# GoekeLab/m6anet

Measured on AMD Instinct MI355X. Metric: DRACH sites/sec at num_iterations=1000, higher is better.
Workload: dtype f32

## Files before the change

include/m6a.h:

```cpp
#ifndef M6A_H
#define M6A_H
#include <stddef.h>
#include <stdint.h>
#ifdef __cplusplus
extern "C" {
#endif

typedef struct m6a_ctx m6a_ctx;

enum {
    M6A_OK = 0,
    M6A_EINVAL = -1,
    M6A_ENOMEM = -2,
    M6A_EHIP = -3,
    M6A_ESTREAM = -4,
    M6A_ENODEV = -5,
    M6A_EUNSUPPORTED = -6,
    M6A_EFORMAT = -7,
    M6A_EIO = -8,
    M6A_EDECLINED = -9
};

enum { M6A_RNG_NUMPY = 0 };

#define M6A_N_WEIGHTS 7997
#define M6A_N_FEATURES 9
#define M6A_MAX_SAMPLES 64
#define M6A_N_REPR 32
#define M6A_N_KMERS 66

int m6a_create(m6a_ctx **out, const float *weights, size_t n_floats, int device_id);
void m6a_destroy(m6a_ctx *ctx);
const char *m6a_last_error(const m6a_ctx *ctx);

int m6a_set_stream(m6a_ctx *ctx, void *hip_stream);
int m6a_set_job_offset(m6a_ctx *ctx, int64_t first_site);
int m6a_sync(m6a_ctx *ctx);
int m6a_set_host_offsets(m6a_ctx *ctx, const int64_t *off_host);
int m6a_prepare_host_io(m6a_ctx *ctx);
int m6a_host_alloc(size_t bytes, void **out);
int m6a_host_free(void *p);
int m6a_host_is_pinned(const void *p, size_t bytes);

int m6a_encode_reads(m6a_ctx *ctx, const float *X, const uint8_t *site_kmers, const int64_t *off,
                     int64_t n_sites, float *read_prob);

int m6a_read_representation(m6a_ctx *ctx, const float *X, const uint8_t *site_kmers, const int64_t *off,
                            int64_t n_sites, float *repr, float *read_prob);

#define M6A_REPR_F32 0
#define M6A_REPR_F16 1
int m6a_read_representation_dtype(m6a_ctx *ctx, const float *X, const uint8_t *site_kmers, const int64_t *off,
                                  int64_t n_sites, void *repr, int dtype, float *read_prob);

int m6a_site_pool(m6a_ctx *ctx, const float *read_prob, const int64_t *off, int64_t n_sites,
                  int n_iters, int n_samples, float read_proba_threshold, uint32_t seed,
                  int rng_mode, int64_t batch_size, int64_t save_per_batch,
                  float *site_prob, double *mod_ratio);

int m6a_infer(m6a_ctx *ctx, const float *X, const uint8_t *site_kmers, const int64_t *off,
              int64_t n_sites, int n_iters, int n_samples, float read_proba_threshold,
              uint32_t seed, int rng_mode, int64_t batch_size, int64_t save_per_batch,
              float *read_prob, float *site_prob, double *mod_ratio);

int m6a_site_expectation(m6a_ctx *ctx, const float *read_prob, const int64_t *off, int64_t n_sites, int n_samples,
                         float read_proba_threshold, float *site_prob, double *mod_ratio, double *mc_sigma);
enum { M6A_SITE_SAMPLED = 0, M6A_SITE_EXPECTED = 1 };
int m6a_set_site_mode(m6a_ctx *ctx, int mode);

int m6a_job_begin(m6a_ctx *ctx, int n_iters, int n_samples, float read_proba_threshold, uint32_t seed, int rng_mode,
                  int64_t batch_size, int64_t save_per_batch, int64_t expect_sites, int64_t expect_reads);
int m6a_job_feed(m6a_ctx *ctx, const float *X, const uint8_t *site_kmers, const int64_t *off, int64_t n_sites);
int m6a_job_feed_collated(m6a_ctx *ctx, const float *features, const int64_t *kmers, const int64_t *n_reads, int64_t n_sites);
int m6a_job_size(const m6a_ctx *ctx, int64_t *n_sites, int64_t *n_reads);
int m6a_job_end(m6a_ctx *ctx, float *read_prob, float *site_prob, double *mod_ratio);
int m6a_job_abort(m6a_ctx *ctx);

int m6a_bag_forward(m6a_ctx *ctx, const float *X, const uint8_t *site_kmers, int64_t n_bags,
                    int bag, float *site_prob);

int m6a_validate_pool(m6a_ctx *ctx, const float *read_prob, const int64_t *off, int64_t n_sites,
                      int n_iters, int n_samples, uint32_t seed, float *y_pred, float *y_pred_avg);
int m6a_validate(m6a_ctx *ctx, const float *X, const uint8_t *site_kmers, const int64_t *off,
                 int64_t n_sites, int n_iters, int n_samples, uint32_t seed, float *read_prob,
                 float *y_pred, float *y_pred_avg);


int64_t m6a_flush_groups(int64_t n_sites, int64_t batch_size, int64_t save_per_batch,
                         int64_t *group_off, int64_t cap);

int64_t m6a_reference_written_sites(int64_t n_sites, int64_t batch_size, int64_t save_per_batch);

int m6a_shard_plan(const int64_t *off, int64_t n_sites, int64_t batch_size, int64_t save_per_batch,
                   int n_shards, int64_t *shard_site_off);

#define M6A_COMM_ID_BYTES 128
int m6a_comm_unique_id(void *id_out);
int m6a_comm_init(m6a_ctx *ctx, const void *unique_id, int rank, int world_size);
int m6a_gather(m6a_ctx *ctx, const float *site_prob, const double *mod_ratio, const int64_t *shard_site_off,
               int dst, float *site_all, double *mod_all);
int m6a_gather_reads(m6a_ctx *ctx, const float *read_prob, const int64_t *shard_read_off, int dst, float *read_all);
int m6a_comm_destroy(m6a_ctx *ctx);
int m6a_comm_count(m6a_ctx *ctx, int *ranks_seen);
int m6a_comm_info(m6a_ctx *ctx, int *rank, int *device, int *rccl_version);
int m6a_device_link(int dev_a, int dev_b, int *link_type, int *hops, int *peer_access);
int m6a_device_count(void);

int m6a_random_stream(m6a_ctx *ctx, uint32_t seed, int64_t n_words, uint32_t *words);

int m6a_profile_enable(m6a_ctx *ctx, int on);
int m6a_profile_read(m6a_ctx *ctx, int kind, double *total_ms, int64_t *n_launches);
int m6a_profile_clock(m6a_ctx *ctx, int kind, double *ghz_median, double *ghz_min, double *ghz_max, double *span_ms, int *n_waves);
int m6a_set_encoder_variant(m6a_ctx *ctx, int mode);
const char *m6a_last_encoder_variant(const m6a_ctx *ctx);
const char *m6a_last_encoder_kernel(const m6a_ctx *ctx);
int m6a_set_scan_driver(m6a_ctx *ctx, int mode);
int m6a_set_table_variant(m6a_ctx *ctx, int mode);
const char *m6a_last_pool_variant(const m6a_ctx *ctx);

const char *m6a_version(void);

typedef struct m6a_prep m6a_prep;
struct m6a_io_prep_table;
int m6a_prep_eventalign(int device_id, const char *path, int n_neighbors, const char *index_path, m6a_prep **out);
const struct m6a_io_prep_table *m6a_prep_table(const m6a_prep *p);
int m6a_prep_times(const m6a_prep *p, double *ms6);
void m6a_prep_free(m6a_prep *p);
const char *m6a_prep_last_error(void);

typedef struct m6a_prep_sites m6a_prep_sites;
struct m6a_io_rows;
typedef struct m6a_prep_host_half {
    int (*rows)(const char *eventalign_path, int64_t n_runs, const int64_t *start, const int64_t *end, const int64_t *read,
                int n_neighbors, int n_threads, struct m6a_io_rows **out);
    const struct m6a_io_prep_table *(*table)(const struct m6a_io_rows *r);
    void (*free)(struct m6a_io_rows *r);
    const char *(*error)(void);
} m6a_prep_host_half;
typedef struct m6a_prep_sites_info {
    int64_t n_sites, n_reads, n_tx;
    const float *X;
    const uint8_t *site_kmers;
    const int64_t *off;
    float *read_prob, *site_prob;
    double *mod_ratio;
    const int64_t *off_host;
    const uint32_t *site_tx;
    const int64_t *site_pos;
    const char *site_kmer7;
    const char *tx_blob;
    const int64_t *tx_off;
    const double *read_ids;
    double ms[8];
    int64_t d2h_bytes;
    int n_rep;
    const int32_t *read_rep;
    int64_t peak_bytes;
    int64_t n_windows, window_bytes;
    int64_t n_bgzf_blocks, compressed_bytes;
    double ms_inflate;
    int64_t n_declined_sites;
} m6a_prep_sites_info;
int m6a_prep_sites_build(int device_id, const char *path, int readcount_min, int readcount_max, int min_segment_count,
                         const char *norm_kmers, const double *norm_mean, const double *norm_std, int n_norm,
                         const m6a_prep_host_half *host, int n_threads, m6a_prep_sites **out);
int m6a_prep_sites_build_multi(int device_id, const char *const *paths, int n_paths, int readcount_min, int readcount_max,
                               int min_segment_count, const char *norm_kmers, const double *norm_mean, const double *norm_std, int n_norm,
                               const m6a_prep_host_half *host, int n_threads, m6a_prep_sites **out);
int m6a_prep_sites_build_windows(int device_id, const char *const *paths, int n_paths, int readcount_min, int readcount_max,
                                 int min_segment_count, const char *norm_kmers, const double *norm_mean, const double *norm_std, int n_norm,
                                 const m6a_prep_host_half *host, int n_threads, int64_t window_bytes, m6a_prep_sites **out);
int m6a_prep_sites_build_names(int device_id, const char *const *paths, int n_paths, int readcount_min, int readcount_max,
                               int min_segment_count, const char *norm_kmers, const double *norm_mean, const double *norm_std, int n_norm,
                               const m6a_prep_host_half *host, int n_threads, int64_t window_bytes, int read_names, m6a_prep_sites **out);
int m6a_prep_sites_read_names(const m6a_prep_sites *p, const uint8_t **names16, const int64_t **name_off, int *n_rep);
double m6a_prep_sites_intern_ms(const m6a_prep_sites *p);
#define M6A_PREP_STREAM_WINDOW_BYTES ((int64_t)256 << 20)
int64_t m6a_prep_sites_stream_bytes(const m6a_prep_sites *p);
int64_t m6a_prep_sites_n_streams(const m6a_prep_sites *p);
const m6a_prep_sites_info *m6a_prep_sites_get(const m6a_prep_sites *p);
int m6a_prep_sites_fetch(m6a_prep_sites *p, float *read_prob, float *site_prob, double *mod_ratio);
int m6a_prep_sites_inputs(m6a_prep_sites *p, float *X, uint8_t *site_kmers, int64_t *off);
void m6a_prep_sites_free(m6a_prep_sites *p);

struct m6a_io_info;
struct m6a_io_info_table;
typedef struct m6a_json_host_half {
    int (*open)(const char *dir, int min_reads, struct m6a_io_info **out);
    const struct m6a_io_info_table *(*table)(const struct m6a_io_info *info);
    int (*rows)(struct m6a_io_info *info, const int64_t *sites, int64_t n, const char *norm_kmers, const double *norm_mean,
                const double *norm_std, int n_norm, int n_threads, float *X, double *read_ids, uint8_t *site_kmers, char *kmer7);
    void (*free)(struct m6a_io_info *info);
    const char *(*error)(void);
} m6a_json_host_half;
int m6a_json_sites_build(int device_id, const char *const *dirs, int n_dirs, int min_reads, const char *norm_kmers,
                         const double *norm_mean, const double *norm_std, int n_norm, const m6a_json_host_half *host, int n_threads,
                         m6a_prep_sites **out);

typedef struct m6a_norm_host_half {
    int (*partials)(const char *json_path, int64_t n_sites, const char *tx_blob, const int64_t *tx_off, const int64_t *pos,
                    const int64_t *start, const int64_t *end, const int64_t *n_reads, const int64_t *sites, int64_t n, int n_threads,
                    double *s, double *s2, char *kmer7);
    const char *(*error)(void);
} m6a_norm_host_half;
typedef struct m6a_norm_stats {
    double ms_upload, ms_kernels, ms_host, ms_fold, ms_total;
    int64_t n_sites, n_reads, n_kmers, n_declined, d2h_bytes, peak_bytes;
} m6a_norm_stats;
int m6a_norm_factors_build(int device_id, const char *json_path, int64_t n_sites, const char *tx_blob, const int64_t *tx_off,
                           const int64_t *pos, const int64_t *start, const int64_t *end, const int64_t *n_reads,
                           const m6a_norm_host_half *host, int n_threads, char *kmers, int64_t *N, double *S, double *S2, double *mean,
                           double *std, int64_t *n_kmers, uint8_t *status, char *kmer7, m6a_norm_stats *stats);

typedef struct m6a_csv_arrays {
    int64_t n_sites, n_tx;
    const int64_t *off;
    const uint32_t *site_tx;
    const int64_t *site_pos;
    const char *kmer5;
    const char *tx_blob;
    const int64_t *tx_off;
    const double *read_ids;
    const int32_t *read_rep;
    int n_rep;
    const float *read_prob, *site_prob;
    const double *mod_ratio;
} m6a_csv_arrays;
typedef struct m6a_csv_stats {
    double ms_format, ms_copy, ms_write;
    int64_t site_bytes, indiv_bytes;
    int64_t n_declined, d2h_bytes, n_rounds;
} m6a_csv_stats;
int m6a_csv_format(int device_id, const m6a_csv_arrays *a, int64_t site_begin, int64_t site_end, char *site_text, int64_t site_cap,
                   char *indiv_text, int64_t indiv_cap, int64_t *site_bytes, int64_t *indiv_bytes, int64_t *n_declined);
int m6a_prep_sites_write_csv(m6a_prep_sites *p, const char *out_dir, int write_header, int64_t n_sites_limit, int n_threads,
                             m6a_csv_stats *stats);

typedef struct m6a_dataprep_stats {
    double ms_front, ms_back, ms_format, ms_copy, ms_write;
    int64_t json_bytes, index_bytes;
    int64_t n_sites, n_runs, n_declined, n_rounds;
    int64_t d2h_bytes, peak_bytes;
} m6a_dataprep_stats;
int m6a_repr_format(int device_id, const double *v, int64_t n, int round3, char *text, int64_t cap, int64_t *off ,
                    int64_t *n_declined);
int m6a_prep_dataprep_write(int device_id, const char *path, const char *out_dir, int readcount_min, int readcount_max,
                            int min_segment_count, int compress, const m6a_prep_host_half *host, int n_threads,
                            m6a_dataprep_stats *stats);

typedef struct m6a_bgzf_stats {
    int64_t n_blocks, compressed_bytes;
    double ms_upload, ms_inflate, ms_crc, ms_copy;
    int64_t d2h_bytes;
} m6a_bgzf_stats;
int m6a_bgzf_inflate(int device_id, const char *path, char *text, int64_t cap, int64_t *n_bytes, m6a_bgzf_stats *stats);

typedef struct m6a_deflate_stats {
    int64_t n_blocks, n_stored;
    double ms_deflate, ms_copy;
    int64_t d2h_bytes;
} m6a_deflate_stats;
int m6a_bgzf_deflate(int device_id, const char *text, int64_t n, char *out, int64_t cap, int64_t *n_bytes, m6a_deflate_stats *stats);
int m6a_bgzf_deflate_level(int device_id, const char *text, int64_t n, int level, char *out, int64_t cap, int64_t *n_bytes,
                           m6a_deflate_stats *stats, int64_t n_by_type[3]);
typedef struct m6a_csv_bgzf_stats {
    double ms_format, ms_deflate, ms_copy, ms_write;
    int64_t site_bytes, indiv_bytes;
    int64_t site_compressed, indiv_compressed;
    int64_t n_blocks, n_stored;
    int64_t n_declined, d2h_bytes, n_rounds;
} m6a_csv_bgzf_stats;
int m6a_prep_sites_write_csv_bgzf(m6a_prep_sites *p, const char *out_dir, int write_header, int64_t n_sites_limit, int n_threads,
                                  m6a_csv_bgzf_stats *stats);
int m6a_prep_sites_write_csv_bgzf_level(m6a_prep_sites *p, const char *out_dir, int write_header, int64_t n_sites_limit, int n_threads,
                                        int level, m6a_csv_bgzf_stats *stats, int64_t n_by_type[3]);

typedef struct m6a_repr_write_stats {
    double ms_kernel, ms_copy, ms_write;
    int64_t n_rounds, n_rows;
    int64_t bytes;
    int64_t round_bytes;
    int64_t d2h_bytes;
} m6a_repr_write_stats;
int m6a_prep_sites_write_read_representation(m6a_prep_sites *p, m6a_ctx *ctx, const char *path, int dtype, int64_t n_sites_limit,
                                             m6a_repr_write_stats *stats);

typedef struct m6a_trainer m6a_trainer;
typedef struct { float lr, beta1, beta2, eps, weight_decay; } m6a_train_config;
int m6a_train_create(m6a_ctx *ctx, const float *weights, size_t n_floats, const m6a_train_config *cfg, m6a_trainer **out);
void m6a_train_destroy(m6a_trainer *t);
int m6a_train_step(m6a_trainer *t, const float *X, const uint8_t *site_kmers, const float *y, int64_t n_bags, int bag,
                   float *loss, float *y_pred);
int m6a_train_epoch(m6a_trainer *t, const float *X, const uint8_t *site_kmers, const int64_t *off, const float *y, int64_t n_sites,
                    const int64_t *order, int64_t n_order, int64_t batch_size, int bag, uint64_t seed,
                    float *loss, float *y_pred);
int m6a_train_sample(const int64_t *off, const int64_t *order, int64_t n_order, int bag, uint64_t seed, int64_t *read_idx);
int m6a_train_grads(m6a_trainer *t, float *grads);
int m6a_train_weights(m6a_trainer *t, float *weights, int64_t *n_steps);
int m6a_train_stats(const m6a_trainer *t, int64_t *n_steps, int64_t *n_launches, int64_t *n_syncs);
int m6a_train_set_clip(m6a_trainer *t, float max_norm);
int m6a_train_last_norm(m6a_trainer *t, float *total_norm);
int m6a_train_state_get(m6a_trainer *t, float *m, float *v, int64_t *n_steps);
int m6a_train_state_set(m6a_trainer *t, const float *m, const float *v, int64_t n_steps);
int m6a_train_set_weights(m6a_trainer *t, const float *blob);
int m6a_train_forward(m6a_trainer *t, const float *X, const uint8_t *site_kmers, int64_t n_bags, int bag, int training,
                      float *s, int64_t *ticket);
int m6a_train_running_stats(m6a_trainer *t, float *stats);
int m6a_train_backward(m6a_trainer *t, int64_t ticket, const float *grad_s, float *grads);

#ifdef __cplusplus
}
#endif
#endif
```

m6anet_amd/_lib.py:

```python
import ctypes as C
import os

_PKG = os.path.dirname(os.path.abspath(__file__))
LIB_PATH = os.environ.get("M6A_HIP_LIB") or os.path.join(_PKG, "libm6a_hip.so")

M6A_OK = 0
ERRORS = {-1: "M6A_EINVAL", -2: "M6A_ENOMEM", -3: "M6A_EHIP", -4: "M6A_ESTREAM", -5: "M6A_ENODEV",
          -6: "M6A_EUNSUPPORTED", -7: "M6A_EFORMAT", -8: "M6A_EIO", -9: "M6A_EDECLINED"}
M6A_EDECLINED = -9
RNG_NUMPY = 0
REPR_DTYPES = {"float32": 0, "float16": 1}

SYMBOLS = ["m6a_create", "m6a_destroy", "m6a_last_error", "m6a_set_stream", "m6a_set_job_offset", "m6a_set_scan_driver", "m6a_set_table_variant", "m6a_set_encoder_variant", "m6a_last_encoder_variant", "m6a_last_encoder_kernel", "m6a_sync", "m6a_set_host_offsets", "m6a_prepare_host_io", "m6a_host_alloc", "m6a_host_free", "m6a_host_is_pinned",
           "m6a_encode_reads", "m6a_read_representation", "m6a_read_representation_dtype", "m6a_site_pool", "m6a_site_expectation", "m6a_set_site_mode", "m6a_infer", "m6a_job_begin", "m6a_job_feed", "m6a_job_feed_collated", "m6a_job_size", "m6a_job_end", "m6a_job_abort", "m6a_bag_forward", "m6a_validate_pool", "m6a_validate", "m6a_flush_groups",
           "m6a_reference_written_sites",
           "m6a_shard_plan", "m6a_comm_unique_id", "m6a_comm_init", "m6a_gather", "m6a_gather_reads", "m6a_device_count", "m6a_random_stream", "m6a_comm_destroy", "m6a_comm_count", "m6a_comm_info", "m6a_device_link", "m6a_profile_enable", "m6a_profile_read", "m6a_profile_clock", "m6a_last_pool_variant",
           "m6a_version", "m6a_prep_eventalign", "m6a_prep_table", "m6a_prep_times", "m6a_prep_free", "m6a_prep_last_error",
           "m6a_prep_sites_build", "m6a_prep_sites_build_multi", "m6a_prep_sites_build_windows", "m6a_prep_sites_build_names", "m6a_prep_sites_read_names", "m6a_prep_sites_intern_ms", "m6a_prep_sites_stream_bytes", "m6a_prep_sites_n_streams", "m6a_prep_sites_get", "m6a_prep_sites_fetch", "m6a_prep_sites_inputs", "m6a_prep_sites_free",
           "m6a_csv_format", "m6a_prep_sites_write_csv", "m6a_bgzf_inflate", "m6a_bgzf_deflate", "m6a_prep_sites_write_csv_bgzf",
           "m6a_bgzf_deflate_level", "m6a_prep_sites_write_csv_bgzf_level", "m6a_prep_sites_write_read_representation", "m6a_json_sites_build", "m6a_norm_factors_build", "m6a_repr_format", "m6a_prep_dataprep_write",
           "m6a_train_create", "m6a_train_destroy", "m6a_train_step", "m6a_train_epoch", "m6a_train_sample", "m6a_train_grads", "m6a_train_weights", "m6a_train_stats",
           "m6a_train_set_clip", "m6a_train_last_norm", "m6a_train_state_get", "m6a_train_state_set",
           "m6a_train_set_weights", "m6a_train_forward", "m6a_train_running_stats", "m6a_train_backward"]

_lib = None


class HostHalf(C.Structure):
    _fields_ = [("rows", C.c_void_p), ("table", C.c_void_p), ("free", C.c_void_p), ("error", C.c_void_p)]


class JsonHostHalf(C.Structure):
    _fields_ = [("open", C.c_void_p), ("table", C.c_void_p), ("rows", C.c_void_p), ("free", C.c_void_p), ("error", C.c_void_p)]


class NormHostHalf(C.Structure):
    _fields_ = [("partials", C.c_void_p), ("error", C.c_void_p)]


class NormStats(C.Structure):
    _fields_ = [("ms_upload", C.c_double), ("ms_kernels", C.c_double), ("ms_host", C.c_double), ("ms_fold", C.c_double),
                ("ms_total", C.c_double), ("n_sites", C.c_int64), ("n_reads", C.c_int64), ("n_kmers", C.c_int64),
                ("n_declined", C.c_int64), ("d2h_bytes", C.c_int64), ("peak_bytes", C.c_int64)]


class PrepSitesInfo(C.Structure):
    _fields_ = [("n_sites", C.c_int64), ("n_reads", C.c_int64), ("n_tx", C.c_int64), ("X", C.c_void_p), ("site_kmers", C.c_void_p),
                ("off", C.c_void_p), ("read_prob", C.c_void_p), ("site_prob", C.c_void_p), ("mod_ratio", C.c_void_p),
                ("off_host", C.c_void_p), ("site_tx", C.c_void_p), ("site_pos", C.c_void_p), ("site_kmer7", C.c_void_p),
                ("tx_blob", C.c_void_p), ("tx_off", C.c_void_p), ("read_ids", C.c_void_p), ("ms", C.c_double * 8),
                ("d2h_bytes", C.c_int64), ("n_rep", C.c_int), ("read_rep", C.c_void_p), ("peak_bytes", C.c_int64),
                ("n_windows", C.c_int64), ("window_bytes", C.c_int64),
                ("n_bgzf_blocks", C.c_int64), ("compressed_bytes", C.c_int64), ("ms_inflate", C.c_double),
                ("n_declined_sites", C.c_int64)]


class BgzfStats(C.Structure):
    _fields_ = [("n_blocks", C.c_int64), ("compressed_bytes", C.c_int64), ("ms_upload", C.c_double), ("ms_inflate", C.c_double),
                ("ms_crc", C.c_double), ("ms_copy", C.c_double), ("d2h_bytes", C.c_int64)]


class DeflateStats(C.Structure):
    _fields_ = [("n_blocks", C.c_int64), ("n_stored", C.c_int64), ("ms_deflate", C.c_double), ("ms_copy", C.c_double), ("d2h_bytes", C.c_int64)]


class CsvBgzfStats(C.Structure):
    _fields_ = [("ms_format", C.c_double), ("ms_deflate", C.c_double), ("ms_copy", C.c_double), ("ms_write", C.c_double),
                ("site_bytes", C.c_int64), ("indiv_bytes", C.c_int64), ("site_compressed", C.c_int64), ("indiv_compressed", C.c_int64),
                ("n_blocks", C.c_int64), ("n_stored", C.c_int64), ("n_declined", C.c_int64), ("d2h_bytes", C.c_int64), ("n_rounds", C.c_int64)]


class CsvArrays(C.Structure):
    _fields_ = [("n_sites", C.c_int64), ("n_tx", C.c_int64), ("off", C.c_void_p), ("site_tx", C.c_void_p), ("site_pos", C.c_void_p),
                ("kmer5", C.c_void_p), ("tx_blob", C.c_char_p), ("tx_off", C.c_void_p), ("read_ids", C.c_void_p), ("read_rep", C.c_void_p),
                ("n_rep", C.c_int), ("read_prob", C.c_void_p), ("site_prob", C.c_void_p), ("mod_ratio", C.c_void_p)]


class CsvStats(C.Structure):
    _fields_ = [("ms_format", C.c_double), ("ms_copy", C.c_double), ("ms_write", C.c_double), ("site_bytes", C.c_int64),
                ("indiv_bytes", C.c_int64), ("n_declined", C.c_int64), ("d2h_bytes", C.c_int64), ("n_rounds", C.c_int64)]


class ReprWriteStats(C.Structure):
    _fields_ = [("ms_kernel", C.c_double), ("ms_copy", C.c_double), ("ms_write", C.c_double), ("n_rounds", C.c_int64), ("n_rows", C.c_int64),
                ("bytes", C.c_int64), ("round_bytes", C.c_int64), ("d2h_bytes", C.c_int64)]


class DataprepStats(C.Structure):
    _fields_ = [("ms_front", C.c_double), ("ms_back", C.c_double), ("ms_format", C.c_double), ("ms_copy", C.c_double), ("ms_write", C.c_double),
                ("json_bytes", C.c_int64), ("index_bytes", C.c_int64), ("n_sites", C.c_int64), ("n_runs", C.c_int64), ("n_declined", C.c_int64),
                ("n_rounds", C.c_int64), ("d2h_bytes", C.c_int64), ("peak_bytes", C.c_int64)]


class TrainConfig(C.Structure):
    _fields_ = [("lr", C.c_float), ("beta1", C.c_float), ("beta2", C.c_float), ("eps", C.c_float), ("weight_decay", C.c_float)]


class M6AError(RuntimeError):
    def __init__(self, code, msg):
        super().__init__("%s (%d): %s" % (ERRORS.get(code, "M6A_E?"), code, msg))
        self.code = code


def _preload_hip_runtime():
    import importlib.util
    try:
        spec = importlib.util.find_spec("torch")
    except (ImportError, ValueError):
        spec = None
    if spec and spec.submodule_search_locations:
        libdir = os.path.join(list(spec.submodule_search_locations)[0], "lib")
        rt = os.path.join(libdir, "libamdhip64.so")
        if os.path.exists(rt):
            C.CDLL(rt, mode=C.RTLD_GLOBAL)
        rccl = os.path.join(libdir, "librccl.so")
        if os.path.exists(rccl):
            os.environ.setdefault("M6A_RCCL_LIB", rccl)


def load():
    global _lib
    if _lib is not None:
        return _lib
    if not os.path.exists(LIB_PATH):
        raise ImportError("libm6a_hip.so is not built: run `python -m m6anet_amd.build` "
                          "(or __graft_entry__.build()); there is no CPU fallback")
    _preload_hip_runtime()
    L = C.CDLL(LIB_PATH)
    vp, i64, i32, u32, f32, sz = C.c_void_p, C.c_int64, C.c_int, C.c_uint32, C.c_float, C.c_size_t
    L.m6a_create.argtypes = [C.POINTER(vp), vp, sz, i32]
    L.m6a_destroy.argtypes = [vp]
    L.m6a_destroy.restype = None
    L.m6a_last_error.argtypes = [vp]
    L.m6a_last_error.restype = C.c_char_p
    L.m6a_set_stream.argtypes = [vp, vp]
    L.m6a_sync.argtypes = [vp]
    L.m6a_set_host_offsets.argtypes = [vp, vp]
    L.m6a_prepare_host_io.argtypes = [vp]
    L.m6a_set_job_offset.argtypes = [vp, i64]
    L.m6a_set_scan_driver.argtypes = [vp, i32]
    L.m6a_set_table_variant.argtypes = [vp, i32]
    L.m6a_set_encoder_variant.argtypes = [vp, i32]
    L.m6a_last_encoder_variant.argtypes = [vp]
    L.m6a_last_encoder_variant.restype = C.c_char_p
    L.m6a_host_alloc.argtypes = [C.c_size_t, C.POINTER(vp)]
    L.m6a_host_free.argtypes = [vp]
    L.m6a_host_is_pinned.argtypes = [vp, C.c_size_t]
    L.m6a_last_encoder_kernel.argtypes = [vp]
    L.m6a_last_encoder_kernel.restype = C.c_char_p
    L.m6a_encode_reads.argtypes = [vp, vp, vp, vp, i64, vp]
    L.m6a_read_representation.argtypes = [vp, vp, vp, vp, i64, vp, vp]
    L.m6a_read_representation_dtype.argtypes = [vp, vp, vp, vp, i64, vp, i32, vp]
    L.m6a_site_pool.argtypes = [vp, vp, vp, i64, i32, i32, f32, u32, i32, i64, i64, vp, vp]
    L.m6a_site_expectation.argtypes = [vp, vp, vp, i64, i32, f32, vp, vp, vp]
    L.m6a_set_site_mode.argtypes = [vp, i32]
    L.m6a_infer.argtypes = [vp, vp, vp, vp, i64, i32, i32, f32, u32, i32, i64, i64, vp, vp, vp]
    L.m6a_job_begin.argtypes = [vp, i32, i32, f32, u32, i32, i64, i64, i64, i64]
    L.m6a_job_feed.argtypes = [vp, vp, vp, vp, i64]
    L.m6a_job_feed_collated.argtypes = [vp, vp, vp, vp, i64]
    L.m6a_job_size.argtypes = [vp, C.POINTER(i64), C.POINTER(i64)]
    L.m6a_job_end.argtypes = [vp, vp, vp, vp]
    L.m6a_job_abort.argtypes = [vp]
    L.m6a_bag_forward.argtypes = [vp, vp, vp, i64, i32, vp]
    L.m6a_validate_pool.argtypes = [vp, vp, vp, i64, i32, i32, C.c_uint32, vp, vp]
    L.m6a_validate.argtypes = [vp, vp, vp, vp, i64, i32, i32, C.c_uint32, vp, vp, vp]
    L.m6a_flush_groups.argtypes = [i64, i64, i64, vp, i64]
    L.m6a_flush_groups.restype = i64
    L.m6a_reference_written_sites.argtypes = [i64, i64, i64]
    L.m6a_reference_written_sites.restype = i64
    L.m6a_shard_plan.argtypes = [vp, i64, i64, i64, i32, vp]
    L.m6a_comm_unique_id.argtypes = [vp]
    L.m6a_comm_init.argtypes = [vp, vp, i32, i32]
    L.m6a_gather.argtypes = [vp, vp, vp, vp, i32, vp, vp]
    L.m6a_gather_reads.argtypes = [vp, vp, vp, i32, vp]
    L.m6a_device_count.argtypes = []
    L.m6a_random_stream.argtypes = [vp, u32, i64, vp]
    L.m6a_comm_destroy.argtypes = [vp]
    pi = C.POINTER(i32)
    L.m6a_comm_count.argtypes = [vp, pi]
    L.m6a_comm_info.argtypes = [vp, pi, pi, pi]
    L.m6a_device_link.argtypes = [i32, i32, pi, pi, pi]
    L.m6a_profile_enable.argtypes = [vp, i32]
    L.m6a_profile_read.argtypes = [vp, i32, C.POINTER(C.c_double), C.POINTER(i64)]
    L.m6a_profile_clock.argtypes = [vp, i32] + [C.POINTER(C.c_double)] * 4 + [C.POINTER(i32)]
    L.m6a_last_pool_variant.argtypes = [vp]
    L.m6a_last_pool_variant.restype = C.c_char_p
    L.m6a_version.restype = C.c_char_p
    L.m6a_prep_eventalign.argtypes = [i32, C.c_char_p, i32, C.c_char_p, C.POINTER(vp)]
    L.m6a_prep_table.argtypes = [vp]
    L.m6a_prep_table.restype = vp
    L.m6a_prep_times.argtypes = [vp, C.POINTER(C.c_double)]
    L.m6a_prep_free.argtypes = [vp]
    L.m6a_prep_free.restype = None
    L.m6a_prep_sites_build.argtypes = [i32, C.c_char_p, i32, i32, i32, C.c_char_p, vp, vp, i32, C.POINTER(HostHalf), i32, C.POINTER(vp)]
    L.m6a_prep_sites_build_multi.argtypes = [i32, C.POINTER(C.c_char_p), i32, i32, i32, i32, C.c_char_p, vp, vp, i32, C.POINTER(HostHalf), i32,
                                             C.POINTER(vp)]
    L.m6a_prep_sites_build_windows.argtypes = [i32, C.POINTER(C.c_char_p), i32, i32, i32, i32, C.c_char_p, vp, vp, i32, C.POINTER(HostHalf), i32,
                                               i64, C.POINTER(vp)]
    L.m6a_prep_sites_build_names.argtypes = [i32, C.POINTER(C.c_char_p), i32, i32, i32, i32, C.c_char_p, vp, vp, i32, C.POINTER(HostHalf), i32,
                                             i64, i32, C.POINTER(vp)]
    L.m6a_prep_sites_read_names.argtypes = [vp, C.POINTER(vp), C.POINTER(vp), C.POINTER(i32)]
    L.m6a_prep_sites_intern_ms.argtypes = [vp]
    L.m6a_prep_sites_intern_ms.restype = C.c_double
    for f in (L.m6a_prep_sites_stream_bytes, L.m6a_prep_sites_n_streams):
        f.argtypes = [vp]
        f.restype = C.c_int64
    L.m6a_json_sites_build.argtypes = [i32, C.POINTER(C.c_char_p), i32, i32, C.c_char_p, vp, vp, i32, C.POINTER(JsonHostHalf), i32, C.POINTER(vp)]
    L.m6a_norm_factors_build.argtypes = [i32, C.c_char_p, i64, vp, vp, vp, vp, vp, vp, C.POINTER(NormHostHalf), i32, vp, vp, vp, vp, vp, vp,
                                         C.POINTER(i64), vp, vp, C.POINTER(NormStats)]
    L.m6a_prep_sites_get.argtypes = [vp]
    L.m6a_prep_sites_get.restype = C.POINTER(PrepSitesInfo)
    L.m6a_prep_sites_fetch.argtypes = [vp, vp, vp, vp]
    L.m6a_prep_sites_inputs.argtypes = [vp, vp, vp, vp]
    L.m6a_prep_sites_free.argtypes = [vp]
    L.m6a_prep_sites_free.restype = None
    pl = C.POINTER(i64)
    L.m6a_csv_format.argtypes = [i32, C.POINTER(CsvArrays), i64, i64, vp, i64, vp, i64, pl, pl, pl]
    L.m6a_prep_sites_write_csv.argtypes = [vp, C.c_char_p, i32, i64, i32, C.POINTER(CsvStats)]
    L.m6a_bgzf_inflate.argtypes = [i32, C.c_char_p, vp, i64, pl, C.POINTER(BgzfStats)]
    L.m6a_bgzf_deflate.argtypes = [i32, C.c_char_p, i64, vp, i64, pl, C.POINTER(DeflateStats)]
    L.m6a_prep_sites_write_csv_bgzf.argtypes = [vp, C.c_char_p, i32, i64, i32, C.POINTER(CsvBgzfStats)]
    L.m6a_bgzf_deflate_level.argtypes = [i32, C.c_char_p, i64, i32, vp, i64, pl, C.POINTER(DeflateStats), pl]
    L.m6a_prep_sites_write_csv_bgzf_level.argtypes = [vp, C.c_char_p, i32, i64, i32, i32, C.POINTER(CsvBgzfStats), pl]
    L.m6a_prep_sites_write_read_representation.argtypes = [vp, vp, C.c_char_p, i32, i64, C.POINTER(ReprWriteStats)]
    L.m6a_repr_format.argtypes = [i32, vp, i64, i32, vp, i64, vp, pl]
    L.m6a_prep_dataprep_write.argtypes = [i32, C.c_char_p, C.c_char_p, i32, i32, i32, i32, C.POINTER(HostHalf), i32, C.POINTER(DataprepStats)]
    L.m6a_train_create.argtypes = [vp, vp, sz, C.POINTER(TrainConfig), C.POINTER(vp)]
    L.m6a_train_destroy.argtypes = [vp]
    L.m6a_train_destroy.restype = None
    L.m6a_train_step.argtypes = [vp, vp, vp, vp, i64, i32, vp, vp]
    L.m6a_train_epoch.argtypes = [vp, vp, vp, vp, vp, i64, vp, i64, i64, i32, C.c_uint64, vp, vp]
    L.m6a_train_sample.argtypes = [vp, vp, i64, i32, C.c_uint64, vp]
    L.m6a_train_grads.argtypes = [vp, vp]
    L.m6a_train_weights.argtypes = [vp, vp, pl]
    L.m6a_train_stats.argtypes = [vp, pl, pl, pl]
    L.m6a_train_set_clip.argtypes = [vp, C.c_float]
    L.m6a_train_last_norm.argtypes = [vp, vp]
    L.m6a_train_state_get.argtypes = [vp, vp, vp, pl]
    L.m6a_train_state_set.argtypes = [vp, vp, vp, i64]
    L.m6a_train_set_weights.argtypes = [vp, vp]
    L.m6a_train_forward.argtypes = [vp, vp, vp, i64, i32, i32, vp, pl]
    L.m6a_train_running_stats.argtypes = [vp, vp]
    L.m6a_train_backward.argtypes = [vp, i64, vp, vp]
    L.m6a_prep_last_error.argtypes = []
    L.m6a_prep_last_error.restype = C.c_char_p
    for name in SYMBOLS:
        fn = getattr(L, name)
        if fn.restype is C.c_int and name not in ("m6a_flush_groups", "m6a_reference_written_sites"):
            fn.restype = C.c_int
    _lib = L
    return L
```

m6anet_amd/csrc/m6a_api.hip:

```cpp
#include "m6a_ctx.h"

#if !defined(__HIP_DEVICE_COMPILE__)
#ifndef M6A_MT_JUMP_PATH
#error "build with -DM6A_MT_JUMP_PATH=\"<repo>/m6anet_amd/assets/mt19937_jump.bin\" (m6anet_amd/build.py does)"
#endif
asm(".section .rodata\n"
    ".global m6a_mt_jump_blob\n.global m6a_mt_jump_blob_end\n.hidden m6a_mt_jump_blob\n.hidden m6a_mt_jump_blob_end\n.balign 64\n"
    "m6a_mt_jump_blob:\n.incbin \"" M6A_MT_JUMP_PATH "\"\n"
    "m6a_mt_jump_blob_end:\n.byte 0\n.previous\n");
#endif

namespace {

thread_local std::string g_create_error;

std::mutex g_live_mu;
std::vector<m6a_ctx *> g_live;
void join_background_setups()
{
    std::lock_guard<std::mutex> g(g_live_mu);
    for (m6a_ctx *c : g_live)
        if (c->warm.joinable()) c->warm.join();
    g_live.clear();
}

}

using namespace m6a_detail;

namespace m6a_detail {


int fail(m6a_ctx *c, int code, const char *fmt, ...)
{
    char buf[512];
    va_list ap;
    va_start(ap, fmt);
    vsnprintf(buf, sizeof buf, fmt, ap);
    va_end(ap);
    if (c && c->warm.joinable() && std::this_thread::get_id() != c->warm.get_id()) c->warm.join();
    if (c) c->err = buf; else g_create_error = buf;
    return code;
}


bool is_device_ptr(const void *p)
{
    if (!p) return false;
    hipPointerAttribute_t at;
    hipError_t e = hipPointerGetAttributes(&at, p);
    if (e != hipSuccess) { (void)hipGetLastError(); return false; }
    return at.type == hipMemoryTypeDevice || at.type == hipMemoryTypeManaged;
}

enum { O_E = 0, O_W1 = 132, O_B1 = 2382, O_G = 2532, O_BE = 2682, O_MU = 2832, O_VAR = 2982,
       O_W2 = 3132, O_B2 = 7932, O_W3 = 7964, O_B3 = 7996 };

void build_fragments(const float *w, std::vector<float> &frag, std::vector<float> &frag2, std::vector<float> &w1e)
{
    std::vector<float> w1(160 * 16, 0.f), w2(32 * 160, 0.f), alpha(160, 0.f), beta(160, 0.f);
    for (int j = 0; j < 150; j++) {
        for (int k = 0; k < 15; k++) w1[j * 16 + k] = w[O_W1 + 15 * j + k];
        w1[j * 16 + 15] = w[O_B1 + j];
        const float invstd = 1.0f / std::sqrt(w[O_VAR + j] + 1e-5f);
        alpha[j] = w[O_G + j] * invstd;
        beta[j] = std::fmaf(-w[O_MU + j], alpha[j], w[O_BE + j]);
    }
    w1[150 * 16 + 15] = 1.0f;
    alpha[150] = 1.0f;
    for (int o = 0; o < 32; o++) {
        for (int k = 0; k < 150; k++) w2[o * 160 + k] = w[O_W2 + 150 * o + k];
        w2[o * 160 + 150] = w[O_B2 + o];
    }
    const float bn_scale = 0x1p-64f;
    for (float &v : alpha) v *= bn_scale;
    for (float &v : beta) v *= bn_scale;
    for (float &v : w2) v *= 0x1p+64f;
    const float w3_scale = 0.5f;
    auto unit_of_row = [](int m, int i) { return 32 * m + 2 * ((i & 3) + 4 * (i >> 3)) + ((i >> 2) & 1); };
    auto out_unit = [](int q, int half) {
        if (half == 0) return q < 8 ? 2 * q + 1 : 2 * (q - 8) + 17;
        return q < 8 ? 2 * q + 2 : (q < 15 ? 2 * (q - 8) + 18 : 0);
    };
    auto out_unit_of_row = [&](int i) { return out_unit((i & 3) + 4 * (i >> 3), (i >> 2) & 1); };
    frag.assign(M6A_WFRAG_FLOATS, 0.f);
    for (int lane = 0; lane < 64; lane++) {
        const int col = lane & 31, half = lane >> 5;
        for (int m = 0; m < 5; m++) {
            for (int st = 0; st < 8; st++)
                frag[(m * 8 + st) * 64 + lane] = w1[unit_of_row(m, col) * 16 + 2 * st + half];
            for (int q = 0; q < 16; q++)
                frag[(40 + m * 16 + q) * 64 + lane] = w2[out_unit_of_row(col) * 160 + 32 * m + 2 * q + half];
        }
        for (int q = 0; q < 16; q++)
            frag[(120 + q) * 64 + lane] = w3_scale * w[O_W3 + out_unit(q, half)];
    }
    frag2.assign(M6A_WFRAG2_FLOATS, 0.f);
    w1e.assign(M6A_W1E_FLOATS + M6A_BN_FLOATS, 0.f);
    for (int lane = 0; lane < 64; lane++) {
        const int col = lane & 31, half = lane >> 5;
        for (int m = 0; m < 5; m++) {
            for (int st = 0; st < 4; st++) frag2[(m * 4 + st) * 64 + lane] = w1[unit_of_row(m, col) * 16 + 2 * st + half];
            frag2[(20 + m) * 64 + lane] = w1[unit_of_row(m, col) * 16 + 8];
        }
    }
    for (int m = 0; m < 5; m++)
        for (int col = 0; col < 32; col++) {
            for (int e = 0; e < 6; e++) w1e[(m * 7 + e) * 32 + col] = w1[unit_of_row(m, col) * 16 + 9 + e];
            w1e[(m * 7 + 6) * 32 + col] = w1[unit_of_row(m, col) * 16 + 15];
        }
    for (int m = 0; m < 5; m++)
        for (int half = 0; half < 2; half++)
            for (int q = 0; q < 16; q++) {
                const int u = 32 * m + 2 * q + half;
                w1e[M6A_W1E_FLOATS + ((m * 2 + half) * 16 + q) * 2] = alpha[u];
                w1e[M6A_W1E_FLOATS + ((m * 2 + half) * 16 + q) * 2 + 1] = beta[u];
            }
}

int64_t flush_groups(int64_t S, int64_t bs, int64_t spb, int64_t base, std::vector<int64_t> &goff)
{
    goff.clear();
    goff.push_back(0);
    if (S <= 0) return 0;
    const int64_t it0 = base / bs;
    const int64_t nb = (S + bs - 1) / bs;
    int64_t start_b = 0;
    for (int64_t b = 0; b < nb; b++) {
        if ((it0 + b + 1) % spb) {
            goff.push_back(std::min((b + 1) * bs, S));
            start_b = b + 1;
        }
    }
    if (start_b < nb) goff.push_back(S);
    return (int64_t)goff.size() - 1;
}

bool base_is_group_start(int64_t base, int64_t bs, int64_t spb)
{
    if (base < 0 || base % bs) return false;
    const int64_t it0 = base / bs;
    return it0 == 0 || (it0 % spb) != 0;
}

int ensure_groups(m6a_ctx *c, hipStream_t st, int64_t S, int64_t bs, int64_t spb)
{
    const int64_t base = c->job_offset;
    if (c->goff_key.valid && c->goff_key.S == S && c->goff_key.bs == bs && c->goff_key.spb == spb &&
        c->goff_key.base == base) return M6A_OK;
    if (!base_is_group_start(base, bs, spb))
        return fail(c, M6A_EINVAL, "job offset %lld does not start a flush group for batch_size=%lld save_per_batch=%lld",
                    (long long)base, (long long)bs, (long long)spb);
    std::vector<int64_t> g;
    const int64_t G = flush_groups(S, bs, spb, base, g);
    int64_t gmax = 0;
    for (int64_t i = 0; i < G; i++) gmax = std::max(gmax, g[i + 1] - g[i]);
    HIPCHK(c, c->goff.ensure(g.size() * sizeof(int64_t)));
    HIPCHK(c, hipMemcpyAsync(c->goff.p, g.data(), g.size() * sizeof(int64_t), hipMemcpyHostToDevice, st));
    HIPCHK(c, hipStreamSynchronize(st));
    c->goff_key = {S, bs, spb, base, G, gmax, true};
    return M6A_OK;
}

constexpr int kJumpPerRegime = 31, kJumpPolyWords = 312;
constexpr int64_t kXheadWords = 22016;

extern "C" const unsigned char m6a_mt_jump_blob[];
extern "C" const unsigned char m6a_mt_jump_blob_end[];

struct JumpRegime { int64_t G; const uint64_t *polys; };

const JumpRegime *jump_regimes(int *n_out)
{
    static JumpRegime reg[8];
    static int n = 0;
    static std::once_flag once;
    std::call_once(once, [] {
        const unsigned char *b = m6a_mt_jump_blob;
        const size_t len = (size_t)(m6a_mt_jump_blob_end - m6a_mt_jump_blob);
        uint32_t hdr[4];
        if (len >= 24 && std::memcmp(b, "M6AMTJP1", 8) == 0) {
            std::memcpy(hdr, b + 8, 16);
            const size_t per = 8 + (size_t)hdr[1] * hdr[2] * 8;
            if (hdr[0] <= 8 && hdr[1] == (uint32_t)kJumpPerRegime && hdr[2] == (uint32_t)kJumpPolyWords && hdr[3] == 512 &&
                len == 24 + hdr[0] * per)
                for (uint32_t r = 0; r < hdr[0]; r++) {
                    const unsigned char *q = b + 24 + r * per;
                    int64_t G;
                    std::memcpy(&G, q, 8);
                    reg[n++] = {G, (const uint64_t *)(q + 8)};
                }
        }
    });
    *n_out = n;
    return reg;
}

int launch_stream(m6a_ctx *c, hipStream_t st, uint32_t seed, int64_t len, uint32_t *raw)
{
    int n_reg = 0;
    const JumpRegime *reg = jump_regimes(&n_reg);
    const JumpRegime *use = nullptr;
    static const bool allowed = !(getenv("M6A_MT_SEGMENTS") && getenv("M6A_MT_SEGMENTS")[0] == '0');
    if (allowed && n_reg > 0 && len > reg[0].G + kXheadWords) {
        use = &reg[n_reg - 1];
        for (int r = 0; r < n_reg; r++) if (len <= (int64_t)(kJumpPerRegime + 1) * reg[r].G) { use = &reg[r]; break; }
    }
    if (!use) {
        hipLaunchKernelGGL(mt19937_kernel, dim3(1), dim3(640), 0, st, seed, len, raw, (const uint32_t *)nullptr, len,
                           (uint32_t *)nullptr, (int64_t)0);
        HIPCHK(c, hipGetLastError());
        return M6A_OK;
    }
    const int n_seg = (int)std::min<int64_t>((len + use->G - 1) / use->G, kJumpPerRegime + 1);
    const size_t poly_bytes = (size_t)kJumpPerRegime * kJumpPolyWords * 8;
    HIPCHK(c, c->mt_scratch.ensure((size_t)kXheadWords * 4 + (size_t)kJumpPerRegime * 1078 * 4 + poly_bytes));
    uint32_t *xhead = (uint32_t *)c->mt_scratch.p, *hist = xhead + kXheadWords;
    uint64_t *d_polys = (uint64_t *)(hist + (size_t)kJumpPerRegime * 1078);
    if (c->mt_polys_G != use->G) {
        HIPCHK(c, hipMemcpyAsync(d_polys, use->polys, poly_bytes, hipMemcpyHostToDevice, st));
        c->mt_polys_G = use->G;
    }
    hipLaunchKernelGGL(mt19937_kernel, dim3(1), dim3(640), 0, st, seed, kXheadWords - 624, raw, (const uint32_t *)nullptr,
                       kXheadWords, xhead, kXheadWords);
    hipLaunchKernelGGL(mt_jump_kernel, dim3(17, (unsigned)(n_seg - 1)), dim3(256), 0, st, (const uint32_t *)xhead,
                       (const uint64_t *)d_polys, hist);
    hipLaunchKernelGGL(mt19937_kernel, dim3((unsigned)n_seg), dim3(640), 0, st, seed, len, raw, (const uint32_t *)hist, use->G,
                       (uint32_t *)nullptr, (int64_t)0);
    HIPCHK(c, hipGetLastError());
    return M6A_OK;
}

int ensure_raw(m6a_ctx *c, hipStream_t st, uint32_t seed, int64_t len)
{
    if (c->raw_len >= len && c->raw_seed == seed) return M6A_OK;
    if (len > ((int64_t)1 << 31) - 512)
        return fail(c, M6A_ESTREAM, "a flush group would need %lld MT19937 words (cap 2^31); "
                    "reduce batch_size*save_per_batch or num_iterations", (long long)len);
    len = (len + 1023) / 1024 * 1024;
    c->raw_len = 0;
    c->rt.valid = false;
    HIPCHK(c, c->raw.ensure((size_t)len * 4));
    int rc = launch_stream(c, st, seed, len, (uint32_t *)c->raw.p);
    if (rc) return rc;
    c->raw_seed = seed; c->raw_len = len;
    return M6A_OK;
}

void pairwise_rec(int lo, int n, MeanPlan &p)
{
    if (n <= 128) {
        p.leaf_start.push_back(lo);
        p.merge_after.push_back(0);
        return;
    }
    int n2 = n / 2;
    n2 -= n2 % 8;
    pairwise_rec(lo, n2, p);
    pairwise_rec(lo + n2, n - n2, p);
    p.merge_after.back()++;
}

int plan_iteration(const MeanPlan &p, int row, int lane)
{
    const int L = (int)p.merge_after.size();
    const int ps = p.row_pass[row], i = p.row_round[row];
    if (ps < 0) return lane < p.n_rem ? p.T - p.n_rem + lane : -1;
    const int b = 8 * ps + (lane >> 3);
    if (b >= L) return -1;
    const int len = p.leaf_start[b + 1] - p.leaf_start[b];
    return i < len / 8 ? p.leaf_start[b] + 8 * i + (lane & 7) : -1;
}

void build_mean_plan(int T, MeanPlan &p)
{
    p = MeanPlan();
    p.T = T;
    pairwise_rec(0, T, p);
    p.leaf_start.push_back(T);
    const int L = (int)p.merge_after.size();
    const int last_len = p.leaf_start[L] - p.leaf_start[L - 1];
    p.n_rem = last_len % 8;
    if (p.n_rem) { p.row_pass.push_back(-1); p.row_round.push_back(0); }
    const int P = (L + 7) / 8;
    for (int ps = 0; ps < P; ps++) {
        int rounds = 0;
        for (int b = 8 * ps; b < std::min(L, 8 * ps + 8); b++)
            rounds = std::max(rounds, (p.leaf_start[b + 1] - p.leaf_start[b]) / 8);
        rounds = std::max(rounds, 1);
        for (int i = 0; i < rounds; i++) { p.row_pass.push_back(ps); p.row_round.push_back(i); }
    }
    int d = 0;
    for (int b = 0; b < L; b++) {
        d++; p.depth = std::max(p.depth, d); d -= p.merge_after[b];
        p.max_merge = std::max<int>(p.max_merge, p.merge_after[b]);
    }
    p.reg_ctl.assign((size_t)std::max(1, (T - p.n_rem) / 8), 0u);
    for (int b = 0; b + 1 < L; b++) p.reg_ctl[(size_t)p.leaf_start[b + 1] / 8 - 1] = 1u | ((uint32_t)p.merge_after[b] << 8);
    const int rows = (int)p.row_pass.size();
    p.row_meta.assign((size_t)rows * 4, 0u);
    for (int r = 0; r < rows; r++) {
        uint32_t *m = &p.row_meta[(size_t)r * 4];
        uint64_t live = 0;
        for (int l = 0; l < 64; l++) live |= (uint64_t)(plan_iteration(p, r, l) >= 0) << l;
        m[1] = (uint32_t)live; m[2] = (uint32_t)(live >> 32);
        const int ps = p.row_pass[r];
        if (ps < 0) { m[0] = 1u << 25; continue; }
        if (r + 1 == rows || p.row_pass[r + 1] != ps) {
            const int nl = std::min(8, L - 8 * ps);
            m[0] = (1u << 24) | ((uint32_t)nl << 26) | (ps == P - 1 ? 1u << 30 : 0u);
            for (int bl = 0; bl < nl; bl++) m[3] |= (uint32_t)(p.merge_after[8 * ps + bl] & 15) << (4 * bl);
        }
    }
}

int ensure_mean_plan(m6a_ctx *c, hipStream_t st, int T)
{
    if (c->plan.T == T && c->plan_dev.p) return M6A_OK;
    build_mean_plan(T, c->plan);
    const MeanPlan &p = c->plan;
    if (p.depth > M6A_MEAN_STACK) return fail(c, M6A_EUNSUPPORTED, "n_iters %d: pairwise-sum tree deeper than %d", T, M6A_MEAN_STACK);
    const size_t b0 = p.leaf_start.size() * 4, b1 = (p.merge_after.size() + 3) / 4 * 4, b2 = std::max<size_t>(p.row_meta.size(), 1) * 4;
    const size_t b3 = p.reg_ctl.size() * 4;
    HIPCHK(c, c->plan_dev.ensure(b0 + b1 + b2 + b3));
    char *d = (char *)c->plan_dev.p;
    HIPCHK(c, hipMemcpyAsync(d, p.leaf_start.data(), b0, hipMemcpyHostToDevice, st));
    HIPCHK(c, hipMemcpyAsync(d + b0, p.merge_after.data(), p.merge_after.size(), hipMemcpyHostToDevice, st));
    if (!p.row_meta.empty())
        HIPCHK(c, hipMemcpyAsync(d + b0 + b1, p.row_meta.data(), p.row_meta.size() * 4, hipMemcpyHostToDevice, st));
    HIPCHK(c, hipMemcpyAsync(d + b0 + b1 + b2, p.reg_ctl.data(), b3, hipMemcpyHostToDevice, st));
    HIPCHK(c, hipStreamSynchronize(st));
    c->plan_off[0] = 0; c->plan_off[1] = b0; c->plan_off[2] = b0 + b1; c->plan_off[3] = b0 + b1 + b2;
    c->tab_key.valid = false;
    return M6A_OK;
}

void plan_args(m6a_ctx *c, PoolArgs &a)
{
    const char *d = (const char *)c->plan_dev.p;
    a.leaf_start = (const int *)(d + c->plan_off[0]);
    a.merge_after = (const uint8_t *)(d + c->plan_off[1]);
    a.row_meta = (const uint32_t *)(d + c->plan_off[2]);
    a.n_leaves = (int)c->plan.merge_after.size();
    a.n_rows = (int)c->plan.row_pass.size();
    a.n_rem = c->plan.n_rem;
    a.stack_depth = c->plan.depth;
    a.reg_ctl = (const uint32_t *)(d + c->plan_off[3]);
    a.reg_rounds = (a.T - c->plan.n_rem) / 8;
    a.reg_final_merges = c->plan.merge_after.back();
}

int64_t stream_need(int64_t gmax, int T, int K)
{
    const int64_t A = (int64_t)T * K;
    return gmax * (2 * A + A / 16) + 8192;
}

uint32_t *ctl_cursor(m6a_ctx *c) { return c->h_ctl; }
int32_t *ctl_slot(m6a_ctx *c) { return (int32_t *)(c->h_ctl + M6A_HIST_BINS); }
int32_t *ctl_build_n(m6a_ctx *c) { return ctl_slot(c) + M6A_RTAB_MAX_N + 1; }
int32_t *ctl_build_slot(m6a_ctx *c) { return ctl_build_n(c) + M6A_RTAB_MAX_N; }
constexpr size_t kCtlWords = M6A_HIST_BINS + (M6A_RTAB_MAX_N + 1) + 2 * M6A_RTAB_MAX_N;

int rtab_missing(const m6a_ctx *c, uint32_t seed, int T, int K, int64_t need, const uint32_t *hist, int *n_distinct)
{
    const bool valid = c->rt.valid && c->rt.seed == seed && c->rt.A == (int64_t)T * K && c->raw_seed == seed &&
                       c->rt.n_blk * 64 >= need && c->rt.n_blk == c->raw_len / 64;
    int missing = 0, distinct = 0;
    for (int n = 2; n <= M6A_RTAB_MAX_N; n++)
        if (hist[n]) { distinct++; if (!valid || c->rt.slot_of_n[n] < 0) missing++; }
    if (n_distinct) *n_distinct = distinct;
    return missing;
}

int ensure_rtab(m6a_ctx *c, hipStream_t st, uint32_t seed, int T, int K, int64_t gmax, const uint32_t *hist, bool *usable)
{
    *usable = false;
    const int64_t need = stream_need(gmax, T, K);
    int rc = ensure_raw(c, st, seed, need);
    if (rc) return rc;
    auto &rt = c->rt;
    const int64_t n_blk = c->raw_len / 64;
    if (!(rt.valid && rt.seed == seed && rt.A == (int64_t)T * K && rt.n_blk == n_blk)) {
        rt.valid = false; rt.used = 0;
        for (int n = 0; n <= M6A_RTAB_MAX_N; n++) rt.slot_of_n[n] = -1;
    }
    std::vector<int> todo;
    for (int n = 2; n <= M6A_RTAB_MAX_N; n++)
        if (hist[n] && rt.slot_of_n[n] < 0) todo.push_back(n);
    const int64_t c_stride = n_blk * 64;
    const size_t slot_bytes = (size_t)c_stride * 2 + (size_t)(n_blk + 1) * 4;
    const bool fresh = !rt.valid || rt.n_blk != n_blk;
    const int want = (fresh ? 1 : rt.used) + (int)todo.size();
    if (fresh || want > rt.cap) {
        int new_cap = std::max(want, fresh ? 0 : rt.cap * 2);
        new_cap = std::min(std::max(new_cap, std::max(32, c->rt_presize)), M6A_RTAB_MAX_N + 1);
        size_t free_b = 0, total_b = 0;
        HIPCHK(c, hipMemGetInfo(&free_b, &total_b));
        const size_t held = fresh ? 0 : (size_t)rt.cap * slot_bytes;
        const size_t budget = std::min<size_t>((size_t)16 << 30, (free_b + held) / 2);
        if ((size_t)new_cap * slot_bytes > budget) new_cap = want;
        if ((size_t)new_cap * slot_bytes > budget) return M6A_OK;
        uint16_t *nC = nullptr; uint32_t *nRS = nullptr;
        if (fresh) {
            if (rt.C) (void)hipFree(rt.C);
            if (rt.RS) (void)hipFree(rt.RS);
            rt.C = nullptr; rt.RS = nullptr; rt.cap = 0;
        }
        if (hipMalloc((void **)&nC, (size_t)new_cap * c_stride * 2 + 64) != hipSuccess) { (void)hipGetLastError(); return M6A_OK; }
        if (hipMalloc((void **)&nRS, (size_t)new_cap * (n_blk + 1) * 4) != hipSuccess) { (void)hipGetLastError(); (void)hipFree(nC); return M6A_OK; }
        if (!fresh && rt.used) {
            HIPCHK(c, hipMemcpyAsync(nC, rt.C, (size_t)rt.used * c_stride * 2, hipMemcpyDeviceToDevice, st));
            HIPCHK(c, hipMemcpyAsync(nRS, rt.RS, (size_t)rt.used * (n_blk + 1) * 4, hipMemcpyDeviceToDevice, st));
            HIPCHK(c, hipStreamSynchronize(st));
            c->graveyard.push_back(rt.C); c->graveyard.push_back(rt.RS);
        }
        rt.C = nC; rt.RS = nRS; rt.cap = new_cap;
        if (fresh) {
            HIPCHK(c, hipMemsetAsync(rt.C, 0, (size_t)c_stride * 2, st));
            HIPCHK(c, hipMemsetAsync(rt.RS, 0, (size_t)(n_blk + 1) * 4, st));
            rt.used = 1;
        }
        rt.valid = true; rt.seed = seed; rt.A = (int64_t)T * K; rt.n_blk = n_blk;
    }
    if (!todo.empty()) {
        int32_t *bn = ctl_build_n(c), *bs = ctl_build_slot(c);
        for (size_t i = 0; i < todo.size(); i++) { bn[i] = todo[i]; bs[i] = rt.used; rt.slot_of_n[todo[i]] = rt.used++; }
        HIPCHK(c, c->ctl_dev.ensure(kCtlWords * 4));
        int32_t *d_bn = (int32_t *)c->ctl_dev.p + (ctl_build_n(c) - (int32_t *)c->h_ctl);
        HIPCHK(c, hipMemcpyAsync(d_bn, bn, (size_t)2 * M6A_RTAB_MAX_N * 4, hipMemcpyHostToDevice, st));
        RtabBuild b;
        b.raw = (const uint32_t *)c->raw.p; b.n_blk = (uint32_t)n_blk; b.build_n = d_bn; b.build_slot = d_bn + M6A_RTAB_MAX_N;
        b.C = rt.C; b.RS = rt.RS; b.c_stride = c_stride; b.n_build = (int)todo.size();
        const unsigned gx = (unsigned)std::min<int64_t>((n_blk + 63) / 64, 65535);
        const unsigned gn = (unsigned)((todo.size() + 7) / 8);
        hipLaunchKernelGGL(rtab_count_kernel, dim3(gn, gx), dim3(256), 0, st, b);
        hipLaunchKernelGGL(rtab_scan_kernel, dim3((unsigned)todo.size()), dim3(256), 0, st, b);
        hipLaunchKernelGGL(rtab_fill_kernel, dim3(gn, gx), dim3(256), 0, st, b);
        HIPCHK(c, hipGetLastError());
        HIPCHK(c, hipStreamSynchronize(st));
    }
    *usable = true;
    return M6A_OK;
}

int uniform_slice(m6a_ctx *c, hipStream_t st, uint32_t seed, int n, int T, int K, int jmax, const uint16_t **C)
{
    *C = nullptr;
    if (n < 2) return M6A_OK;
    std::vector<uint32_t> hist(M6A_HIST_BINS, 0u);
    hist[n] = 1;
    bool usable = false;
    int rc = ensure_rtab(c, st, seed, T, K, jmax, hist.data(), &usable);
    if (rc) return rc;
    if (!usable) return fail(c, M6A_ENOMEM, "no device memory for the index table of bag size %d", n);
    const int64_t slot = c->rt.slot_of_n[n], A = (int64_t)T * K;
    uint32_t total = 0;
    HIPCHK(c, hipMemcpyAsync(&total, c->rt.RS + slot * (c->rt.n_blk + 1) + c->rt.n_blk, 4, hipMemcpyDeviceToHost, st));
    HIPCHK(c, hipStreamSynchronize(st));
    if ((int64_t)total < A * jmax) return fail(c, M6A_ESTREAM, "MT19937 stream too short for a flush group");
    *C = c->rt.C + slot * c->rt.n_blk * 64;
    return M6A_OK;
}

int ensure_table_reg(m6a_ctx *c, hipStream_t st, uint32_t seed, int n, int T, int K, int jmax)
{
    auto &k = c->tab_reg_key;
    if (k.valid && k.seed == seed && k.n == n && k.T == T && k.K == K && k.jmax >= jmax) return M6A_OK;
    k.valid = false;
    const size_t per_j = (size_t)(T + 8) * K;
    const size_t bytes = (size_t)jmax * per_j * 2 + 4096;
    HIPCHK(c, c->tab_reg.ensure(bytes));
    HIPCHK(c, hipMemsetAsync(c->tab_reg.p, 0, bytes, st));
    const uint16_t *C = nullptr;
    int rc = uniform_slice(c, st, seed, n, T, K, jmax, &C);
    if (rc) return rc;
    if (C) {
        const int64_t A = (int64_t)T * K;
        hipLaunchKernelGGL(rtab_to_reg_table_kernel, dim3((unsigned)((A * jmax + 255) / 256)), dim3(256), 0, st,
                           C, A, (int64_t)per_j, jmax, (uint16_t *)c->tab_reg.p);
        HIPCHK(c, hipGetLastError());
    }
    k = {seed, n, T, K, jmax, true};
    return M6A_OK;
}

int ensure_table(m6a_ctx *c, hipStream_t st, uint32_t seed, int n, int T, int K, int jmax)
{
    int rc = ensure_mean_plan(c, st, T);
    if (rc) return rc;
    auto &k = c->tab_key;
    if (k.valid && k.seed == seed && k.n == n && k.T == T && k.K == K && k.jmax >= jmax) return M6A_OK;
    k.valid = false;
    const MeanPlan &p = c->plan;
    const int rows = (int)p.row_pass.size();
    c->iter_of.resize((size_t)rows * 64);
    for (int r = 0; r < rows; r++)
        for (int l = 0; l < 64; l++) c->iter_of[(size_t)r * 64 + l] = plan_iteration(p, r, l);
    const size_t words = (size_t)jmax * rows * 5 * 64;
    HIPCHK(c, c->tab.ensure(words * 4 + c->iter_of.size() * 4));
    int *d_iter = (int *)((uint32_t *)c->tab.p + words);
    HIPCHK(c, hipMemcpyAsync(d_iter, c->iter_of.data(), c->iter_of.size() * 4, hipMemcpyHostToDevice, st));
    const uint16_t *C = nullptr;
    rc = uniform_slice(c, st, seed, n, T, K, jmax, &C);
    if (rc) return rc;
    if (C) {
        hipLaunchKernelGGL(rtab_to_lds_table_kernel, dim3((unsigned)((words + 255) / 256)), dim3(256), 0, st,
                           C, (int64_t)T * K, K, rows, jmax, (const int *)d_iter, (uint32_t *)c->tab.p);
        HIPCHK(c, hipGetLastError());
    } else {
        HIPCHK(c, hipMemsetAsync(c->tab.p, 0, words * 4, st));
    }
    k = {seed, n, T, K, jmax, true};
    return M6A_OK;
}

void prof_begin(m6a_ctx *c, int kind)
{
    Profiler &p = c->prof;
    if (!p.on || !(p.mask >> kind & 1)) return;
    if (p.used[kind] >= kMaxProfiled) { p.dropped[kind]++; return; }
    if ((int)p.start[kind].size() <= p.used[kind]) {
        hipEvent_t a, b;
        (void)hipEventCreate(&a); (void)hipEventCreate(&b);
        p.start[kind].push_back(a); p.stop[kind].push_back(b);
    }
    (void)hipEventRecord(p.start[kind][p.used[kind]], c->stream);
}
void prof_end(m6a_ctx *c, int kind)
{
    Profiler &p = c->prof;
    if (!p.on || !(p.mask >> kind & 1) || p.used[kind] >= kMaxProfiled) return;
    (void)hipEventRecord(p.stop[kind][p.used[kind]], c->stream);
    p.used[kind]++;
}

void host_bag_range(m6a_ctx *c, const int64_t *off, int64_t S);
int sync_and_check(m6a_ctx *c);

int query_bags(m6a_ctx *c, const int64_t *d_off, int64_t S)
{
    if (c->side_work) { HIPCHK(c, hipStreamSynchronize(c->s_prep)); c->side_work = false; }
    c->h_minmax[0] = ~0ull; c->h_minmax[1] = 0ull; c->h_minmax[2] = 0ull;
    HIPCHK(c, hipMemcpyAsync(c->d_minmax, c->h_minmax, 24, hipMemcpyHostToDevice, c->stream));
    HIPCHK(c, hipMemsetAsync(c->d_hist, 0, M6A_HIST_BINS * 4, c->stream));
    hipLaunchKernelGGL(bag_minmax_kernel, dim3((unsigned)std::min<int64_t>((S + 255) / 256, 512)), dim3(256), 0,
                       c->stream, d_off, S, c->d_minmax, c->d_hist);
    HIPCHK(c, hipGetLastError());
    HIPCHK(c, hipMemcpyAsync(c->h_minmax, c->d_minmax, 24, hipMemcpyDeviceToHost, c->stream));
    HIPCHK(c, hipMemcpyAsync(c->h_hist, c->d_hist, M6A_HIST_BINS * 4, hipMemcpyDeviceToHost, c->stream));
    HIPCHK(c, hipStreamSynchronize(c->stream));
    c->bag_min = (int64_t)c->h_minmax[0];
    c->bag_max = (int64_t)c->h_minmax[1];
    c->n_reads = (int64_t)c->h_minmax[2];
    return M6A_OK;
}

int bag_stats(m6a_ctx *c, const int64_t *d_off, int64_t S)
{
    const int64_t *h = c->hint_off;
    c->hint_off = nullptr;
    if (!h) return query_bags(c, d_off, S);
    if (h[0] != 0) return fail(c, M6A_EINVAL, "off[0] must be 0");
    host_bag_range(c, h, S);
    if (c->bag_min < 0) return fail(c, M6A_EINVAL, "off[] must be non-decreasing");
    unsigned long long hash = 0;
    for (int i = 0; i < M6A_HIST_BINS; i++) hash += (unsigned long long)c->h_hist[i] * m6a_bin_weight(i);
    hipStream_t st = c->s_prep ? c->s_prep : c->stream;
    if (st != c->stream) {
        HIPCHK(c, hipEventRecord(c->ev_main, c->stream));
        HIPCHK(c, hipStreamWaitEvent(st, c->ev_main, 0));
    }
    HIPCHK(c, hipMemsetAsync(c->d_minmax, 0xff, 8, st));
    HIPCHK(c, hipMemsetAsync(c->d_minmax + 1, 0, 16, st));
    HIPCHK(c, hipMemsetAsync(c->d_hist, 0, M6A_HIST_BINS * 4, st));
    hipLaunchKernelGGL(bag_minmax_kernel, dim3((unsigned)std::min<int64_t>((S + 255) / 256, 512)), dim3(256), 0,
                       st, d_off, S, c->d_minmax, c->d_hist);
    hipLaunchKernelGGL(bag_verify_kernel, dim3(1), dim3(256), 0, st, c->d_minmax, c->d_hist, (unsigned long long)c->bag_min,
                       (unsigned long long)c->bag_max, (unsigned long long)c->n_reads, hash, c->d_err);
    HIPCHK(c, hipGetLastError());
    c->side_work = true;
    return M6A_OK;
}

static unsigned enc_args(m6a_ctx *c, EncArgs &a, const float *X, const uint8_t *km, const int64_t *off, int64_t S, int64_t R, float *rp)
{
    a.X = X; a.site_kmers = km; a.off = off; a.wfrag = c->d_wfrag; a.emb = c->d_emb; a.read_prob = rp;
    a.wfrag2 = c->d_wfrag2; a.w1e_tab = c->d_w1e; a.bn = c->d_w1e + M6A_W1E_FLOATS; a.err = c->d_err;
    a.n_sites = S; a.n_reads = R; a.n_tiles = (R + 31) / 32; a.b3 = c->b3;
    a.clk = nullptr;
    const int64_t max_waves = (int64_t)c->n_cu * 8;
    a.tiles_per_wave = (a.n_tiles + max_waves - 1) / max_waves;
    const int64_t waves = (a.n_tiles + a.tiles_per_wave - 1) / a.tiles_per_wave;
    return (unsigned)((waves + 3) / 4);
}

int launch_encode(m6a_ctx *c, const float *X, const uint8_t *km, const int64_t *off, int64_t S,
                  int64_t R, float *rp)
{
    if (R <= 0 || S <= 0) return M6A_OK;
    EncArgs a;
    const unsigned blocks = enc_args(c, a, X, km, off, S, R, rp);
    a.clk = c->prof.clk_for(0);
    const bool fits32 = S < 0x7ffffff0LL && a.n_tiles < 0x7ffffff0LL;
    if (c->enc_variant == 2 && !fits32) return fail(c, M6A_EUNSUPPORTED, "12-slot encoder: more than 2^31 sites or tiles");
    const bool scalar_chain = c->bag_min >= M6A_CSITE_MIN_BAG && fits32;
    const bool csite = c->enc_variant == 2 || (c->enc_variant == 4 && scalar_chain);
    const bool site16 = !csite && c->enc_variant != 3 && scalar_chain;
    c->enc_variant_used = csite ? "csite12" : "general16";
    c->enc_kernel_used = csite ? "enc_csite_kernel" : site16 ? "enc_site16_kernel" : "enc_kernel";
    prof_begin(c, 0);
    if (csite) hipLaunchKernelGGL(enc_csite_kernel, dim3(blocks), dim3(256), 0, c->stream, a);
    else if (site16) hipLaunchKernelGGL(enc_site16_kernel, dim3(blocks), dim3(256), 0, c->stream, a);
    else hipLaunchKernelGGL(enc_kernel, dim3(blocks), dim3(256), 0, c->stream, a);
    prof_end(c, 0);
    HIPCHK(c, hipGetLastError());
    return M6A_OK;
}

int launch_repr(m6a_ctx *c, const float *X, const uint8_t *km, const int64_t *off, int64_t S, int64_t R, void *repr, int dtype, float *rp)
{
    if (R <= 0 || S <= 0) return M6A_OK;
    EncReprArgs ra;
    const unsigned blocks = enc_args(c, ra.enc, X, km, off, S, R, rp);
    ra.repr = repr;
    c->enc_variant_used = "general16";
    c->enc_kernel_used = dtype == M6A_REPR_F16 ? "enc_repr_kernel<true>" : "enc_repr_kernel";
    prof_begin(c, 0);
    if (dtype == M6A_REPR_F16)
        hipLaunchKernelGGL(enc_repr_kernel<true>, dim3(blocks), dim3(256), 0, c->stream, ra);
    else
        hipLaunchKernelGGL(enc_repr_kernel<false>, dim3(blocks), dim3(256), 0, c->stream, ra);
    prof_end(c, 0);
    HIPCHK(c, hipGetLastError());
    return M6A_OK;
}

int repr_writer_begin(m6a_ctx *c, int device, hipStream_t *stream)
{
    settle(c);
    HintScope hint_scope(c);
    if (c->job.open) return job_busy(c);
    if (c->device != device) return fail(c, M6A_EINVAL, "the context is on device %d, the sites are on device %d", c->device, device);
    HIPCHK(c, hipSetDevice(c->device));
    *stream = c->stream;
    return M6A_OK;
}

int repr_writer_round(m6a_ctx *c, const float *X, const uint8_t *km, const int64_t *off, int64_t *off_round, int64_t s0, int64_t s1,
                      int64_t r0, int64_t nr, void *repr, int dtype)
{
    if (nr <= 0 || s1 <= s0) return M6A_OK;
    hipLaunchKernelGGL(rebase_off_kernel, dim3((unsigned)((s1 - s0 + 1 + 255) / 256)), dim3(256), 0, c->stream, off + s0, s1 - s0 + 1, off_round);
    HIPCHK(c, hipGetLastError());
    return launch_repr(c, X + r0 * 9, km + s0 * 3, off_round, s1 - s0, nr, repr, dtype, nullptr);
}

RtabUse rtab_use(m6a_ctx *c, int64_t nmax, uint32_t si_base = 0, uint32_t si_count = 0)
{
    RtabUse u;
    u.C = c->rt.C; u.RS = c->rt.RS; u.slot_of_n = (const int32_t *)c->ctl_dev.p + M6A_HIST_BINS;
    u.rank = (uint32_t *)c->rt_rank.p; u.order = (const uint32_t *)c->rt_order.p;
    u.c_stride = c->rt.n_blk * 64; u.n_blk = (uint32_t)c->rt.n_blk;
    u.bag_cap = (int)std::max<int64_t>(64, (nmax + 63) / 64 * 64);
    u.si_base = si_base; u.si_count = si_count;
    return u;
}

int rtab_prepare(m6a_ctx *c, hipStream_t st, PoolArgs a, int64_t nmax, int64_t gmax, uint32_t seed, bool *use)
{
    *use = false;
    const int T = a.T, K = a.K;
    const int64_t S = a.n_sites;
    const int64_t need = stream_need(gmax, T, K);
    if (nmax > M6A_RTAB_MAX_N || c->scan_driver == 1 || c->scan_driver == 2) {
        if (c->scan_driver == 3)
            return fail(c, M6A_EUNSUPPORTED, "index-table pooling needs every bag <= %d reads (largest: %lld)", M6A_RTAB_MAX_N, (long long)nmax);
        return M6A_OK;
    }
    int distinct = 0;
    const int missing = rtab_missing(c, seed, T, K, need, c->h_hist, &distinct);
    if (c->rt_credit_seed != seed || c->rt_credit_A != (int64_t)T * K) { c->rt_credit_seed = seed; c->rt_credit_A = (int64_t)T * K; c->rt_credit = 0; }
    bool use_rtab = c->scan_driver == 3 || missing == 0 || c->rt_credit + S >= (int64_t)16 * missing;
    if (use_rtab) c->rt_credit = 0; else c->rt_credit += S;
    if (!use_rtab) return M6A_OK;
    int rc = ensure_rtab(c, st, seed, T, K, gmax, c->h_hist, &use_rtab);
    if (rc) return rc;
    if (!use_rtab) return M6A_OK;
    a.raw = (const uint32_t *)c->raw.p; a.raw_len = c->raw_len;
    HIPCHK(c, c->rt_rank.ensure((size_t)S * 4));
    HIPCHK(c, c->rt_order.ensure((size_t)S * 4));
    HIPCHK(c, c->ctl_dev.ensure(kCtlWords * 4));
    HIPCHK(c, hipEventSynchronize(c->ev_ctl));
    uint32_t *cur = ctl_cursor(c);
    uint32_t run = 0;
    for (int n = M6A_HIST_BINS - 1; n > M6A_RTAB_SMALL_N; n--) { cur[n] = run; run += c->h_hist[n]; }
    for (int x = 0; x < 8; x++)
        for (int n = M6A_RTAB_SMALL_N - ((M6A_RTAB_SMALL_N - x) & 7); n >= 0; n -= 8) { cur[n] = run; run += c->h_hist[n]; }
    std::memcpy(ctl_slot(c), c->rt.slot_of_n, sizeof c->rt.slot_of_n);
    HIPCHK(c, hipMemcpyAsync(c->ctl_dev.p, c->h_ctl, (size_t)(M6A_HIST_BINS + M6A_RTAB_MAX_N + 1) * 4, hipMemcpyHostToDevice, st));
    HIPCHK(c, hipEventRecord(c->ev_ctl, st));
    const RtabUse u = rtab_use(c, nmax);
    const unsigned n_order_blocks = (unsigned)((S + 255) / 256);
    const unsigned n_chain_blocks = (unsigned)std::min<int64_t>((a.n_groups + 3) / 4, (int64_t)c->n_cu * 16);
    hipLaunchKernelGGL(rtab_prep_kernel, dim3(n_order_blocks + n_chain_blocks), dim3(256), 0, st, a, u,
                       (uint32_t *)c->ctl_dev.p, (uint32_t *)c->rt_order.p, n_order_blocks);
    HIPCHK(c, hipGetLastError());
    *use = true;
    return M6A_OK;
}

struct PoolPlan {
    enum Kind { none, table_reg, table, ragged_table, scan_group, scan_site, expected } kind = none;
    PoolArgs a = {};
    int64_t bag_min = 0, bag_max = 0;
    unsigned blocks = 0, start_blocks = 0;
    size_t lds = 0;
    int64_t n_big = 0, cap_big = 0, cap_small = 0;
};

int pool_plan(m6a_ctx *c, hipStream_t st, const int64_t *off, int64_t S, int T, int K, uint32_t seed, int64_t bs, int64_t spb,
              PoolPlan *p)
{
    *p = PoolPlan();
    PoolArgs &a = p->a;
    if (S <= 0) return M6A_OK;
    if (c->site_mode == M6A_SITE_EXPECTED) {
        if (!base_is_group_start(c->job_offset, bs, spb))
            return fail(c, M6A_EINVAL, "job offset %lld does not start a flush group for batch_size=%lld save_per_batch=%lld",
                        (long long)c->job_offset, (long long)bs, (long long)spb);
        if (c->bag_min < 0 || c->bag_max > 0x7fffffff) return fail(c, M6A_EINVAL, "off[] is not a non-decreasing CSR array");
        a.off = off; a.n_sites = S; a.K = K;
        p->bag_min = c->bag_min; p->bag_max = c->bag_max;
        p->kind = PoolPlan::expected;
        return M6A_OK;
    }
    int rc = ensure_groups(c, st, S, bs, spb);
    if (rc) return rc;
    const int64_t nmin = c->bag_min, nmax = c->bag_max;
    if (nmin < 0 || nmax > 0x7fffffff) return fail(c, M6A_EINVAL, "off[] is not a non-decreasing CSR array");
    a.off = off; a.goff = (const int64_t *)c->goff.p; a.err = c->d_err;
    a.n_groups = c->goff_key.G; a.n_sites = S; a.T = T; a.K = K;
    const int64_t gmax = c->goff_key.gmax;

    rc = ensure_mean_plan(c, st, T);
    if (rc) return rc;
    plan_args(c, a);
    const bool uniform = nmin == nmax && nmin >= 1 && nmin <= M6A_TABLE_MAX_N && K == 20 && gmax <= 4096;
    const bool reg_ok = uniform && c->plan.depth <= M6A_REG_STACK && c->n_reads < (int64_t)1 << 30 &&
                        (int64_t)gmax * (T + 8) * K * 2 <= (int64_t)256 << 20;
    if (uniform && reg_ok && c->table_variant != 1) {
        rc = ensure_table_reg(c, st, seed, (int)nmin, T, K, (int)gmax);
        if (rc) return rc;
        a.tab = (const uint32_t *)c->tab_reg.p; a.uniform_n = (int)nmin; a.jmax = (int)gmax;
        const int64_t wpj = (a.n_groups + 255) / 256;
        a.reg_items = wpj * a.jmax;
        p->blocks = (unsigned)((a.reg_items + 7) / 8 * 8);
        p->kind = PoolPlan::table_reg;
        return M6A_OK;
    }
    if (uniform && c->plan.max_merge <= 15) {
        rc = ensure_table(c, st, seed, (int)nmin, T, K, (int)gmax);
        if (rc) return rc;
        a.tab = (const uint32_t *)c->tab.p; a.uniform_n = (int)nmin; a.jmax = (int)gmax;
        const int64_t gblocks = (a.n_groups + 7) / 8;
        int64_t nbj = std::max<int64_t>(1, ((int64_t)c->n_cu * 5 + a.jmax - 1) / a.jmax);
        nbj = std::min<int64_t>(nbj, (gblocks + 3) / 4);
        p->blocks = (unsigned)(nbj * a.jmax);
        p->lds = (size_t)4 * (128 + 8 * a.stack_depth) * sizeof(float);
        p->kind = PoolPlan::table;
        return M6A_OK;
    }
    bool use_rtab = false;
    rc = rtab_prepare(c, st, a, nmax, gmax, seed, &use_rtab);
    if (rc) return rc;
    if (use_rtab) {
        a.raw = (const uint32_t *)c->raw.p; a.raw_len = c->raw_len;
        for (int n = M6A_RTAB_SMALL_N + 1; n < M6A_HIST_BINS; n++) p->n_big += c->h_hist[n];
        p->cap_big = nmax; p->cap_small = std::min<int64_t>(nmax, M6A_RTAB_SMALL_N);
        p->kind = PoolPlan::ragged_table;
        return M6A_OK;
    }
    rc = ensure_raw(c, st, seed, stream_need(gmax, T, K));
    if (rc) return rc;
    a.raw = (const uint32_t *)c->raw.p; a.raw_len = c->raw_len;
    HIPCHK(c, c->start_pos.ensure((size_t)S * sizeof(uint32_t)));
    a.start_pos = (uint32_t *)c->start_pos.p;
    int64_t cap = 64;
    while (cap < nmax && cap < M6A_BAG_LDS) cap *= 2;
    a.bag_cap = (int)cap;
    p->lds = (size_t)4 * (a.bag_cap + (32 * K + 256) * 5 / 4 + 32 + M6A_MEAN_STACK) * sizeof(float);
    const int64_t wg_per_cu = std::max<int64_t>(1, std::min<int64_t>(a.bag_cap >= 256 ? 5 : 8, (160 * 1024) / (int64_t)p->lds));
    const int64_t wave_slots = (int64_t)c->n_cu * wg_per_cu * 4;
    const bool by_group = c->scan_driver ? c->scan_driver == 1 : a.n_groups * 5 >= wave_slots * 3;
    p->kind = by_group ? PoolPlan::scan_group : PoolPlan::scan_site;
    p->blocks = (unsigned)std::min<int64_t>(((by_group ? a.n_groups : S) + 3) / 4, wave_slots / 4);
    p->start_blocks = (unsigned)std::min<int64_t>((a.n_groups + 3) / 4, (int64_t)c->n_cu * 8);
    return M6A_OK;
}

int launch_expect(m6a_ctx *c, const float *rp, const int64_t *off, int64_t S, int K, float thr, int64_t nmin, int64_t nmax,
                  float *site, double *mod, double *sigma)
{
    if (S <= 0) return M6A_OK;
    ExpectArgs a;
    a.read_prob = rp; a.off = off; a.site_prob = site; a.mod_ratio = mod; a.mc_sigma = sigma;
    a.n_sites = S; a.K = K; a.thr = thr;
    const bool lane = nmin == nmax && nmin >= 1 && nmin <= 32;
    a.uniform_n = lane ? (int)nmin : 0;
    c->pool_variant = lane ? "expected-lane" : "expected-wave";
    prof_begin(c, 1);
    if (lane) {
        const unsigned blocks = (unsigned)std::min<int64_t>((S + 255) / 256, (int64_t)c->n_cu * 8);
        if (nmin % 4 == 0 && (uintptr_t)rp % 16 == 0) hipLaunchKernelGGL(site_expect_lane_kernel<true>, dim3(blocks), dim3(256), 0, c->stream, a);
        else hipLaunchKernelGGL(site_expect_lane_kernel<false>, dim3(blocks), dim3(256), 0, c->stream, a);
    } else {
        const unsigned blocks = (unsigned)std::min<int64_t>((S + 15) / 16, (int64_t)c->n_cu * 4);
        hipLaunchKernelGGL(site_expect_wave_kernel, dim3(blocks), dim3(256), 0, c->stream, a);
    }
    prof_end(c, 1);
    HIPCHK(c, hipGetLastError());
    return M6A_OK;
}

int pool_run(m6a_ctx *c, const PoolPlan &p, const float *rp, float thr, float *site, double *mod)
{
    if (p.kind == PoolPlan::none) return M6A_OK;
    if (p.kind == PoolPlan::expected)
        return launch_expect(c, rp, p.a.off, p.a.n_sites, p.a.K, thr, p.bag_min, p.bag_max, site, mod, nullptr);
    static const char *const names[] = {"none", "table-reg", "table", "ragged-table", "scan-group", "scan-site"};
    PoolArgs a = p.a;
    a.read_prob = rp; a.site_prob = site; a.mod_ratio = mod; a.thr = thr;
    a.clk = c->prof.clk_for(1);
    c->pool_variant = names[p.kind];
    const bool k20 = a.K == 20;
    prof_begin(c, 1);
    switch (p.kind) {
    case PoolPlan::none: case PoolPlan::expected: break;
    case PoolPlan::table_reg:
        hipLaunchKernelGGL(pool_reg_kernel, dim3(p.blocks), dim3(64), 0, c->stream, a);
        break;
    case PoolPlan::table:
        hipLaunchKernelGGL(pool_table_kernel, dim3(p.blocks), dim3(256), p.lds, c->stream, a);
        break;
    case PoolPlan::ragged_table: {
        auto launch = [&](int64_t base, int64_t count, int64_t cap_n) {
            if (count <= 0) return;
            const RtabUse u = rtab_use(c, cap_n, (uint32_t)base, (uint32_t)count);
            const size_t lds = (size_t)(u.bag_cap + 16 + M6A_MEAN_STACK) * sizeof(float);
            const unsigned blocks = (unsigned)((count + 7) / 8 * 8);
            if (k20) hipLaunchKernelGGL(pool_rtab_kernel<20>, dim3(blocks), dim3(64), lds, c->stream, a, u);
            else hipLaunchKernelGGL(pool_rtab_kernel<0>, dim3(blocks), dim3(64), lds, c->stream, a, u);
        };
        launch(0, p.n_big, p.cap_big);
        launch(p.n_big, a.n_sites - p.n_big, p.cap_small);
        break;
    }
    case PoolPlan::scan_group:
        if (k20) hipLaunchKernelGGL(pool_scan_group_kernel<20>, dim3(p.blocks), dim3(256), p.lds, c->stream, a);
        else hipLaunchKernelGGL(pool_scan_group_kernel<0>, dim3(p.blocks), dim3(256), p.lds, c->stream, a);
        break;
    case PoolPlan::scan_site:
        hipLaunchKernelGGL(pool_scan_start_kernel, dim3(p.start_blocks), dim3(256), 0, c->stream, a);
        if (k20) hipLaunchKernelGGL(pool_scan_site_kernel<20>, dim3(p.blocks), dim3(256), p.lds, c->stream, a);
        else hipLaunchKernelGGL(pool_scan_site_kernel<0>, dim3(p.blocks), dim3(256), p.lds, c->stream, a);
        break;
    }
    prof_end(c, 1);
    HIPCHK(c, hipGetLastError());
    return M6A_OK;
}

int launch_pool(m6a_ctx *c, const float *rp, const int64_t *off, int64_t S, int T, int K, float thr,
                uint32_t seed, int64_t bs, int64_t spb, float *site, double *mod)
{
    PoolPlan p;
    const int rc = pool_plan(c, c->stream, off, S, T, K, seed, bs, spb, &p);
    return rc ? rc : pool_run(c, p, rp, thr, site, mod);
}

template <int>
static inline void bag_range_loop(const int64_t *off, int64_t S, int64_t *mn_out, int64_t *mx_out)
{
    int64_t mn = INT64_MAX, mx = 0;
    for (int64_t s = 0; s < S; s++) {
        const int64_t n = off[s + 1] - off[s];
        mn = n < mn ? n : mn;
        mx = n > mx ? n : mx;
    }
    *mn_out = mn; *mx_out = mx;
}
__attribute__((target("avx2"))) static void bag_range_avx2(const int64_t *off, int64_t S, int64_t *mn, int64_t *mx) { bag_range_loop<1>(off, S, mn, mx); }
static void bag_range_base(const int64_t *off, int64_t S, int64_t *mn, int64_t *mx) { bag_range_loop<0>(off, S, mn, mx); }

void host_bag_range(m6a_ctx *c, const int64_t *off, int64_t S)
{
    int64_t mn = INT64_MAX, mx = 0;
    static const bool avx2 = __builtin_cpu_supports("avx2");
    (avx2 ? bag_range_avx2 : bag_range_base)(off, S, &mn, &mx);
    auto bin = [](int64_t n) { return n < 0 ? 0 : n > M6A_RTAB_MAX_N ? M6A_RTAB_MAX_N + 1 : n; };
    std::memset(c->h_hist, 0, M6A_HIST_BINS * 4);
    if (mn == mx || S == 0) {
        if (S > 0) c->h_hist[bin(mn)] = (uint32_t)S;
    } else {
        c->hist_part.assign((size_t)8 * M6A_HIST_BINS, 0u);
        uint32_t (*part)[M6A_HIST_BINS] = (uint32_t (*)[M6A_HIST_BINS])c->hist_part.data();
        int64_t s = 0;
        for (; s + 8 <= S; s += 8)
            for (int k = 0; k < 8; k++) part[k][bin(off[s + k + 1] - off[s + k])]++;
        for (; s < S; s++) part[0][bin(off[s + 1] - off[s])]++;
        for (int i = 0; i < M6A_HIST_BINS; i++) {
            uint32_t t = 0;
            for (int k = 0; k < 8; k++) t += part[k][i];
            c->h_hist[i] = t;
        }
    }
    c->bag_min = S > 0 ? mn : 0; c->bag_max = mx; c->n_reads = off[S];
}

int job_busy(m6a_ctx *c)
{
    if (c->job.open) return fail(c, M6A_EINVAL, "a streaming job is open on this context (m6a_job_end or m6a_job_abort first)");
    return M6A_OK;
}

int check_pool_args(m6a_ctx *c, int64_t S, int T, int K, int rng_mode, int64_t bs, int64_t spb)
{
    if (!c) return M6A_EINVAL;
    if (S < 0) return fail(c, M6A_EINVAL, "n_sites < 0");
    if (T < 1) return fail(c, M6A_EINVAL, "n_iters must be >= 1");
    if (K < 1 || K > M6A_MAX_SAMPLES) return fail(c, M6A_EINVAL, "n_samples must be in 1..%d", M6A_MAX_SAMPLES);
    if ((int64_t)T * K > 0x3fffffff) return fail(c, M6A_EINVAL, "n_iters*n_samples too large");
    if (rng_mode != M6A_RNG_NUMPY) return fail(c, M6A_EINVAL, "rng_mode %d: M6A_RNG_NUMPY (0) is the only value (include/m6a.h)", rng_mode);
    if (bs < 1 || spb < 1) return fail(c, M6A_EINVAL, "batch_size and save_per_batch must be >= 1");
    return M6A_OK;
}

int deferred_error(m6a_ctx *c)
{
    if (*c->h_err) {
        const int e = *c->h_err;
        *c->h_err = 0;
        if (e == 2) return fail(c, M6A_EINVAL, "encoder: a 32-read tile spans more than 3 sites (bag < 16 reads) in the 12-slot kernel");
        if (e == 4) return fail(c, M6A_EHIP, "pool_rtab_kernel: the dynamic LDS block does not start at offset 0");
        if (e == 3) return fail(c, M6A_EINVAL, "the host offsets given to m6a_set_host_offsets differ from the device off[] of the call");
        return fail(c, M6A_ESTREAM, "MT19937 stream too short for a flush group");
    }
    return M6A_OK;
}

int sync_and_check(m6a_ctx *c)
{
    if (c->side_work) { HIPCHK(c, hipStreamSynchronize(c->s_prep)); c->side_work = false; }
    HIPCHK(c, hipMemcpyAsync(c->h_err, c->d_err, sizeof(int), hipMemcpyDeviceToHost, c->stream));
    HIPCHK(c, hipStreamSynchronize(c->stream));
    for (void *p : c->graveyard) (void)hipFree(p);
    c->graveyard.clear();
    if (*c->h_err) {
        HIPCHK(c, hipMemsetAsync(c->d_err, 0, sizeof(int), c->stream));
        return deferred_error(c);
    }
    return M6A_OK;
}

void warm_default(m6a_ctx *c)
{
    if (hipSetDevice(c->device) != hipSuccess) { (void)hipGetLastError(); return; }
    const uint32_t seed = 0;
    const int T = 1000, K = 20, n = 20;
    const int64_t gmax = 32;
    hipStream_t st = c->s_prep;
    hipLaunchKernelGGL(m6a_touch_kernels, dim3(1), dim3(1), 0, st);
    hipLaunchKernelGGL(m6a_touch_pool_reg, dim3(1), dim3(1), 0, st);
    hipLaunchKernelGGL(m6a_touch_pool_rtab, dim3(1), dim3(1), 0, st);
    hipLaunchKernelGGL(m6a_touch_expect, dim3(1), dim3(1), 0, st);
    (void)hipGetLastError();
    auto cancelled = [c] { return c->warm_cancel.load(std::memory_order_relaxed); };
    int rc = cancelled() ? 0 : ensure_mean_plan(c, st, T);
    if (!rc && !cancelled()) rc = ensure_raw(c, st, seed, stream_need(gmax, T, K));
    if (!rc && !cancelled()) {
        const char *e = getenv("M6A_WARM_SLOTS");
        c->rt_presize = e && atoi(e) > 0 ? std::min(atoi(e), M6A_RTAB_MAX_N + 1) : 0;
        rc = ensure_table_reg(c, st, seed, n, T, K, (int)gmax);
        if (!rc && c->rt_presize > 2) {
            std::vector<uint32_t> hist(M6A_HIST_BINS, 0u);
            for (int m = 2; m < c->rt_presize && m <= M6A_RTAB_MAX_N; m++) hist[m] = 1;
            bool usable = false;
            rc = ensure_rtab(c, st, seed, T, K, gmax, hist.data(), &usable);
        }
        c->rt_presize = 0;
    }
    (void)hipStreamSynchronize(st);
    if (rc) { c->tab_reg_key.valid = false; c->err.clear(); }
}

}


extern "C" {

const char *m6a_version(void) { return "m6a_hip 0.1 (gfx950)"; }

const char *m6a_last_error(const m6a_ctx *ctx)
{
    settle(const_cast<m6a_ctx *>(ctx));
    return ctx ? ctx->err.c_str() : g_create_error.c_str();
}

int m6a_create(m6a_ctx **out, const float *weights, size_t n_floats, int device_id)
{
    if (!out) return M6A_EINVAL;
    *out = nullptr;
    if (!weights || n_floats != M6A_N_WEIGHTS)
        return fail(nullptr, M6A_EINVAL, "weights must be %d floats (got %zu)", M6A_N_WEIGHTS, n_floats);
    for (int i = O_W2; i < O_W3; i++)
        if (std::isfinite(weights[i]) && std::fabs(weights[i]) >= 0x1p+63f)
            return fail(nullptr, M6A_EUNSUPPORTED, "layer-2 weight %d is %g: beyond 2^63 in magnitude", i - O_W2, (double)weights[i]);
    int env_enc = 0;
    if (const char *ev = getenv("M6A_ENCODER")) {
        if (!*ev || !strcmp(ev, "auto") || !strcmp(ev, "reference")) env_enc = 0;
        else if (!strcmp(ev, "general16")) env_enc = 1;
        else if (!strcmp(ev, "csite12")) env_enc = 2;
        else if (!strcmp(ev, "walk16")) env_enc = 3;
        else if (!strcmp(ev, "fast")) env_enc = 4;
        else return fail(nullptr, M6A_EINVAL, "M6A_ENCODER=%s: must be auto, reference, general16, csite12, walk16 or fast", ev);
    }
    int ndev = 0;
    if (hipGetDeviceCount(&ndev) != hipSuccess || ndev <= 0) {
        (void)hipGetLastError();
        return fail(nullptr, M6A_ENODEV, "no HIP device visible");
    }
    if (device_id < 0 || device_id >= ndev) return fail(nullptr, M6A_EINVAL, "device_id %d out of range (%d devices)", device_id, ndev);
    m6a_ctx *c = new (std::nothrow) m6a_ctx;
    if (!c) return fail(nullptr, M6A_ENOMEM, "out of host memory");
    c->device = device_id;
#define CRCHK(expr)                                                                                  \
    do {                                                                                             \
        hipError_t e_ = (expr);                                                                      \
        if (e_ != hipSuccess) {                                                                      \
            (void)hipGetLastError();                                                                 \
            fail(nullptr, M6A_EHIP, "%s: %s", #expr, hipGetErrorString(e_));                         \
            m6a_destroy(c);                                                                          \
            return M6A_EHIP;                                                                         \
        }                                                                                            \
    } while (0)
    CRCHK(hipSetDevice(device_id));
    hipDeviceProp_t prop;
    CRCHK(hipGetDeviceProperties(&prop, device_id));
    if (std::strncmp(prop.gcnArchName, "gfx950", 6) != 0) {
        fail(nullptr, M6A_ENODEV, "device %d is %s; this library is built for gfx950 only", device_id, prop.gcnArchName);
        m6a_destroy(c);
        return M6A_ENODEV;
    }
    c->n_cu = prop.multiProcessorCount > 0 ? prop.multiProcessorCount : 256;
    CRCHK(hipStreamCreate(&c->own_stream));
    CRCHK(hipStreamCreateWithFlags(&c->s_prep, hipStreamNonBlocking));
    CRCHK(hipEventCreateWithFlags(&c->ev_main, hipEventDisableTiming));
    CRCHK(hipEventCreateWithFlags(&c->ev_prep, hipEventDisableTiming));
    CRCHK(hipEventCreateWithFlags(&c->ev_ctl, hipEventDisableTiming));
    c->stream = c->own_stream;
    std::vector<float> frag, frag2, w1e;
    build_fragments(weights, frag, frag2, w1e);
    CRCHK(hipMalloc((void **)&c->d_wfrag, frag.size() * sizeof(float)));
    CRCHK(hipMalloc((void **)&c->d_wfrag2, frag2.size() * sizeof(float)));
    CRCHK(hipMalloc((void **)&c->d_w1e, w1e.size() * sizeof(float)));
    CRCHK(hipMemcpy(c->d_wfrag2, frag2.data(), frag2.size() * sizeof(float), hipMemcpyHostToDevice));
    CRCHK(hipMemcpy(c->d_w1e, w1e.data(), w1e.size() * sizeof(float), hipMemcpyHostToDevice));
    CRCHK(hipMalloc((void **)&c->d_emb, 132 * sizeof(float)));
    CRCHK(hipMemcpy(c->d_wfrag, frag.data(), frag.size() * sizeof(float), hipMemcpyHostToDevice));
    CRCHK(hipMemcpy(c->d_emb, weights + O_E, 132 * sizeof(float), hipMemcpyHostToDevice));
    c->b3 = weights[O_B3];
    CRCHK(hipMalloc((void **)&c->d_err, sizeof(int)));
    CRCHK(hipMemset(c->d_err, 0, sizeof(int)));
    CRCHK(hipMalloc((void **)&c->d_minmax, 24));
    CRCHK(hipHostMalloc((void **)&c->h_minmax, 24, hipHostMallocDefault));
    CRCHK(hipHostMalloc((void **)&c->h_err, sizeof(int), hipHostMallocDefault));
    *c->h_err = 0;
    CRCHK(hipMalloc((void **)&c->d_hist, M6A_HIST_BINS * 4));
    CRCHK(hipHostMalloc((void **)&c->h_hist, M6A_HIST_BINS * 4, hipHostMallocDefault));
    CRCHK(hipHostMalloc((void **)&c->h_ctl, kCtlWords * 4, hipHostMallocDefault));
    for (int n = 0; n <= M6A_RTAB_MAX_N; n++) c->rt.slot_of_n[n] = -1;
#undef CRCHK
    c->enc_variant = env_enc;
    const char *w = getenv("M6A_WARMUP");
    if (!(w && w[0] == '0')) {
        try { c->warm = std::thread(warm_default, c); } catch (...) {  }
        if (c->warm.joinable()) {
            static std::once_flag once;
            std::call_once(once, [] { atexit(join_background_setups); });
            std::lock_guard<std::mutex> g(g_live_mu);
            g_live.push_back(c);
        }
    }
    *out = c;
    return M6A_OK;
}

void m6a_destroy(m6a_ctx *c)
{
    if (!c) return;
    settle(c);
    {
        std::lock_guard<std::mutex> g(g_live_mu);
        g_live.erase(std::remove(g_live.begin(), g_live.end(), c), g_live.end());
    }
    (void)hipSetDevice(c->device);
    if (c->stream) (void)hipStreamSynchronize(c->stream);
    for (int k = 0; k < 2; k++) {
        for (auto e : c->prof.start[k]) (void)hipEventDestroy(e);
        for (auto e : c->prof.stop[k]) (void)hipEventDestroy(e);
    }
    for (DevBuf *b : {&c->raw, &c->tab, &c->goff, &c->rp_scratch, &c->off_scratch, &c->start_pos, &c->plan_dev, &c->tab_reg, &c->val_idx, &c->val_y, &c->val_avg, &c->sX, &c->sK, &c->sOff,
                      &c->sP, &c->sSite, &c->sMod}) b->release();
    if (c->prof.d_clk) (void)hipFree(c->prof.d_clk);
    if (c->d_wfrag) (void)hipFree(c->d_wfrag);
    if (c->d_wfrag2) (void)hipFree(c->d_wfrag2);
    if (c->d_w1e) (void)hipFree(c->d_w1e);
    if (c->d_emb) (void)hipFree(c->d_emb);
    if (c->d_err) (void)hipFree(c->d_err);
    if (c->d_minmax) (void)hipFree(c->d_minmax);
    if (c->h_minmax) (void)hipHostFree(c->h_minmax);
    if (c->h_err) (void)hipHostFree(c->h_err);
    if (c->d_hist) (void)hipFree(c->d_hist);
    if (c->h_hist) (void)hipHostFree(c->h_hist);
    if (c->h_ctl) (void)hipHostFree(c->h_ctl);
    for (void *p : c->graveyard) (void)hipFree(p);
    if (c->rt.C) (void)hipFree(c->rt.C);
    if (c->rt.RS) (void)hipFree(c->rt.RS);
    for (DevBuf *b : {&c->ctl_dev, &c->rt_rank, &c->rt_order, &c->sOffChunk, &c->jX, &c->jP, &c->jOff, &c->gSite, &c->gMod, &c->gP, &c->mt_scratch, &c->sSigma, &c->sRepr}) b->release();
    for (auto e : c->job.ev_h2d) (void)hipEventDestroy(e);
    for (auto e : c->job.ev_enc) (void)hipEventDestroy(e);
    release_staging(c);
    comm_release(c);
    if (c->s_prep) (void)hipStreamDestroy(c->s_prep);
    if (c->ev_main) (void)hipEventDestroy(c->ev_main);
    if (c->ev_prep) (void)hipEventDestroy(c->ev_prep);
    if (c->ev_ctl) (void)hipEventDestroy(c->ev_ctl);
    if (c->own_stream) (void)hipStreamDestroy(c->own_stream);
    delete c;
}

int m6a_set_stream(m6a_ctx *c, void *hip_stream)
{
    settle(c);
    if (!c) return M6A_EINVAL;
    if (c->job.open) return job_busy(c);
    c->stream = hip_stream ? (hipStream_t)hip_stream : c->own_stream;
    return M6A_OK;
}

int m6a_set_host_offsets(m6a_ctx *c, const int64_t *off_host)
{
    if (!c) return M6A_EINVAL;
    if (off_host && is_device_ptr(off_host)) return fail(c, M6A_EINVAL, "m6a_set_host_offsets takes a host pointer");
    c->hint_off = off_host;
    return M6A_OK;
}

int m6a_set_job_offset(m6a_ctx *c, int64_t first_site)
{
    if (!c) return M6A_EINVAL;
    if (c->job.open) return job_busy(c);
    if (first_site < 0) return fail(c, M6A_EINVAL, "job offset must be >= 0");
    c->job_offset = first_site;
    return M6A_OK;
}

int m6a_set_encoder_variant(m6a_ctx *c, int mode)
{
    if (!c) return M6A_EINVAL;
    if (mode < 0 || mode > 4)
        return fail(c, M6A_EINVAL, "encoder variant must be 0 (auto: 16-slot), 1 (16-slot), 2 (12-slot), 3 (16-slot, per-lane walk) or 4 (fast: 12-slot where every bag has >= 16 reads)");
    c->enc_variant = mode;
    return M6A_OK;
}

const char *m6a_last_encoder_variant(const m6a_ctx *c) { return c ? c->enc_variant_used : "none"; }
const char *m6a_last_encoder_kernel(const m6a_ctx *c) { return c ? c->enc_kernel_used : "none"; }

int m6a_set_scan_driver(m6a_ctx *c, int mode)
{
    if (!c) return M6A_EINVAL;
    if (mode < 0 || mode > 3) return fail(c, M6A_EINVAL, "scan driver must be 0 (auto), 1 (group), 2 (site) or 3 (index tables)");
    c->scan_driver = mode;
    return M6A_OK;
}

int m6a_set_table_variant(m6a_ctx *c, int mode)
{
    if (!c) return M6A_EINVAL;
    if (mode < 0 || mode > 2) return fail(c, M6A_EINVAL, "table variant must be 0 (auto), 1 (LDS) or 2 (registers)");
    c->table_variant = mode;
    return M6A_OK;
}

int m6a_sync(m6a_ctx *c)
{
    settle(c);
    if (!c) return M6A_EINVAL;
    HIPCHK(c, hipSetDevice(c->device));
    return sync_and_check(c);
}

int m6a_prepare_host_io(m6a_ctx *c)
{
    settle(c);
    if (!c) return M6A_EINVAL;
    HIPCHK(c, hipSetDevice(c->device));
    return ensure_staging(c);
}

int m6a_host_alloc(size_t bytes, void **out)
{
    if (!out) return M6A_EINVAL;
    *out = nullptr;
    if (bytes == 0) return M6A_OK;
    const hipError_t e = hipHostMalloc(out, bytes, hipHostMallocDefault);
    if (e != hipSuccess) { (void)hipGetLastError(); *out = nullptr; return e == hipErrorOutOfMemory ? M6A_ENOMEM : M6A_EHIP; }
    return M6A_OK;
}

int m6a_host_free(void *p)
{
    if (!p) return M6A_OK;
    if (hipHostFree(p) != hipSuccess) { (void)hipGetLastError(); return M6A_EHIP; }
    return M6A_OK;
}

int m6a_encode_reads(m6a_ctx *c, const float *X, const uint8_t *km, const int64_t *off, int64_t S, float *rp)
{
    settle(c);
    HintScope hint_scope(c);
    if (c && c->job.open) return job_busy(c);
    if (!c) return M6A_EINVAL;
    if (S < 0) return fail(c, M6A_EINVAL, "n_sites < 0");
    if (S == 0) return M6A_OK;
    if (!X || !km || !off || !rp) return fail(c, M6A_EINVAL, "null pointer argument");
    HIPCHK(c, hipSetDevice(c->device));
    const bool dev = is_device_ptr(X);
    if (dev != is_device_ptr(km) || dev != is_device_ptr(off) || dev != is_device_ptr(rp))
        return fail(c, M6A_EINVAL, "X, site_kmers, off, read_prob must be all host or all device pointers");
    if (!dev) {
        if (off[0] != 0) return fail(c, M6A_EINVAL, "off[0] must be 0");
        for (int64_t s = 0; s < S; s++) if (off[s + 1] < off[s]) return fail(c, M6A_EINVAL, "off[] must be non-decreasing");
        const int64_t R = off[S];
        if (R == 0) return M6A_OK;
        host_bag_range(c, off, S);
        Prefault pf_rp;
        pf_rp.start(rp, (size_t)R * 4, 2);
        int rc = staged_encode(c, X, km, off, S, R, rp);
        if (rc) return rc;
        return sync_and_check(c);
    }
    int rc = bag_stats(c, off, S);
    if (rc) return rc;
    return launch_encode(c, X, km, off, S, c->n_reads, rp);
}

int m6a_read_representation(m6a_ctx *c, const float *X, const uint8_t *km, const int64_t *off, int64_t S, float *repr, float *rp)
{
    return m6a_read_representation_dtype(c, X, km, off, S, repr, M6A_REPR_F32, rp);
}

int m6a_read_representation_dtype(m6a_ctx *c, const float *X, const uint8_t *km, const int64_t *off, int64_t S, void *repr, int dtype, float *rp)
{
    settle(c);
    HintScope hint_scope(c);
    if (c && c->job.open) return job_busy(c);
    if (!c) return M6A_EINVAL;
    if (dtype != M6A_REPR_F32 && dtype != M6A_REPR_F16) return fail(c, M6A_EINVAL, "dtype %d is neither M6A_REPR_F32 nor M6A_REPR_F16", dtype);
    const size_t row_bytes = dtype == M6A_REPR_F16 ? M6A_N_REPR * 2 : M6A_N_REPR * 4;
    if (S < 0) return fail(c, M6A_EINVAL, "n_sites < 0");
    if (!repr) return fail(c, M6A_EINVAL, "repr is NULL: m6a_encode_reads is the call without the representation");
    if (S == 0) return M6A_OK;
    if (!X || !km || !off) return fail(c, M6A_EINVAL, "null pointer argument");
    HIPCHK(c, hipSetDevice(c->device));
    const bool dev = is_device_ptr(X);
    if (dev != is_device_ptr(km) || dev != is_device_ptr(off) || dev != is_device_ptr(repr) || (rp && dev != is_device_ptr(rp)))
        return fail(c, M6A_EINVAL, "X, site_kmers, off, repr, read_prob must be all host or all device pointers");
    if (dev) {
        if ((uintptr_t)repr & 15) return fail(c, M6A_EINVAL, "repr must be 16-byte aligned in device memory");
        int rc = bag_stats(c, off, S);
        if (rc) return rc;
        return launch_repr(c, X, km, off, S, c->n_reads, repr, dtype, rp);
    }
    if (off[0] != 0) return fail(c, M6A_EINVAL, "off[0] must be 0");
    for (int64_t s = 0; s < S; s++) if (off[s + 1] < off[s]) return fail(c, M6A_EINVAL, "off[] must be non-decreasing");
    const int64_t R = off[S];
    if (R == 0) return M6A_OK;
    const int64_t chunk_reads = (int64_t)1 << 20;
    std::vector<int64_t> cs{0};
    int64_t widest = 0;
    while (cs.back() < S) {
        const int64_t s0 = cs.back();
        int64_t s1 = std::upper_bound(off + s0, off + S + 1, off[s0] + chunk_reads) - off - 1;
        s1 = std::min<int64_t>(S, std::max<int64_t>(s1, s0 + 1));
        widest = std::max(widest, off[s1] - off[s0]);
        cs.push_back(s1);
    }
    const int64_t nchunk = (int64_t)cs.size() - 1;
    HIPCHK(c, c->sX.ensure((size_t)widest * 9 * 4));
    HIPCHK(c, c->sK.ensure((size_t)S * 3));
    HIPCHK(c, c->sOff.ensure((size_t)(S + 1) * 8));
    HIPCHK(c, c->sOffChunk.ensure((size_t)(S + nchunk) * 8));
    HIPCHK(c, c->sRepr.ensure((size_t)widest * row_bytes));
    if (rp) HIPCHK(c, c->sP.ensure((size_t)widest * 4));
    HIPCHK(c, hipMemcpyAsync(c->sK.p, km, (size_t)S * 3, hipMemcpyHostToDevice, c->stream));
    HIPCHK(c, hipMemcpyAsync(c->sOff.p, off, (size_t)(S + 1) * 8, hipMemcpyHostToDevice, c->stream));
    for (int64_t k = 0; k < nchunk; k++) {
        const int64_t s0 = cs[k], s1 = cs[k + 1], r0 = off[s0], nr = off[s1] - r0;
        if (nr == 0) continue;
        HIPCHK(c, hipMemcpyAsync(c->sX.p, X + r0 * 9, (size_t)nr * 9 * 4, hipMemcpyHostToDevice, c->stream));
        int64_t *d_off = (int64_t *)c->sOffChunk.p + s0 + k;
        hipLaunchKernelGGL(rebase_off_kernel, dim3((unsigned)((s1 - s0 + 1 + 255) / 256)), dim3(256), 0, c->stream,
                           (const int64_t *)c->sOff.p + s0, s1 - s0 + 1, d_off);
        int rc = launch_repr(c, (const float *)c->sX.p, (const uint8_t *)c->sK.p + s0 * 3, d_off, s1 - s0, nr, c->sRepr.p, dtype,
                             rp ? (float *)c->sP.p : nullptr);
        if (rc) return rc;
        HIPCHK(c, hipMemcpyAsync((char *)repr + (size_t)r0 * row_bytes, c->sRepr.p, (size_t)nr * row_bytes, hipMemcpyDeviceToHost, c->stream));
        if (rp) HIPCHK(c, hipMemcpyAsync(rp + r0, c->sP.p, (size_t)nr * 4, hipMemcpyDeviceToHost, c->stream));
        HIPCHK(c, hipStreamSynchronize(c->stream));
    }
    return sync_and_check(c);
}

int m6a_site_pool(m6a_ctx *c, const float *rp, const int64_t *off, int64_t S, int T, int K, float thr,
                  uint32_t seed, int rng_mode, int64_t bs, int64_t spb, float *site, double *mod)
{
    settle(c);
    HintScope hint_scope(c);
    if (c && c->job.open) return job_busy(c);
    int rc = check_pool_args(c, S, T, K, rng_mode, bs, spb);
    if (rc) return rc;
    if (S == 0) return M6A_OK;
    if (!rp || !off || !site || !mod) return fail(c, M6A_EINVAL, "null pointer argument");
    HIPCHK(c, hipSetDevice(c->device));
    const bool dev = is_device_ptr(rp);
    if (dev != is_device_ptr(off) || dev != is_device_ptr(site) || dev != is_device_ptr(mod))
        return fail(c, M6A_EINVAL, "read_prob, off, site_prob, mod_ratio must be all host or all device pointers");
    if (dev) {
        rc = bag_stats(c, off, S);
        if (rc) return rc;
        return launch_pool(c, rp, off, S, T, K, thr, seed, bs, spb, site, mod);
    }
    if (off[0] != 0) return fail(c, M6A_EINVAL, "off[0] must be 0");
    for (int64_t s = 0; s < S; s++) if (off[s + 1] < off[s]) return fail(c, M6A_EINVAL, "off[] must be non-decreasing");
    const int64_t R = off[S];
    HIPCHK(c, c->sP.ensure((size_t)std::max<int64_t>(R, 1) * 4));
    HIPCHK(c, c->sOff.ensure((size_t)(S + 1) * 8));
    HIPCHK(c, c->sSite.ensure((size_t)S * 4));
    HIPCHK(c, c->sMod.ensure((size_t)S * 8));
    HIPCHK(c, hipMemcpyAsync(c->sP.p, rp, (size_t)R * 4, hipMemcpyHostToDevice, c->stream));
    HIPCHK(c, hipMemcpyAsync(c->sOff.p, off, (size_t)(S + 1) * 8, hipMemcpyHostToDevice, c->stream));
    host_bag_range(c, off, S);
    rc = launch_pool(c, (const float *)c->sP.p, (const int64_t *)c->sOff.p, S, T, K, thr, seed, bs, spb,
                     (float *)c->sSite.p, (double *)c->sMod.p);
    if (rc) return rc;
    HIPCHK(c, hipMemcpyAsync(site, c->sSite.p, (size_t)S * 4, hipMemcpyDeviceToHost, c->stream));
    HIPCHK(c, hipMemcpyAsync(mod, c->sMod.p, (size_t)S * 8, hipMemcpyDeviceToHost, c->stream));
    return sync_and_check(c);
}

int m6a_set_site_mode(m6a_ctx *c, int mode)
{
    if (!c) return M6A_EINVAL;
    if (mode != M6A_SITE_SAMPLED && mode != M6A_SITE_EXPECTED) {
        settle(c);
        return fail(c, M6A_EINVAL, "site mode must be M6A_SITE_SAMPLED (0) or M6A_SITE_EXPECTED (1), not %d", mode);
    }
    if (mode == M6A_SITE_EXPECTED) c->warm_cancel.store(true, std::memory_order_relaxed);
    settle(c);
    if (c->job.open) return job_busy(c);
    c->site_mode = mode;
    return M6A_OK;
}

int m6a_site_expectation(m6a_ctx *c, const float *rp, const int64_t *off, int64_t S, int K, float thr,
                         float *site, double *mod, double *sigma)
{
    settle(c);
    HintScope hint_scope(c);
    if (c && c->job.open) return job_busy(c);
    int rc = check_pool_args(c, S, 1, K, M6A_RNG_NUMPY, 1, 1);
    if (rc) return rc;
    if (S == 0) return M6A_OK;
    if (!rp || !off || !site || !mod) return fail(c, M6A_EINVAL, "null pointer argument");
    HIPCHK(c, hipSetDevice(c->device));
    const bool dev = is_device_ptr(rp);
    if (dev != is_device_ptr(off) || dev != is_device_ptr(site) || dev != is_device_ptr(mod) || (sigma && dev != is_device_ptr(sigma)))
        return fail(c, M6A_EINVAL, "read_prob, off, site_prob, mod_ratio, mc_sigma must be all host or all device pointers");
    if (dev) {
        rc = bag_stats(c, off, S);
        if (rc) return rc;
        if (c->bag_min < 0 || c->bag_max > 0x7fffffff) return fail(c, M6A_EINVAL, "off[] is not a non-decreasing CSR array");
        return launch_expect(c, rp, off, S, K, thr, c->bag_min, c->bag_max, site, mod, sigma);
    }
    if (off[0] != 0) return fail(c, M6A_EINVAL, "off[0] must be 0");
    for (int64_t s = 0; s < S; s++) if (off[s + 1] < off[s]) return fail(c, M6A_EINVAL, "off[] must be non-decreasing");
    const int64_t R = off[S];
    HIPCHK(c, c->sP.ensure((size_t)std::max<int64_t>(R, 1) * 4));
    HIPCHK(c, c->sOff.ensure((size_t)(S + 1) * 8));
    HIPCHK(c, c->sSite.ensure((size_t)S * 4));
    HIPCHK(c, c->sMod.ensure((size_t)S * 8));
    if (sigma) HIPCHK(c, c->sSigma.ensure((size_t)S * 8));
    HIPCHK(c, hipMemcpyAsync(c->sP.p, rp, (size_t)R * 4, hipMemcpyHostToDevice, c->stream));
    HIPCHK(c, hipMemcpyAsync(c->sOff.p, off, (size_t)(S + 1) * 8, hipMemcpyHostToDevice, c->stream));
    host_bag_range(c, off, S);
    if (c->bag_max > 0x7fffffff) return fail(c, M6A_EINVAL, "a bag of more than 2^31 reads");
    rc = launch_expect(c, (const float *)c->sP.p, (const int64_t *)c->sOff.p, S, K, thr, c->bag_min, c->bag_max,
                       (float *)c->sSite.p, (double *)c->sMod.p, sigma ? (double *)c->sSigma.p : nullptr);
    if (rc) return rc;
    HIPCHK(c, hipMemcpyAsync(site, c->sSite.p, (size_t)S * 4, hipMemcpyDeviceToHost, c->stream));
    HIPCHK(c, hipMemcpyAsync(mod, c->sMod.p, (size_t)S * 8, hipMemcpyDeviceToHost, c->stream));
    if (sigma) HIPCHK(c, hipMemcpyAsync(sigma, c->sSigma.p, (size_t)S * 8, hipMemcpyDeviceToHost, c->stream));
    return sync_and_check(c);
}

int m6a_infer(m6a_ctx *c, const float *X, const uint8_t *km, const int64_t *off, int64_t S, int T, int K,
              float thr, uint32_t seed, int rng_mode, int64_t bs, int64_t spb, float *rp, float *site, double *mod)
{
    settle(c);
    HintScope hint_scope(c);
    if (c && c->job.open) return job_busy(c);
    int rc = check_pool_args(c, S, T, K, rng_mode, bs, spb);
    if (rc) return rc;
    if (S == 0) return M6A_OK;
    if (!X || !km || !off || !site || !mod) return fail(c, M6A_EINVAL, "null pointer argument");
    HIPCHK(c, hipSetDevice(c->device));
    const bool dev = is_device_ptr(X);
    if (dev != is_device_ptr(km) || dev != is_device_ptr(off) || dev != is_device_ptr(site) ||
        dev != is_device_ptr(mod) || (rp && dev != is_device_ptr(rp)))
        return fail(c, M6A_EINVAL, "all data pointers must be host pointers or all device pointers");
    if (dev) {
        rc = bag_stats(c, off, S);
        if (rc) return rc;
        const int64_t R = c->n_reads;
        float *p = rp;
        if (!p) { HIPCHK(c, c->rp_scratch.ensure((size_t)std::max<int64_t>(R, 1) * 4)); p = (float *)c->rp_scratch.p; }
        HIPCHK(c, hipEventRecord(c->ev_main, c->stream));
        rc = launch_encode(c, X, km, off, S, R, p);
        if (rc) return rc;
        hipStream_t st = c->s_prep ? c->s_prep : c->stream;
        if (st != c->stream) HIPCHK(c, hipStreamWaitEvent(st, c->ev_main, 0));
        PoolPlan plan;
        rc = pool_plan(c, st, off, S, T, K, seed, bs, spb, &plan);
        if (rc) return rc;
        if (st != c->stream) {
            HIPCHK(c, hipEventRecord(c->ev_prep, st));
            HIPCHK(c, hipStreamWaitEvent(c->stream, c->ev_prep, 0));
        }
        return pool_run(c, plan, p, thr, site, mod);
    }
    if (off[0] != 0) return fail(c, M6A_EINVAL, "off[0] must be 0");
    for (int64_t s = 0; s < S; s++) if (off[s + 1] < off[s]) return fail(c, M6A_EINVAL, "off[] must be non-decreasing");
    const int64_t R = off[S];
    HIPCHK(c, c->sSite.ensure((size_t)S * 4));
    HIPCHK(c, c->sMod.ensure((size_t)S * 8));
    host_bag_range(c, off, S);
    Prefault pf_rp, pf_out;
    if (rp) pf_rp.start(rp, (size_t)R * 4, 2);
    pf_out.start(mod, (size_t)S * 8, 1);
    rc = staged_encode(c, X, km, off, S, R, rp);
    if (rc) return rc;
    rc = launch_pool(c, (const float *)c->sP.p, (const int64_t *)c->sOff.p, S, T, K, thr, seed, bs, spb,
                     (float *)c->sSite.p, (double *)c->sMod.p);
    if (rc) return rc;
    return staged_outputs(c, S, site, mod);
}

int m6a_bag_forward(m6a_ctx *c, const float *X, const uint8_t *km, int64_t B, int bag, float *site)
{
    settle(c);
    HintScope hint_scope(c);
    if (c && c->job.open) return job_busy(c);
    if (!c) return M6A_EINVAL;
    if (B < 0 || bag < 1) return fail(c, M6A_EINVAL, "n_bags must be >= 0 and bag >= 1");
    if (B == 0) return M6A_OK;
    if (!X || !km || !site) return fail(c, M6A_EINVAL, "null pointer argument");
    HIPCHK(c, hipSetDevice(c->device));
    const bool dev = is_device_ptr(X);
    if (dev != is_device_ptr(km) || dev != is_device_ptr(site))
        return fail(c, M6A_EINVAL, "X, site_kmers, site_prob must be all host or all device pointers");
    const int64_t R = B * bag;
    HIPCHK(c, c->off_scratch.ensure((size_t)(B + 1) * 8));
    HIPCHK(c, c->rp_scratch.ensure((size_t)R * 4));
    int64_t *d_off = (int64_t *)c->off_scratch.p;
    float *d_p = (float *)c->rp_scratch.p;
    hipLaunchKernelGGL(iota_off_kernel, dim3((unsigned)((B + 1 + 255) / 256)), dim3(256), 0, c->stream, d_off, B + 1, (int64_t)bag);
    HIPCHK(c, hipGetLastError());
    const float *dX = X; const uint8_t *dK = km; float *dS = site;
    if (!dev) {
        HIPCHK(c, c->sX.ensure((size_t)R * 9 * 4));
        HIPCHK(c, c->sK.ensure((size_t)B * 3));
        HIPCHK(c, c->sSite.ensure((size_t)B * 4));
        HIPCHK(c, hipMemcpyAsync(c->sX.p, X, (size_t)R * 9 * 4, hipMemcpyHostToDevice, c->stream));
        HIPCHK(c, hipMemcpyAsync(c->sK.p, km, (size_t)B * 3, hipMemcpyHostToDevice, c->stream));
        dX = (const float *)c->sX.p; dK = (const uint8_t *)c->sK.p; dS = (float *)c->sSite.p;
    }
    c->bag_min = c->bag_max = bag; c->n_reads = R;
    int rc = launch_encode(c, dX, dK, d_off, B, R, d_p);
    if (rc) return rc;
    hipLaunchKernelGGL(bag_noisy_or_kernel, dim3((unsigned)((B + 255) / 256)), dim3(256), 0, c->stream, d_p, B, bag, dS);
    HIPCHK(c, hipGetLastError());
    if (!dev) {
        HIPCHK(c, hipMemcpyAsync(site, dS, (size_t)B * 4, hipMemcpyDeviceToHost, c->stream));
        HIPCHK(c, hipStreamSynchronize(c->stream));
    }
    return M6A_OK;
}

int64_t m6a_flush_groups(int64_t S, int64_t bs, int64_t spb, int64_t *group_off, int64_t cap)
{
    if (S < 0 || bs < 1 || spb < 1 || !group_off) return M6A_EINVAL;
    std::vector<int64_t> g;
    const int64_t G = flush_groups(S, bs, spb, 0, g);
    if (cap < G + 1) return M6A_EINVAL;
    std::copy(g.begin(), g.end(), group_off);
    return G;
}

int64_t m6a_reference_written_sites(int64_t S, int64_t bs, int64_t spb)
{
    if (S < 0 || bs < 1 || spb < 1) return M6A_EINVAL;
    const int64_t nb = (S + bs - 1) / bs;
    for (int64_t b = nb - 1; b >= 0; b--)
        if ((b + 1) % spb) return std::min((b + 1) * bs, S);
    return 0;
}

int m6a_shard_plan(const int64_t *off, int64_t S, int64_t bs, int64_t spb, int n_shards, int64_t *shard_off)
{
    if (!off || !shard_off || S < 0 || n_shards < 1 || bs < 1 || spb < 1) return M6A_EINVAL;
    std::vector<int64_t> g;
    const int64_t G = flush_groups(S, bs, spb, 0, g);
    const int64_t R = S > 0 ? off[S] : 0;
    shard_off[0] = 0;
    int64_t gi = 0;
    for (int k = 1; k <= n_shards; k++) {
        if (k == n_shards) { shard_off[k] = S; break; }
        const double target = (double)R * k / n_shards;
        while (gi < G && (double)off[g[gi]] < target) gi++;
        if (gi > 0 && gi <= G) {
            const double hi = (double)off[g[std::min(gi, G)]], lo = (double)off[g[gi - 1]];
            if (target - lo < hi - target && g[gi - 1] >= shard_off[k - 1]) gi--;
        }
        shard_off[k] = std::max(g[std::min(gi, G)], shard_off[k - 1]);
    }
    return M6A_OK;
}

int m6a_random_stream(m6a_ctx *c, uint32_t seed, int64_t n_words, uint32_t *words)
{
    settle(c);
    if (!c) return M6A_EINVAL;
    if (n_words < 0 || n_words > ((int64_t)1 << 31) - 2048) return fail(c, M6A_EINVAL, "n_words out of range");
    if (n_words == 0) return M6A_OK;
    if (!words) return fail(c, M6A_EINVAL, "null pointer argument");
    HIPCHK(c, hipSetDevice(c->device));
    if (is_device_ptr(words)) return launch_stream(c, c->stream, seed, n_words, words);
    HIPCHK(c, c->val_idx.ensure((size_t)n_words * 4));
    int rc = launch_stream(c, c->stream, seed, n_words, (uint32_t *)c->val_idx.p);
    if (rc) return rc;
    rc = d2h_through_ring(c, words, c->val_idx.p, (size_t)n_words * 4);
    if (rc) return rc;
    return sync_and_check(c);
}

int m6a_device_count(void)
{
    int n = 0;
    if (hipGetDeviceCount(&n) != hipSuccess) { (void)hipGetLastError(); return 0; }
    return n;
}

int m6a_profile_enable(m6a_ctx *c, int on)
{
    if (!c) return M6A_EINVAL;
    if (on && !c->prof.d_clk) {
        HIPCHK(c, hipSetDevice(c->device));
        HIPCHK(c, hipMalloc((void **)&c->prof.d_clk, (size_t)2 * M6A_CLK_SLOTS * 4 * sizeof(unsigned long long)));
    }
    if (on) HIPCHK(c, hipMemsetAsync(c->prof.d_clk, 0, (size_t)2 * M6A_CLK_SLOTS * 4 * sizeof(unsigned long long), c->stream));
    c->prof.on = on != 0;
    c->prof.mask = on == 2 ? 1 : on == 3 ? 2 : 3;
    c->prof.used[0] = c->prof.used[1] = 0;
    c->prof.dropped[0] = c->prof.dropped[1] = 0;
    return M6A_OK;
}

int m6a_profile_read(m6a_ctx *c, int kind, double *total_ms, int64_t *n_launches)
{
    settle(c);
    if (!c || kind < 0 || kind > 1 || !total_ms || !n_launches) return M6A_EINVAL;
    HIPCHK(c, hipSetDevice(c->device));
    HIPCHK(c, hipStreamSynchronize(c->stream));
    double tot = 0;
    for (int i = 0; i < c->prof.used[kind]; i++) {
        float ms = 0;
        HIPCHK(c, hipEventElapsedTime(&ms, c->prof.start[kind][i], c->prof.stop[kind][i]));
        tot += ms;
    }
    *total_ms = tot;
    *n_launches = c->prof.used[kind];
    return M6A_OK;
}

int m6a_profile_clock(m6a_ctx *c, int kind, double *ghz_median, double *ghz_min, double *ghz_max, double *span_ms, int *n_waves)
{
    settle(c);
    if (!c || kind < 0 || kind > 1) return M6A_EINVAL;
    if (!c->prof.d_clk) return fail(c, M6A_EINVAL, "m6a_profile_clock: profiling was never enabled on this context");
    HIPCHK(c, hipSetDevice(c->device));
    HIPCHK(c, hipStreamSynchronize(c->stream));
    unsigned long long h[M6A_CLK_SLOTS * 4];
    HIPCHK(c, hipMemcpy(h, c->prof.d_clk + (size_t)kind * M6A_CLK_SLOTS * 4, sizeof h, hipMemcpyDeviceToHost));
    std::vector<double> ghz;
    unsigned long long r_first = ~0ull, r_last = 0;
    for (int i = 0; i < M6A_CLK_SLOTS; i++) {
        const unsigned long long c0 = h[4 * i], r0 = h[4 * i + 1], c1 = h[4 * i + 2], r1 = h[4 * i + 3];
        if (!r0 || r1 <= r0 || c1 <= c0) continue;
        ghz.push_back((double)(c1 - c0) / (double)(r1 - r0) * 0.1);
        r_first = std::min(r_first, r0);
        r_last = std::max(r_last, r1);
    }
    std::sort(ghz.begin(), ghz.end());
    const bool any = !ghz.empty();
    if (ghz_median) *ghz_median = any ? ghz[ghz.size() / 2] : 0.0;
    if (ghz_min) *ghz_min = any ? ghz.front() : 0.0;
    if (ghz_max) *ghz_max = any ? ghz.back() : 0.0;
    if (span_ms) *span_ms = any ? (double)(r_last - r_first) * 1e-5 : 0.0;
    if (n_waves) *n_waves = (int)ghz.size();
    return M6A_OK;
}

const char *m6a_last_pool_variant(const m6a_ctx *c) { return c ? c->pool_variant : "none"; }

}
```

m6anet_amd/csrc/m6a_ctx.h:

```cpp
#pragma once
#include <hip/hip_runtime.h>
#include <dlfcn.h>
#include <sys/mman.h>

#include <algorithm>
#include <atomic>
#include <cmath>
#include <cstdarg>
#include <cstdio>
#include <cstdlib>
#include <cstring>
#include <condition_variable>
#include <functional>
#include <memory>
#include <mutex>
#include <new>
#include <string>
#include <thread>
#include <vector>

#include "m6a.h"
#include "m6a_kernels.h"
#include "m6a_host_cpus.h"




struct DevBuf {
    void *p = nullptr;
    size_t cap = 0;
    hipError_t ensure(size_t bytes)
    {
        if (bytes <= cap) return hipSuccess;
        if (p) (void)hipFree(p);
        p = nullptr; cap = 0;
        size_t want = bytes + bytes / 8 + 256;
        hipError_t e = hipMalloc(&p, want);
        if (e == hipSuccess) cap = want;
        return e;
    }
    void release() { if (p) (void)hipFree(p); p = nullptr; cap = 0; }
};

constexpr int kMaxProfiled = 8192;

struct Profiler {
    unsigned long long *d_clk = nullptr;
    unsigned long long *clk_for(int kind) const { return on && (mask >> kind & 1) ? d_clk + (size_t)kind * M6A_CLK_SLOTS * 4 : nullptr; }
    bool on = false;
    int mask = 3;
    std::vector<hipEvent_t> start[2], stop[2];
    int used[2] = {0, 0};
    int64_t dropped[2] = {0, 0};
};


class CopyPool {
public:
    explicit CopyPool(int n_threads)
    {
        for (int i = 0; i < n_threads; i++) workers_.emplace_back([this] { loop(); });
    }
    ~CopyPool()
    {
        { std::lock_guard<std::mutex> g(mu_); stop_ = true; }
        cv_job_.notify_all();
        for (auto &t : workers_) t.join();
    }
    void copy(void *dst, const void *src, size_t n)
    {
        const size_t parts = std::max<size_t>(1, std::min<size_t>(workers_.size() + 1, n / ((size_t)256 << 10)));
        if (parts == 1) { std::memcpy(dst, src, n); return; }
        const size_t slice = ((n + parts - 1) / parts + 4095) & ~(size_t)4095;
        {
            std::lock_guard<std::mutex> g(mu_);
            dst_ = (char *)dst; src_ = (const char *)src; n_ = n; slice_ = slice; next_ = 0; pending_ = (n + slice - 1) / slice;
        }
        cv_job_.notify_all();
        work();
        std::unique_lock<std::mutex> g(mu_);
        cv_done_.wait(g, [this] { return pending_ == 0; });
    }

private:
    bool work()
    {
        bool any = false;
        for (;;) {
            size_t off;
            {
                std::lock_guard<std::mutex> g(mu_);
                if (next_ * slice_ >= n_) return any;
                off = next_++ * slice_;
            }
            std::memcpy(dst_ + off, src_ + off, std::min(slice_, n_ - off));
            any = true;
            std::lock_guard<std::mutex> g(mu_);
            if (--pending_ == 0) cv_done_.notify_all();
        }
    }
    void loop()
    {
        for (;;) {
            {
                std::unique_lock<std::mutex> g(mu_);
                cv_job_.wait(g, [this] { return stop_ || next_ * slice_ < n_; });
                if (stop_) return;
            }
            work();
        }
    }
    std::vector<std::thread> workers_;
    std::mutex mu_;
    std::condition_variable cv_job_, cv_done_;
    char *dst_ = nullptr; const char *src_ = nullptr;
    size_t n_ = 0, slice_ = 1, next_ = 0, pending_ = 0;
    bool stop_ = false;
};

class Prefault {
public:
    Prefault() = default;
    void start(void *p, size_t bytes, int n_threads)
    {
        if (!p || bytes < ((size_t)4 << 20)) return;
        char *b = (char *)p;
        const size_t page = 4096;
        const size_t first = (page - ((uintptr_t)b & (page - 1))) & (page - 1);
        if (first >= bytes) return;
        const size_t n_pages = (bytes - first) / page;
        for (int t = 0; t < n_threads; t++)
            th_.emplace_back([=] {
                const size_t p0 = n_pages * (size_t)t / (size_t)n_threads, p1 = n_pages * (size_t)(t + 1) / (size_t)n_threads;
                char *lo = b + first + p0 * page, *hi = b + first + p1 * page;
                bool populate = true;
                for (char *q = lo; q < hi;) {
                    const size_t len = std::min<size_t>((size_t)2 << 20, (size_t)(hi - q));
                    if (populate && madvise(q, len, 23 ) != 0) populate = false;
                    if (!populate)
                        for (size_t o = 0; o < len; o += page) __atomic_fetch_add(q + o, (char)0, __ATOMIC_RELAXED);
                    q += len;
                }
            });
    }
    void join() { for (auto &t : th_) t.join(); th_.clear(); }
    ~Prefault() { join(); }
private:
    std::vector<std::thread> th_;
};

constexpr int kStageSlots = 3;
struct Staging {
    hipStream_t s_h2d = nullptr, s_d2h = nullptr;
    char *pin_in[kStageSlots] = {nullptr, nullptr, nullptr};
    char *pin_out[kStageSlots] = {nullptr, nullptr, nullptr};
    hipEvent_t ev_h2d[kStageSlots] = {nullptr, nullptr, nullptr}, ev_enc[kStageSlots] = {nullptr, nullptr, nullptr},
               ev_d2h[kStageSlots] = {nullptr, nullptr, nullptr};
    int64_t chunk_reads = 0;
    std::unique_ptr<CopyPool> pool;
    bool ready = false;
};

struct MeanPlan {
    int T = 0;
    std::vector<int> leaf_start;
    std::vector<uint8_t> merge_after;
    std::vector<uint32_t> row_meta;
    std::vector<int> row_pass, row_round;
    std::vector<uint32_t> reg_ctl;
    int n_rem = 0;
    int depth = 1;
    int max_merge = 0;
};

struct m6a_ctx {
    int device = 0;
    int n_cu = 256;
    hipStream_t own_stream = nullptr;
    hipStream_t stream = nullptr;
    std::string err;
    float *d_wfrag = nullptr, *d_wfrag2 = nullptr, *d_w1e = nullptr, *d_emb = nullptr;
    float b3 = 0.f;
    DevBuf raw, tab, tab_reg, goff, rp_scratch, off_scratch, start_pos, plan_dev;
    MeanPlan plan; size_t plan_off[4] = {0, 0, 0, 0};
    uint32_t raw_seed = 0; int64_t raw_len = 0;
    struct { uint32_t seed; int n, T, K, jmax; bool valid; } tab_key = {0, 0, 0, 0, 0, false}, tab_reg_key = {0, 0, 0, 0, 0, false};
    int table_variant = 0;
    struct { int64_t S, bs, spb, base, G, gmax; bool valid; } goff_key = {0, 0, 0, 0, 0, 0, false};
    int64_t job_offset = 0;
    int64_t bag_min = 0, bag_max = 0, n_reads = 0;
    int enc_variant = 0;
    const char *enc_variant_used = "none";
    const char *enc_kernel_used = "none";
    int scan_driver = 0;
    int *d_err = nullptr;
    unsigned long long *d_minmax = nullptr;
    unsigned long long *h_minmax = nullptr;
    int *h_err = nullptr;
    uint32_t *h_hist = nullptr, *d_hist = nullptr;
    std::vector<uint32_t> hist_part;
    uint32_t *h_ctl = nullptr;
    DevBuf ctl_dev, rt_rank, rt_order;
    bool side_work = false;
    const int64_t *hint_off = nullptr;
    hipEvent_t ev_ctl = nullptr;
    hipStream_t s_prep = nullptr;
    hipEvent_t ev_main = nullptr, ev_prep = nullptr;
    struct {
        bool valid = false; uint32_t seed = 0; int64_t A = 0, n_blk = 0;
        int cap = 0, used = 0;
        uint16_t *C = nullptr; uint32_t *RS = nullptr;
        int32_t slot_of_n[M6A_RTAB_MAX_N + 1];
    } rt;
    DevBuf sX, sK, sOff, sP, sSite, sMod, val_idx, val_y, val_avg, sOffChunk;
    Staging stg;
    std::vector<void *> graveyard;
    int rt_presize = 0;
    uint32_t rt_credit_seed = 0; int64_t rt_credit_A = 0, rt_credit = 0;
    struct Job {
        bool open = false;
        int failed = 0;
        std::string failed_msg;
        int T = 0, K = 0; float thr = 0.f; uint32_t seed = 0; int64_t bs = 1, spb = 1;
        std::vector<int64_t> off;
        int64_t S = 0, R = 0;
        int n_sub = 0; size_t sub_bytes = 0, o_goff = 0, o_km = 0, o_x = 0;
        int64_t cap_sites = 0, cap_reads = 0;
        std::vector<char *> pin;
        std::vector<hipEvent_t> ev_h2d, ev_enc;
        std::vector<char> used;
        int64_t item = 0;
        int64_t fill_sites = 0, fill_reads = 0, fill_min = INT64_MAX;
        bool cur_ready = false;
        int64_t chunks = 0;
    } job;
    DevBuf gSite, gMod, gP;
    DevBuf jX, jP, jOff;
    DevBuf mt_scratch; int64_t mt_polys_G = 0;
    std::vector<int> iter_of;
    std::thread warm;
    void *comm = nullptr;
    int comm_rank = 0, comm_world = 0;
    Profiler prof;
    const char *pool_variant = "none";
    int site_mode = M6A_SITE_SAMPLED;
    std::atomic<bool> warm_cancel{false};
    DevBuf sSigma;
    DevBuf sRepr;
};

namespace m6a_detail {

int fail(m6a_ctx *c, int code, const char *fmt, ...);

#define HIPCHK(c, expr)                                                                    \
    do {                                                                                   \
        hipError_t e_ = (expr);                                                            \
        if (e_ != hipSuccess) {                                                            \
            (void)hipGetLastError();                                                       \
            return fail((c), e_ == hipErrorOutOfMemory ? M6A_ENOMEM : M6A_EHIP, "%s: %s (%s:%d)", \
                        #expr, hipGetErrorString(e_), __FILE__, __LINE__);                 \
        }                                                                                  \
    } while (0)

bool is_device_ptr(const void *p);
inline void settle(m6a_ctx *c) { if (c && c->warm.joinable()) c->warm.join(); }
int job_busy(m6a_ctx *c);
int check_pool_args(m6a_ctx *c, int64_t S, int T, int K, int rng_mode, int64_t bs, int64_t spb);
int deferred_error(m6a_ctx *c);
int sync_and_check(m6a_ctx *c);
struct HintScope {
    m6a_ctx *c;
    explicit HintScope(m6a_ctx *ctx) : c(ctx) {}
    ~HintScope() { if (c) c->hint_off = nullptr; }
};
int launch_encode(m6a_ctx *c, const float *X, const uint8_t *km, const int64_t *off, int64_t S, int64_t R, float *rp);
int launch_repr(m6a_ctx *c, const float *X, const uint8_t *km, const int64_t *off, int64_t S, int64_t R, void *repr, int dtype, float *rp);
int repr_writer_begin(m6a_ctx *c, int device, hipStream_t *stream);
int repr_writer_round(m6a_ctx *c, const float *X, const uint8_t *km, const int64_t *off, int64_t *off_round, int64_t s0, int64_t s1,
                      int64_t r0, int64_t nr, void *repr, int dtype);
int launch_pool(m6a_ctx *c, const float *rp, const int64_t *off, int64_t S, int T, int K, float thr, uint32_t seed, int64_t bs, int64_t spb,
                float *site, double *mod);
int bag_stats(m6a_ctx *c, const int64_t *d_off, int64_t S);
void host_bag_range(m6a_ctx *c, const int64_t *off, int64_t S);
void prof_begin(m6a_ctx *c, int kind);
void prof_end(m6a_ctx *c, int kind);
int ensure_staging(m6a_ctx *c);
void release_staging(m6a_ctx *c);
int staged_encode(m6a_ctx *c, const float *X, const uint8_t *km, const int64_t *off, int64_t S, int64_t R, float *rp_host);
int staged_outputs(m6a_ctx *c, int64_t S, float *site, double *mod);
int d2h_through_ring(m6a_ctx *c, void *host, const void *dev, size_t bytes);
bool base_is_group_start(int64_t base, int64_t bs, int64_t spb);
void comm_release(m6a_ctx *c);

}
```

m6anet_amd/csrc/m6a_kernels.h:

```cpp
#ifndef M6A_KERNELS_H
#define M6A_KERNELS_H
#include <hip/hip_runtime.h>
#include <stdint.h>

#define M6A_BAG_LDS 1024
#define M6A_WFRAG_FLOATS (136 * 64)
#define M6A_WFRAG2_FLOATS (25 * 64)
#define M6A_W1E_FLOATS (35 * 32)
#define M6A_BN_FLOATS (5 * 2 * 16 * 2)
#define M6A_MEAN_STACK 32
#define M6A_CSITE_MIN_BAG 16
#define M6A_TABLE_MAX_N 32
#define M6A_REG_STACK 8
#define M6A_RTAB_MAX_N 4096
#define M6A_RTAB_SMALL_N 1024
#define M6A_RTAB_U8_MAX_N 256
#define M6A_HIST_BINS (M6A_RTAB_MAX_N + 2)

__host__ __device__ inline unsigned long long m6a_bin_weight(int i)
{
    unsigned long long z = (unsigned long long)(i + 1) * 0x9E3779B97F4A7C15ull;
    z = (z ^ (z >> 30)) * 0xBF58476D1CE4E5B9ull;
    z = (z ^ (z >> 27)) * 0x94D049BB133111EBull;
    return z ^ (z >> 31);
}

#define M6A_CLK_SLOTS 64
__device__ __forceinline__ void m6a_clk_stamp(unsigned long long *clk, int which)
{
    if (!clk) return;
    const unsigned stride = (gridDim.x >> 6) | 1u, b = blockIdx.x;
    if (threadIdx.x == 0 && b % stride == 0 && b / stride < M6A_CLK_SLOTS) {
        unsigned long long *p = clk + (size_t)(b / stride) * 4 + which * 2;
        p[0] = __builtin_amdgcn_s_memtime();
        p[1] = __builtin_amdgcn_s_memrealtime();
    }
}

struct EncArgs {
    const float *X;
    const uint8_t *site_kmers;
    const int64_t *off;
    const float *wfrag;
    const float *wfrag2;
    const float *w1e_tab;
    const float *bn;
    const float *emb;
    float *read_prob;
    int *err;
    int64_t n_sites, n_reads, n_tiles, tiles_per_wave;
    float b3;
    unsigned long long *clk;
};

struct EncReprArgs {
    EncArgs enc;
    void *repr;
};

struct PoolArgs {
    const float *read_prob;
    const int64_t *off;
    const int64_t *goff;
    const uint32_t *raw;
    const uint32_t *tab;
    float *site_prob;
    double *mod_ratio;
    uint32_t *start_pos;
    const int *leaf_start;
    const uint8_t *merge_after;
    const uint32_t *row_meta;
    int n_leaves, n_rows, n_rem;
    int stack_depth;
    const uint32_t *reg_ctl;
    int reg_rounds, reg_final_merges;
    int64_t reg_items;
    int *err;
    int64_t n_groups, n_sites, raw_len;
    int T, K, uniform_n, jmax, bag_cap;
    float thr;
    unsigned long long *clk;
};

struct ExpectArgs {
    const float *read_prob;
    const int64_t *off;
    float *site_prob;
    double *mod_ratio;
    double *mc_sigma;
    int64_t n_sites;
    int K, uniform_n;
    float thr;
};

struct RtabBuild {
    const uint32_t *raw;
    uint32_t n_blk;
    const int32_t *build_n;
    const int32_t *build_slot;
    int n_build;
    uint16_t *C;
    uint32_t *RS;
    int64_t c_stride;
};
struct RtabUse {
    const uint16_t *C;
    const uint32_t *RS;
    const int32_t *slot_of_n;
    uint32_t *rank;
    const uint32_t *order;
    int64_t c_stride;
    uint32_t n_blk;
    int bag_cap;
    uint32_t si_base, si_count;
};

__global__ void enc_kernel(EncArgs a);
__global__ void enc_site16_kernel(EncArgs a);
__global__ void enc_csite_kernel(EncArgs a);
template <bool F16> __global__ void enc_repr_kernel(EncReprArgs ra);
__global__ void pool_scan_start_kernel(PoolArgs a);
template <int KT> __global__ void pool_scan_group_kernel(PoolArgs a);
template <int KT> __global__ void pool_scan_site_kernel(PoolArgs a);
__global__ void pool_table_kernel(PoolArgs a);
__global__ void pool_reg_kernel(PoolArgs a);
__global__ void bag_noisy_or_kernel(const float *read_prob, int64_t n_bags, int bag, float *site_prob);
__global__ void iota_off_kernel(int64_t *off, int64_t n_plus_1, int64_t step);
__global__ void rebase_off_kernel(const int64_t *off, int64_t count, int64_t *out);
__global__ void sampled_noisy_or_kernel(const float *read_prob, const int32_t *gidx, int64_t n_bags, int k, float *y);
__global__ void mean_over_passes_kernel(const float *y, int n_iters, int64_t n_sites, float *avg);
__global__ void pairwise_mean_kernel(const float *y, int n_iters, float *avg);
__global__ void bag_minmax_kernel(const int64_t *off, int64_t n_sites, unsigned long long *out, uint32_t *hist);
__global__ void bag_verify_kernel(const unsigned long long *got, const uint32_t *hist, unsigned long long mn, unsigned long long mx,
                                  unsigned long long reads, unsigned long long hash, int *err);
__global__ void mt19937_kernel(uint32_t seed, int64_t n_words, uint32_t *raw, const uint32_t *hist, int64_t seg_words, uint32_t *xhead, int64_t xhead_n);
__global__ void mt_jump_kernel(const uint32_t *xhead, const uint64_t *polys, uint32_t *hist);
__global__ void rtab_count_kernel(RtabBuild a);
__global__ void rtab_scan_kernel(RtabBuild a);
__global__ void rtab_fill_kernel(RtabBuild a);
__global__ void rtab_to_reg_table_kernel(const uint16_t *C, int64_t A, int64_t row_words, int jmax, uint16_t *tab);
__global__ void rtab_to_lds_table_kernel(const uint16_t *C, int64_t A, int K, int rows, int jmax, const int *iter_of, uint32_t *tab);
__global__ void rtab_prep_kernel(PoolArgs a, RtabUse u, uint32_t *cursor, uint32_t *order, unsigned n_order_blocks);
template <int KT> __global__ void pool_rtab_kernel(PoolArgs a, RtabUse u);
__global__ void site_expect_wave_kernel(ExpectArgs a);
template <bool VEC4> __global__ void site_expect_lane_kernel(ExpectArgs a);

__global__ void m6a_touch_kernels();
__global__ void m6a_touch_pool_reg();
__global__ void m6a_touch_pool_rtab();
__global__ void m6a_touch_expect();

#endif
```

m6anet_amd/csrc/m6a_kernels.hip:

```cpp
#include <hip/hip_runtime.h>
#include <stdint.h>

#include "m6a_kernels.h"

typedef float f32x16 __attribute__((ext_vector_type(16)));
typedef float f32x2 __attribute__((ext_vector_type(2)));

__device__ __forceinline__ float chain8_sum(float r)
{
    r += __builtin_bit_cast(float, __builtin_amdgcn_update_dpp(0, __builtin_bit_cast(int, r), 0xB1, 0xf, 0xf, false));
    r += __builtin_bit_cast(float, __builtin_amdgcn_update_dpp(0, __builtin_bit_cast(int, r), 0x4E, 0xf, 0xf, false));
    r += __builtin_bit_cast(float, __builtin_amdgcn_update_dpp(0, __builtin_bit_cast(int, r), 0x141, 0xf, 0xf, false));
    return r;
}

__device__ __forceinline__ int wave_sum_i32(int v)
{
#pragma unroll
    for (int m = 1; m < 64; m <<= 1) v += __shfl_xor(v, m, 64);
    return v;
}

#define L2_REGS(m) ((m) == 4 ? 12 : 16)

// ... 874 lines not shown
                                                 __builtin_amdgcn_mbcnt_lo((uint32_t)bal, 0));
                                const unsigned long long lastb = __ballot(ok && rank == A - acc - 1);
                                pos += 64 * i + (uint32_t)__builtin_ctzll(lastb) + 1;
                                found = true;
                            } else {
                                acc += c;
                            }
                        }
                        break;
                    }
                    acc += tot;
                }
                pos += STEP;
#pragma unroll
                for (int i = 0; i < M6A_SCAN_A_LOADS; i++) w[i] = wn[i];
            }
        }
    }
}

#define M6A_TAB_RC 16
#define M6A_TAB_REG_STACK 8
__global__ __launch_bounds__(256) __attribute__((amdgpu_waves_per_eu(5, 5))) void pool_table_kernel(PoolArgs a)
{
    __shared__ __attribute__((aligned(16))) uint32_t s_idx[M6A_TAB_RC * 5 * 64];
    __shared__ __attribute__((aligned(16))) uint32_t s_meta[M6A_TAB_RC * 4];
    __shared__ __attribute__((aligned(256))) float s_bag[4 * 528];
    extern __shared__ __attribute__((aligned(16))) float s_mean[];
    const int lane = threadIdx.x & 63;
    const int wib = __builtin_amdgcn_readfirstlane((int)(threadIdx.x >> 6));
    float *bag = s_bag + wib * 64;
    const char *bagb = (const char *)bag;
    const int depth = a.stack_depth;
    float *w_stage = s_mean + wib * (128 + 8 * depth);
    float *w_rem = w_stage + 64;
    float *w_stack = w_rem + 64 + (lane & 7) * depth;
    const int n = a.uniform_n;
    const int rows = a.n_rows;
    const int n_chunks = (rows + M6A_TAB_RC - 1) / M6A_TAB_RC;
    const int j = (int)(blockIdx.x % (unsigned)a.jmax);
    const int64_t c = blockIdx.x / (unsigned)a.jmax;
    const int64_t nbj = gridDim.x / (unsigned)a.jmax;
    const int64_t gblocks = (a.n_groups + 7) >> 3;
    const int64_t stride = nbj * 4;
    const int64_t n_iter = (gblocks + stride - 1) / stride;
    const uint32_t *row = a.tab + (int64_t)j * rows * 5 * 64;

    if (n_chunks == 1) {
        for (int i = threadIdx.x; i < rows * 5 * 64; i += 256) s_idx[i] = row[i];
        if ((int)threadIdx.x < rows * 4) s_meta[threadIdx.x] = a.row_meta[threadIdx.x];
        __syncthreads();
    }
    for (int64_t it = 0; it < n_iter; ++it) {
        const int64_t gb = c * 4 + wib + it * stride;
        const bool active = gb < gblocks;
        int64_t site[8];
        float sum[8];
#pragma unroll
        for (int q = 0; q < 8; q++) { site[q] = -1; sum[q] = 0.0f; }
        if (active) {
#pragma unroll
            for (int q = 0; q < 8; q++) {
                const int64_t g = gb * 8 + q;
                if (g < a.n_groups) {
                    const int64_t s = a.goff[g] + j;
                    if (s < a.goff[g + 1]) site[q] = s;
                }
                float v = 0.0f;
                bool ge = false;
                if (site[q] >= 0 && lane < n) {
                    v = a.read_prob[a.off[site[q]] + lane];
                    ge = v >= a.thr;
                }
                const int cge = __popcll(__ballot(ge));
                if (lane < 32) bag[(q >> 1) * 528 + 2 * lane + (q & 1)] = 1.0f - v;
                if (lane == 0 && site[q] >= 0) a.mod_ratio[site[q]] = (double)cge / (double)n;
            }
            wave_lds_fence();
        }
        int sp = 0;
        float st[M6A_TAB_REG_STACK];
#pragma unroll
        for (int d = 0; d < M6A_TAB_REG_STACK; d++) st[d] = 0.0f;
        for (int ch = 0; ch < n_chunks; ++ch) {
            const int rd0 = ch * M6A_TAB_RC;
            const int nr = rows - rd0 < M6A_TAB_RC ? rows - rd0 : M6A_TAB_RC;
            if (n_chunks > 1) {
                __syncthreads();
                for (int i = threadIdx.x; i < nr * 5 * 64; i += 256) s_idx[i] = row[rd0 * 5 * 64 + i];
                if ((int)threadIdx.x < nr * 4) s_meta[threadIdx.x] = a.row_meta[rd0 * 4 + threadIdx.x];
                __syncthreads();
            }
            if (!active) continue;
            for (int rd = 0; rd < nr; ++rd) {
                float2 prod[4];
#pragma unroll
                for (int pr = 0; pr < 4; pr++) prod[pr] = make_float2(1.0f, 1.0f);
                const uint32_t *ixp = s_idx + rd * 5 * 64 + lane;
                const uint4 mt = *(const uint4 *)(s_meta + rd * 4);
#pragma unroll 1
                for (int pl = 0; pl < 5; pl++) {
                    const uint32_t ixw = ixp[pl * 64];
                    float2 g[4][4];
#pragma unroll
                    for (int bb = 0; bb < 4; bb++) {
                        const uint32_t o = (ixw >> (8 * bb)) & 0xffu;
#pragma unroll
                        for (int pr = 0; pr < 4; pr++) g[bb][pr] = *(const float2 *)(bagb + pr * 2112 + o);
                    }
#pragma unroll
                    for (int bb = 0; bb < 4; bb++)
#pragma unroll
                        for (int pr = 0; pr < 4; pr++) {
                            prod[pr].x *= g[bb][pr].x;
                            prod[pr].y *= g[bb][pr].y;
                        }
                    __builtin_amdgcn_sched_group_barrier(0x002, 4, 0);
                    __builtin_amdgcn_sched_group_barrier(0x100, 16, 0);
                    __builtin_amdgcn_sched_group_barrier(0x002, 16, 0);
                }
                const uint32_t flags = (uint32_t)__builtin_amdgcn_readfirstlane((int)mt.x);
                const uint64_t lmask = ((uint64_t)(uint32_t)__builtin_amdgcn_readfirstlane((int)mt.z) << 32) |
                                       (uint32_t)__builtin_amdgcn_readfirstlane((int)mt.y);
                if (flags & (1u << 25)) {
                    if (lane < 8) {
#pragma unroll
                        for (int pr = 0; pr < 4; pr++) {
                            w_rem[(2 * pr) * 8 + lane] = 1.0f - prod[pr].x;
                            w_rem[(2 * pr + 1) * 8 + lane] = 1.0f - prod[pr].y;
                        }
                    }
                    continue;
                }
                const bool live = (lmask >> lane) & 1;
#pragma unroll
                for (int pr = 0; pr < 4; pr++) {
                    sum[2 * pr] += live ? 1.0f - prod[pr].x : 0.0f;
                    sum[2 * pr + 1] += live ? 1.0f - prod[pr].y : 0.0f;
                }
                if (!(flags & (1u << 24))) continue;
#pragma unroll
                for (int q = 0; q < 8; q++) {
                    const float sv = chain8_sum(sum[q]);
                    if ((lane & 7) == 0) w_stage[q * 8 + (lane >> 3)] = sv;
                    sum[q] = 0.0f;
                }
                wave_lds_fence();
                if (lane < 8) {
                    const uint32_t mc = (uint32_t)__builtin_amdgcn_readfirstlane((int)mt.w);
                    const int nl = (int)((flags >> 26) & 0xfu);
                    const bool final_pass = flags & (1u << 30);
                    if (depth <= M6A_TAB_REG_STACK) {
                        float xs[8], tl[7];
#pragma unroll
                        for (int bl = 0; bl < 8; bl++) xs[bl] = w_stage[lane * 8 + bl];
#pragma unroll
                        for (int i = 0; i < 7; i++) tl[i] = w_rem[lane * 8 + i];
#pragma unroll
                        for (int bl = 0; bl < 8; bl++) {
                            if (bl >= nl) break;
                            float x = xs[bl];
                            if (final_pass && bl == nl - 1) {
#pragma unroll
                                for (int i = 0; i < 7; i++)
                                    if (i < a.n_rem) x += tl[i];
                            }
                            for (int m = (int)((mc >> (4 * bl)) & 15u); m > 0; --m) {
                                --sp;
                                float top = st[0];
#pragma unroll
                                for (int d = 1; d < M6A_TAB_REG_STACK; d++) top = sp == d ? st[d] : top;
                                x = top + x;
                            }
#pragma unroll
                            for (int d = 0; d < M6A_TAB_REG_STACK; d++) st[d] = sp == d ? x : st[d];
                            ++sp;
                        }
                    } else {
                        for (int bl = 0; bl < nl; bl++) {
                            float x = w_stage[lane * 8 + bl];
                            if (final_pass && bl == nl - 1)
                                for (int i = 0; i < a.n_rem; i++) x += w_rem[lane * 8 + i];
                            for (int m = (int)((mc >> (4 * bl)) & 15u); m > 0; --m) x = w_stack[--sp] + x;
                            w_stack[sp++] = x;
                        }
                    }
                }
                wave_lds_fence();
            }
        }
        if (active) {
            float tot = 0.0f;
            if (lane < 8) tot = (depth <= M6A_TAB_REG_STACK ? st[0] : w_stack[0]) / (float)a.T;
#pragma unroll
            for (int q = 0; q < 8; q++)
                if (lane == q && site[q] >= 0) a.site_prob[site[q]] = tot;
            wave_lds_fence();
        }
    }
}

__global__ void bag_noisy_or_kernel(const float *read_prob, int64_t n_bags, int bag, float *site_prob)
{
    const int64_t b = (int64_t)blockIdx.x * blockDim.x + threadIdx.x;
    if (b >= n_bags) return;
    float prod = 1.0f;
    for (int k = 0; k < bag; k++) prod *= 1.0f - read_prob[b * bag + k];
    site_prob[b] = 1.0f - prod;
}

__global__ void sampled_noisy_or_kernel(const float *read_prob, const int32_t *gidx, int64_t n_bags, int k, float *y)
{
    const int64_t b = (int64_t)blockIdx.x * blockDim.x + threadIdx.x;
    if (b >= n_bags) return;
    const int32_t *row = gidx + b * k;
    float prod = 1.0f;
    if (k == 20) {
        int4 q[5];
#pragma unroll
        for (int j = 0; j < 5; j++) q[j] = ((const int4 *)row)[j];
        float g[20];
#pragma unroll
        for (int j = 0; j < 5; j++) {
            g[4 * j] = read_prob[q[j].x]; g[4 * j + 1] = read_prob[q[j].y];
            g[4 * j + 2] = read_prob[q[j].z]; g[4 * j + 3] = read_prob[q[j].w];
        }
#pragma unroll
        for (int j = 0; j < 20; j++) prod *= 1.0f - g[j];
    } else {
        for (int j = 0; j < k; j++) prod *= 1.0f - read_prob[row[j]];
    }
    y[b] = 1.0f - prod;
}

__global__ void mean_over_passes_kernel(const float *y, int n_iters, int64_t n_sites, float *avg)
{
    const int64_t s = (int64_t)blockIdx.x * blockDim.x + threadIdx.x;
    if (s >= n_sites) return;
    float acc = 0.0f;
    for (int t = 0; t < n_iters; t++) acc += y[(int64_t)t * n_sites + s];
    avg[s] = acc / (float)n_iters;
}

__device__ static float pairwise_leaf(const float *a, int64_t n)
{
    if (n < 8) {
        float res = 0.0f;
        for (int64_t i = 0; i < n; i++) res += a[i];
        return res;
    }
    float r[8];
    for (int k = 0; k < 8; k++) r[k] = a[k];
    int64_t i = 8;
    for (; i < n - (n % 8); i += 8)
        for (int k = 0; k < 8; k++) r[k] += a[i + k];
    float res = ((r[0] + r[1]) + (r[2] + r[3])) + ((r[4] + r[5]) + (r[6] + r[7]));
    for (; i < n; i++) res += a[i];
    return res;
}

__global__ void pairwise_mean_kernel(const float *y, int n_iters, float *avg)
{
    if (blockIdx.x != 0 || threadIdx.x != 0) return;
    struct Frame { int64_t off, n; float left; bool right; };
    Frame st[32];
    int sp = 0;
    st[0] = {0, n_iters, 0.0f, false};
    float sum;
    for (;;) {
        Frame &f = st[sp];
        if (f.n > 128) {
            const int64_t n2 = (f.n / 2) - (f.n / 2) % 8;
            st[++sp] = {f.off, n2, 0.0f, false};
            continue;
        }
        sum = pairwise_leaf(y + f.off, f.n);
        for (;;) {
            if (sp == 0) { avg[0] = sum / (float)n_iters; return; }
            Frame &p = st[--sp];
            const int64_t n2 = (p.n / 2) - (p.n / 2) % 8;
            if (!p.right) {
                p.left = sum;
                p.right = true;
                st[++sp] = {p.off + n2, p.n - n2, 0.0f, false};
                break;
            }
            sum = p.left + sum;
        }
    }
}

__global__ void rebase_off_kernel(const int64_t *off, int64_t count, int64_t *out)
{
    const int64_t i = (int64_t)blockIdx.x * blockDim.x + threadIdx.x;
    if (i < count) out[i] = off[i] - off[0];
}

__global__ void iota_off_kernel(int64_t *off, int64_t n_plus_1, int64_t step)
{
    const int64_t i = (int64_t)blockIdx.x * blockDim.x + threadIdx.x;
    if (i < n_plus_1) off[i] = i * step;
}

__global__ __launch_bounds__(256) void bag_minmax_kernel(const int64_t *off, int64_t n_sites, unsigned long long *out, uint32_t *hist)
{
    __shared__ int64_t s_mn[4], s_mx[4];
    __shared__ uint32_t s_hist[M6A_HIST_BINS];
    for (int i = threadIdx.x; i < M6A_HIST_BINS; i += 256) s_hist[i] = 0;
    __syncthreads();
    int64_t mn = INT64_MAX, mx = 0;
    for (int64_t s = (int64_t)blockIdx.x * blockDim.x + threadIdx.x; s < n_sites;
         s += (int64_t)gridDim.x * blockDim.x) {
        const int64_t n = off[s + 1] - off[s];
        mn = n < mn ? n : mn;
        mx = n > mx ? n : mx;
        atomicAdd(&s_hist[n < 0 ? 0 : n > M6A_RTAB_MAX_N ? M6A_RTAB_MAX_N + 1 : n], 1u);
    }
#pragma unroll
    for (int m = 1; m < 64; m <<= 1) {
        const int64_t omn = __shfl_xor(mn, m, 64), omx = __shfl_xor(mx, m, 64);
        mn = omn < mn ? omn : mn;
        mx = omx > mx ? omx : mx;
    }
    if ((threadIdx.x & 63) == 0) { s_mn[threadIdx.x >> 6] = mn; s_mx[threadIdx.x >> 6] = mx; }
    __syncthreads();
    for (int i = threadIdx.x; i < M6A_HIST_BINS; i += 256)
        if (s_hist[i]) atomicAdd(&hist[i], s_hist[i]);
    if (threadIdx.x == 0) {
        for (int w = 1; w < 4; w++) { mn = s_mn[w] < mn ? s_mn[w] : mn; mx = s_mx[w] > mx ? s_mx[w] : mx; }
        atomicMin(&out[0], (unsigned long long)mn);
        atomicMax(&out[1], (unsigned long long)mx);
        if (blockIdx.x == 0) out[2] = (unsigned long long)off[n_sites];
    }
}

__global__ __launch_bounds__(256) void bag_verify_kernel(const unsigned long long *got, const uint32_t *hist, unsigned long long mn,
                                                         unsigned long long mx, unsigned long long reads, unsigned long long hash, int *err)
{
    __shared__ unsigned long long s_part[256];
    unsigned long long h = 0;
    for (int i = threadIdx.x; i < M6A_HIST_BINS; i += 256) h += (unsigned long long)hist[i] * m6a_bin_weight(i);
    s_part[threadIdx.x] = h;
    __syncthreads();
    if (threadIdx.x == 0) {
        for (int i = 1; i < 256; i++) h += s_part[i];
        if (got[0] != mn || got[1] != mx || got[2] != reads || h != hash) atomicExch(err, 3);
    }
}

__global__ void m6a_touch_kernels() {}
```

m6anet_amd/engine.py:

```python
import ctypes as C

import numpy as np

from . import _lib
from .constants import (DEFAULT_PRETRAINED_MODEL, DEFAULT_READ_THRESHOLD, N_REPR, N_SAMPLES, N_WEIGHT_FLOATS,
                        PRETRAINED_CONFIGS, asset_path)


def load_weights(pretrained_model=DEFAULT_PRETRAINED_MODEL):
    if pretrained_model not in PRETRAINED_CONFIGS:
        raise ValueError("Invalid pretrained model {}, must be one of {}".format(
            pretrained_model, list(PRETRAINED_CONFIGS)))
    w = np.fromfile(asset_path(PRETRAINED_CONFIGS[pretrained_model][0]), np.float32)
    assert w.size == N_WEIGHT_FLOATS
    return w


def weights_from_state_dict(sd):
    order = ["read_level_encoder.1.embedding_layer.weight", "read_level_encoder.3.layers.0.weight",
             "read_level_encoder.3.layers.0.bias", "read_level_encoder.3.layers.1.weight",
             "read_level_encoder.3.layers.1.bias", "read_level_encoder.3.layers.1.running_mean",
             "read_level_encoder.3.layers.1.running_var", "read_level_encoder.4.layers.0.weight",
             "read_level_encoder.4.layers.0.bias", "pooling_filter.probability_layer.0.weight",
             "pooling_filter.probability_layer.0.bias"]
    w = np.concatenate([np.asarray(sd[k].detach().cpu().numpy() if hasattr(sd[k], "detach") else sd[k],
                                   np.float32).ravel() for k in order])
    if w.size != N_WEIGHT_FLOATS:
        raise ValueError("state_dict does not have the m6anet.toml topology (%d floats)" % w.size)
    return w


STATE_DICT_KEYS = [("read_level_encoder.1.embedding_layer.weight", (66, 2)), ("read_level_encoder.3.layers.0.weight", (150, 15)),
                   ("read_level_encoder.3.layers.0.bias", (150,)), ("read_level_encoder.3.layers.1.weight", (150,)),
                   ("read_level_encoder.3.layers.1.bias", (150,)), ("read_level_encoder.3.layers.1.running_mean", (150,)),
                   ("read_level_encoder.3.layers.1.running_var", (150,)), ("read_level_encoder.4.layers.0.weight", (32, 150)),
                   ("read_level_encoder.4.layers.0.bias", (32,)), ("pooling_filter.probability_layer.0.weight", (1, 32)),
                   ("pooling_filter.probability_layer.0.bias", (1,))]


def state_dict_from_weights(w, num_batches_tracked=0):
    w = np.ascontiguousarray(w, np.float32)
    if w.size != N_WEIGHT_FLOATS:
        raise ValueError("weights must have %d floats" % N_WEIGHT_FLOATS)
    sd, o = {}, 0
    for key, shape in STATE_DICT_KEYS:
        n = int(np.prod(shape))
        sd[key] = w[o:o + n].reshape(shape).copy()
        o += n
        if key.endswith("running_var"):
            sd[key[:-len("running_var")] + "num_batches_tracked"] = np.array(int(num_batches_tracked), np.int64)
    return sd


def init_weights(seed):
    g = np.random.Generator(np.random.PCG64(int(seed)))
    lin = lambda fan_out, fan_in: (g.uniform(-1, 1, (fan_out, fan_in)) / np.sqrt(fan_in), g.uniform(-1, 1, fan_out) / np.sqrt(fan_in))
    E = g.standard_normal((66, 2))
    W1, b1 = lin(150, 15)
    W2, b2 = lin(32, 150)
    W3, b3 = lin(1, 32)
    parts = [E, W1, b1, np.ones(150), np.zeros(150), np.zeros(150), np.ones(150), W2, b2, W3, b3]
    return np.concatenate([np.asarray(p, np.float64).ravel() for p in parts]).astype(np.float32)


_libc = None


def _hint_huge_pages(a):
    global _libc
    if a.nbytes < (8 << 20):
        return
    try:
        if _libc is None:
            _libc = C.CDLL(None, use_errno=True)
            _libc.madvise.argtypes = [C.c_void_p, C.c_size_t, C.c_int]
        lo = (a.ctypes.data + (1 << 21) - 1) & ~((1 << 21) - 1)
        hi = (a.ctypes.data + a.nbytes) & ~((1 << 21) - 1)
        if hi > lo:
            _libc.madvise(lo, hi - lo, 14)
    except Exception:
        pass


def _is_torch(x):
    return type(x).__module__.startswith("torch")


def pinned_empty(shape, dtype=np.float32):
    import weakref
    L = _lib.load()
    dt = np.dtype(dtype)
    n = int(np.prod(shape)) * dt.itemsize
    p = C.c_void_p()
    rc = L.m6a_host_alloc(max(n, 1), C.byref(p))
    if rc != 0:
        raise _lib.M6AError(rc, "m6a_host_alloc(%d bytes)" % n)
    buf = (C.c_char * max(n, 1)).from_address(p.value)
    weakref.finalize(buf, L.m6a_host_free, C.c_void_p(p.value))
    return np.frombuffer(buf, dtype=dt, count=int(np.prod(shape))).reshape(shape)


class _Arg:

    def __init__(self, x, dtype, torch_dtype_name):
        self.is_dev = False
        if _is_torch(x):
            import torch
            want = getattr(torch, torch_dtype_name)
            if x.dtype != want or not x.is_contiguous():
                raise TypeError("tensor must be contiguous %s" % torch_dtype_name)
            self.keep = x
            self.ptr = x.data_ptr()
            self.is_dev = x.is_cuda
            self.size = x.numel()
        else:
            a = np.ascontiguousarray(x, dtype)
            self.keep = a
            self.ptr = a.ctypes.data
            self.size = a.size


class M6ANetEngine:
    def __init__(self, weights=None, pretrained_model=DEFAULT_PRETRAINED_MODEL, device=0):
        self._L = _lib.load()
        if weights is None:
            weights = load_weights(pretrained_model)
        w = np.ascontiguousarray(weights, np.float32)
        if w.size != N_WEIGHT_FLOATS:
            raise ValueError("weights must have %d floats" % N_WEIGHT_FLOATS)
        if isinstance(device, str):
            device = int(device.split(":")[1]) if ":" in device else 0
        self.device = int(device)
        h = C.c_void_p()
        rc = self._L.m6a_create(C.byref(h), w.ctypes.data, w.size, self.device)
        if rc != 0:
            raise _lib.M6AError(rc, self._L.m6a_last_error(None).decode())
        self._h = h

    def close(self):
        if getattr(self, "_h", None):
            self._L.m6a_destroy(self._h)
            self._h = None

    def __del__(self):
        try:
            self.close()
        except Exception:
            pass

    def _chk(self, rc):
        if rc != 0:
            raise _lib.M6AError(rc, self._L.m6a_last_error(self._h).decode())

    def set_stream(self, stream_handle):
        self._chk(self._L.m6a_set_stream(self._h, C.c_void_p(stream_handle or 0)))
        self._torch_stream = None

    def use_torch_stream(self):
        import torch
        st = torch.cuda.current_stream(self.device)
        self.set_stream(st.cuda_stream)
        self._torch_stream = st.cuda_stream

    def set_job_offset(self, first_site):
        self._chk(self._L.m6a_set_job_offset(self._h, int(first_site)))

    def set_encoder_variant(self, mode):
        self._chk(self._L.m6a_set_encoder_variant(self._h, int(mode)))

    @property
    def last_encoder_variant(self):
        return self._L.m6a_last_encoder_variant(self._h).decode()

    @property
    def last_encoder_kernel(self):
        return self._L.m6a_last_encoder_kernel(self._h).decode()

    def set_scan_driver(self, mode):
        self._chk(self._L.m6a_set_scan_driver(self._h, int(mode)))

    def set_table_variant(self, mode):
        self._chk(self._L.m6a_set_table_variant(self._h, int(mode)))

    def sync(self):
        self._chk(self._L.m6a_sync(self._h))

    def set_host_offsets(self, off_host):
        if off_host is None:
            self._chk(self._L.m6a_set_host_offsets(self._h, None))
            return
        a = np.ascontiguousarray(off_host, dtype=np.int64)
        self._host_off_keepalive = a
        self._chk(self._L.m6a_set_host_offsets(self._h, a.ctypes.data))

    def comm_init(self, unique_id, rank, world_size):
        buf = (C.c_char * 128).from_buffer_copy(bytes(unique_id))
        self._chk(self._L.m6a_comm_init(self._h, buf, int(rank), int(world_size)))
        self._comm = (int(rank), int(world_size))

    def comm_info(self):
        n, r, d, v = C.c_int(0), C.c_int(-1), C.c_int(-1), C.c_int(0)
        self._chk(self._L.m6a_comm_count(self._h, C.byref(n)))
        self._chk(self._L.m6a_comm_info(self._h, C.byref(r), C.byref(d), C.byref(v)))
        return {"ranks_seen": n.value, "rank": r.value, "device": d.value, "rccl_version": v.value}

    def comm_destroy(self):
        self._chk(self._L.m6a_comm_destroy(self._h))

    def gather(self, site, mod, cuts, dst=0, out=None):
        rank, world = self._comm
        cuts = np.ascontiguousarray(cuts, np.int64)
        assert cuts.size == world + 1
        aS, aM = _Arg(site, np.float32, "float32"), _Arg(mod, np.float64, "float64")
        total = int(cuts[-1] - cuts[0])
        sa = ma = None
        if rank == dst:
            sa, ma = out if out is not None else (self._out(aS.is_dev, total, np.float32, "float32"),
                                                  self._out(aS.is_dev, total, np.float64, "float64"))
        oS = _Arg(sa, np.float32, "float32") if sa is not None else None
        oM = _Arg(ma, np.float64, "float64") if ma is not None else None
        self._chk(self._L.m6a_gather(self._h, aS.ptr, aM.ptr, cuts.ctypes.data, int(dst),
                                     oS.ptr if oS else None, oM.ptr if oM else None))
        return sa, ma

    def gather_reads(self, read_prob, read_cuts, dst=0, out=None):
        rank, world = self._comm
        cuts = np.ascontiguousarray(read_cuts, np.int64)
        assert cuts.size == world + 1
        aP = _Arg(read_prob, np.float32, "float32")
        ra = None
        if rank == dst:
            ra = out if out is not None else self._out(aP.is_dev, int(cuts[-1] - cuts[0]), np.float32, "float32")
        oP = _Arg(ra, np.float32, "float32") if ra is not None else None
        self._chk(self._L.m6a_gather_reads(self._h, aP.ptr, cuts.ctypes.data, int(dst), oP.ptr if oP else None))
        return ra

    def random_stream(self, seed, n_words):
        out = np.empty(int(n_words), np.uint32)
        self._chk(self._L.m6a_random_stream(self._h, int(seed) & 0xffffffff, int(n_words), out.ctypes.data))
        return out

    def prepare_host_io(self):
        self._chk(self._L.m6a_prepare_host_io(self._h))

    def profile(self, on=True):
        self._chk(self._L.m6a_profile_enable(self._h, {False: 0, True: 1, 'encoder': 2, 'pooling': 3}[on]))

    def profile_read(self, kind):
        ms, n = C.c_double(), C.c_int64()
        self._chk(self._L.m6a_profile_read(self._h, kind, C.byref(ms), C.byref(n)))
        return ms.value, n.value

    def profile_clock(self, kind):
        g, lo, hi, span, n = C.c_double(), C.c_double(), C.c_double(), C.c_double(), C.c_int32()
        self._chk(self._L.m6a_profile_clock(self._h, kind, C.byref(g), C.byref(lo), C.byref(hi), C.byref(span), C.byref(n)))
        if n.value == 0:
            return None
        return {"ghz": g.value, "ghz_min": lo.value, "ghz_max": hi.value, "span_ms": span.value, "waves": n.value}

    @property
    def last_pool_variant(self):
        return self._L.m6a_last_pool_variant(self._h).decode()

    def _out(self, like_dev, n, np_dtype, torch_name):
        if like_dev:
            import torch
            return torch.empty(n, dtype=getattr(torch, torch_name), device="cuda:%d" % self.device)
        a = np.empty(n, np_dtype)
        _hint_huge_pages(a)
        return a

    def get_read_probability(self, X, site_kmers, off, out=None):
        aX, aK, aO = _Arg(X, np.float32, "float32"), _Arg(site_kmers, np.uint8, "uint8"), _Arg(off, np.int64, "int64")
        S = aO.size - 1
        R = aX.size // 9
        if aK.size != 3 * S:
            raise ValueError("site_kmers must be [n_sites, 3]")
        rp = out if out is not None else self._out(aX.is_dev, R, np.float32, "float32")
        aP = _Arg(rp, np.float32, "float32")
        if aP.size != R:
            raise ValueError("read_prob must have one float per read")
        self._chk(self._L.m6a_encode_reads(self._h, aX.ptr, aK.ptr, aO.ptr, S, aP.ptr))
        return rp

    def get_read_representation(self, X, site_kmers, off, out=None, want_read_probs=False, dtype="float32"):
        if dtype not in _lib.REPR_DTYPES:
            raise ValueError("dtype must be 'float32' or 'float16', not %r" % (dtype,))
        np_dt = np.float16 if dtype == "float16" else np.float32
        aX, aK, aO = _Arg(X, np.float32, "float32"), _Arg(site_kmers, np.uint8, "uint8"), _Arg(off, np.int64, "int64")
        S = aO.size - 1
        R = aX.size // 9
        if aK.size != 3 * S:
            raise ValueError("site_kmers must be [n_sites, 3]")
        rep, rp = out if isinstance(out, (tuple, list)) else (out, None)
        if rep is None:
            rep = self._out(aX.is_dev, R * N_REPR, np_dt, dtype).reshape(R, N_REPR)
        if want_read_probs and rp is None:
            rp = self._out(aX.is_dev, R, np.float32, "float32")
        for o, dt, name in ((rep, np_dt, dtype), (rp, np.float32, "float32")):
            if o is not None and not _is_torch(o) and not (isinstance(o, np.ndarray) and o.dtype == dt and o.flags.c_contiguous):
                raise TypeError("out must be C-contiguous %s" % name)
        aH = _Arg(rep, np_dt, dtype)
        aP = _Arg(rp, np.float32, "float32") if rp is not None else None
        if aH.size != R * N_REPR:
            raise ValueError("repr must be [n_reads, %d]" % N_REPR)
        if aP is not None and aP.size != R:
            raise ValueError("read_prob must have one float per read")
        if dtype == "float32":
            self._chk(self._L.m6a_read_representation(self._h, aX.ptr, aK.ptr, aO.ptr, S, aH.ptr, aP.ptr if aP else None))
        else:
            self._chk(self._L.m6a_read_representation_dtype(self._h, aX.ptr, aK.ptr, aO.ptr, S, aH.ptr, _lib.REPR_DTYPES[dtype],
                                                            aP.ptr if aP else None))
        return (rep, rp) if want_read_probs else rep

    def read_representation_ptrs(self, X, site_kmers, off, n_sites, repr, dtype="float32", read_prob=None):
        code = _lib.REPR_DTYPES[dtype] if isinstance(dtype, str) else int(dtype)
        self._chk(self._L.m6a_read_representation_dtype(self._h, X, site_kmers, off, int(n_sites), repr, code, read_prob))

    def calculate_site_proba(self, read_probs, off, n_iters, n_samples=N_SAMPLES,
                             read_proba_threshold=DEFAULT_READ_THRESHOLD, seed=0, batch_size=16,
                             save_per_batch=2):
        aP, aO = _Arg(read_probs, np.float32, "float32"), _Arg(off, np.int64, "int64")
        S = aO.size - 1
        site = self._out(aP.is_dev, S, np.float32, "float32")
        mod = self._out(aP.is_dev, S, np.float64, "float64")
        aS, aM = _Arg(site, np.float32, "float32"), _Arg(mod, np.float64, "float64")
        self._chk(self._L.m6a_site_pool(self._h, aP.ptr, aO.ptr, S, int(n_iters), int(n_samples),
                                        float(np.float32(read_proba_threshold)), int(seed) & 0xffffffff,
                                        _lib.RNG_NUMPY, int(batch_size), int(save_per_batch), aS.ptr, aM.ptr))
        return site, mod

    SITE_MODES = {"sampled": 0, "expected": 1}

    def set_site_mode(self, mode):
        if mode not in self.SITE_MODES:
            raise ValueError("site mode must be 'sampled' or 'expected', not %r" % (mode,))
        self._chk(self._L.m6a_set_site_mode(self._h, self.SITE_MODES[mode]))

    def site_expectation(self, read_probs, off, n_samples=N_SAMPLES, want_sigma=False, read_proba_threshold=DEFAULT_READ_THRESHOLD):
        aP, aO = _Arg(read_probs, np.float32, "float32"), _Arg(off, np.int64, "int64")
        S = aO.size - 1
        site = self._out(aP.is_dev, S, np.float32, "float32")
        mod = self._out(aP.is_dev, S, np.float64, "float64")
        sigma = self._out(aP.is_dev, S, np.float64, "float64") if want_sigma else None
        aS, aM = _Arg(site, np.float32, "float32"), _Arg(mod, np.float64, "float64")
        aG = _Arg(sigma, np.float64, "float64") if want_sigma else None
        self._chk(self._L.m6a_site_expectation(self._h, aP.ptr, aO.ptr, S, int(n_samples), float(np.float32(read_proba_threshold)),
                                               aS.ptr, aM.ptr, aG.ptr if aG else None))
        return (site, mod, sigma) if want_sigma else (site, mod)

    def infer(self, X, site_kmers, off, n_iters, n_samples=N_SAMPLES,
              read_proba_threshold=DEFAULT_READ_THRESHOLD, seed=0, batch_size=16, save_per_batch=2,
              want_read_probs=True, out=None):
        aX, aK, aO = _Arg(X, np.float32, "float32"), _Arg(site_kmers, np.uint8, "uint8"), _Arg(off, np.int64, "int64")
        S = aO.size - 1
        R = aX.size // 9
        if out is not None:
            rp, site, mod = out
        else:
            rp = self._out(aX.is_dev, R, np.float32, "float32") if want_read_probs else None
            site = self._out(aX.is_dev, S, np.float32, "float32")
            mod = self._out(aX.is_dev, S, np.float64, "float64")
        aP = _Arg(rp, np.float32, "float32") if rp is not None else None
        aS, aM = _Arg(site, np.float32, "float32"), _Arg(mod, np.float64, "float64")
        self.infer_ptrs(aX.ptr, aK.ptr, aO.ptr, S, n_iters, n_samples, read_proba_threshold, seed, batch_size, save_per_batch,
                        aP.ptr if aP else None, aS.ptr, aM.ptr)
        return rp, site, mod

    def infer_ptrs(self, X, site_kmers, off, n_sites, n_iters, n_samples=N_SAMPLES, read_proba_threshold=DEFAULT_READ_THRESHOLD,
                   seed=0, batch_size=16, save_per_batch=2, read_prob=None, site_prob=None, mod_ratio=None):
        self._chk(self._L.m6a_infer(self._h, X, site_kmers, off, int(n_sites), int(n_iters), int(n_samples),
                                    float(np.float32(read_proba_threshold)), int(seed) & 0xffffffff,
                                    _lib.RNG_NUMPY, int(batch_size), int(save_per_batch), read_prob, site_prob, mod_ratio))

    def job_begin(self, n_iters, n_samples=N_SAMPLES, read_proba_threshold=DEFAULT_READ_THRESHOLD, seed=0, batch_size=16,
                  save_per_batch=2, expect_sites=0, expect_reads=0):
        self._chk(self._L.m6a_job_begin(self._h, int(n_iters), int(n_samples), float(np.float32(read_proba_threshold)),
                                        int(seed) & 0xffffffff, _lib.RNG_NUMPY, int(batch_size), int(save_per_batch),
                                        int(expect_sites), int(expect_reads)))
        self._job_dev = False
        self._job_keep = []

    def job_feed(self, X, site_kmers, off):
        aX, aK = _Arg(X, np.float32, "float32"), _Arg(site_kmers, np.uint8, "uint8")
        if aX.is_dev or aK.is_dev:
            import torch
            cur = torch.cuda.current_stream(self.device)
            if getattr(self, "_torch_stream", None) != cur.cuda_stream:
                cur.synchronize()
            self._job_keep.append((aX.keep, aK.keep))
        o = off if (isinstance(off, np.ndarray) and off.dtype == np.int64 and off.flags.c_contiguous) else \
            np.ascontiguousarray(off.cpu().numpy() if _is_torch(off) else off, dtype=np.int64)
        n = o.size - 1
        if aK.size != 3 * n or aX.size != 9 * int(o[-1]):
            raise ValueError("batch shapes disagree: X [off[-1], 9], site_kmers [n_sites, 3], off [n_sites + 1]")
        self._job_dev = self._job_dev or aX.is_dev
        self._chk(self._L.m6a_job_feed(self._h, aX.ptr, aK.ptr, o.ctypes.data, n))

    def job_feed_collated(self, features, kmers, n_reads):
        aX, aK, aN = _Arg(features, np.float32, "float32"), _Arg(kmers, np.int64, "int64"), _Arg(n_reads, np.int64, "int64")
        if aX.is_dev or aK.is_dev or aN.is_dev:
            raise TypeError("job_feed_collated takes the collate's host tensors")
        if aK.size * 3 != aX.size:
            raise ValueError("batch shapes disagree: features [r, 9], kmers [r, 3]")
        self._chk(self._L.m6a_job_feed_collated(self._h, aX.ptr, aK.ptr, aN.ptr, aN.size))

    def job_size(self):
        S, R = C.c_int64(), C.c_int64()
        self._chk(self._L.m6a_job_size(self._h, C.byref(S), C.byref(R)))
        return S.value, R.value

    def job_end(self, want_read_probs=True, device_outputs=None):
        S, R = self.job_size()
        dev = self._job_dev if device_outputs is None else bool(device_outputs)
        rp = self._out(dev, R, np.float32, "float32") if want_read_probs else None
        site = self._out(dev, S, np.float32, "float32")
        mod = self._out(dev, S, np.float64, "float64")
        aP = _Arg(rp, np.float32, "float32") if rp is not None else None
        aS, aM = _Arg(site, np.float32, "float32"), _Arg(mod, np.float64, "float64")
        try:
            self._chk(self._L.m6a_job_end(self._h, aP.ptr if aP else None, aS.ptr, aM.ptr))
        finally:
            self._job_keep = []
        return rp, site, mod

    def job_abort(self):
        try:
            self._chk(self._L.m6a_job_abort(self._h))
            self.sync()
        finally:
            self._job_keep = []

    def forward(self, X, kmer, bag=N_SAMPLES):
        aX, aK = _Arg(X, np.float32, "float32"), _Arg(kmer, np.uint8, "uint8")
        B = aK.size // 3
        if aX.size != B * bag * 9:
            raise ValueError("X must be [B, bag, 9]")
        site = self._out(aX.is_dev, B, np.float32, "float32")
        aS = _Arg(site, np.float32, "float32")
        self._chk(self._L.m6a_bag_forward(self._h, aX.ptr, aK.ptr, B, int(bag), aS.ptr))
        return site


    def trainer(self, weights=None, lr=4e-4, betas=(0.9, 0.999), eps=1e-8, weight_decay=0.0, clip_grad=None):
        t = Trainer(self, init_weights(0) if weights is None else weights, lr, betas, eps, weight_decay)
        if clip_grad is not None:
            try:
                t.set_clip(clip_grad)
            except Exception:
                t.close()
                raise
        return t

    def validate_pool(self, read_probs, off, n_iterations=1, n_samples=N_SAMPLES, seed=0):
        aP, aO = _Arg(read_probs, np.float32, "float32"), _Arg(off, np.int64, "int64")
        S = aO.size - 1
        y = self._out(aP.is_dev, int(n_iterations) * S, np.float32, "float32")
        avg = self._out(aP.is_dev, S, np.float32, "float32")
        aY, aA = _Arg(y, np.float32, "float32"), _Arg(avg, np.float32, "float32")
        self._chk(self._L.m6a_validate_pool(self._h, aP.ptr, aO.ptr, S, int(n_iterations), int(n_samples),
                                            int(seed) & 0xffffffff, aY.ptr, aA.ptr))
        return y.reshape(int(n_iterations), S), avg

    def validate_forward(self, X, site_kmers, off, n_iterations=1, n_samples=N_SAMPLES, seed=0, want_read_probs=False):
        aX, aK, aO = _Arg(X, np.float32, "float32"), _Arg(site_kmers, np.uint8, "uint8"), _Arg(off, np.int64, "int64")
        S = aO.size - 1
        R = aX.size // 9
        y = self._out(aX.is_dev, int(n_iterations) * S, np.float32, "float32")
        avg = self._out(aX.is_dev, S, np.float32, "float32")
        rp = self._out(aX.is_dev, R, np.float32, "float32") if want_read_probs else None
        aY, aA = _Arg(y, np.float32, "float32"), _Arg(avg, np.float32, "float32")
        aP = _Arg(rp, np.float32, "float32") if rp is not None else None
        self._chk(self._L.m6a_validate(self._h, aX.ptr, aK.ptr, aO.ptr, S, int(n_iterations), int(n_samples),
                                       int(seed) & 0xffffffff, aP.ptr if aP else None, aY.ptr, aA.ptr))
        y = y.reshape(int(n_iterations), S)
        return (y, avg, rp) if want_read_probs else (y, avg)


class Trainer:

    def __init__(self, engine, weights, lr=4e-4, betas=(0.9, 0.999), eps=1e-8, weight_decay=0.0):
        self._engine, self._L = engine, engine._L
        w = np.ascontiguousarray(weights, np.float32)
        if w.size != N_WEIGHT_FLOATS:
            raise ValueError("weights must have %d floats" % N_WEIGHT_FLOATS)
        cfg = _lib.TrainConfig(float(lr), float(betas[0]), float(betas[1]), float(eps), float(weight_decay))
        h = C.c_void_p()
        engine._chk(self._L.m6a_train_create(engine._h, w.ctypes.data, w.size, C.byref(cfg), C.byref(h)))
        self._h = h

    def close(self):
        if getattr(self, "_h", None) and getattr(self._engine, "_h", None):
            self._L.m6a_train_destroy(self._h)
        self._h = None

    def __del__(self):
# ... 166 lines not shown
```

Measured before the change: 387.2 million.

## Fuse bag min/max and verify kernels and defer the verification off the critical path

Measured after the change: 387.2 million. No clear change (-0.0%).

```diff
diff --git a/include/m6a.h b/include/m6a.h
--- a/include/m6a.h
+++ b/include/m6a.h
@@ -37,6 +37,8 @@
 int m6a_set_job_offset(m6a_ctx *ctx, int64_t first_site);
 int m6a_sync(m6a_ctx *ctx);
 int m6a_set_host_offsets(m6a_ctx *ctx, const int64_t *off_host);
+#define M6A_BAG_HIST_BINS 4098
+int m6a_bag_statistics(m6a_ctx *ctx, const int64_t *off_dev, int64_t n_sites, int64_t *stats, uint32_t *hist);
 int m6a_prepare_host_io(m6a_ctx *ctx);
 int m6a_host_alloc(size_t bytes, void **out);
 int m6a_host_free(void *p);
diff --git a/m6anet_amd/_lib.py b/m6anet_amd/_lib.py
--- a/m6anet_amd/_lib.py
+++ b/m6anet_amd/_lib.py
@@ -9,9 +9,10 @@
           -6: "M6A_EUNSUPPORTED", -7: "M6A_EFORMAT", -8: "M6A_EIO", -9: "M6A_EDECLINED"}
 M6A_EDECLINED = -9
 RNG_NUMPY = 0
+BAG_HIST_BINS = 4098
 REPR_DTYPES = {"float32": 0, "float16": 1}
 
-SYMBOLS = ["m6a_create", "m6a_destroy", "m6a_last_error", "m6a_set_stream", "m6a_set_job_offset", "m6a_set_scan_driver", "m6a_set_table_variant", "m6a_set_encoder_variant", "m6a_last_encoder_variant", "m6a_last_encoder_kernel", "m6a_sync", "m6a_set_host_offsets", "m6a_prepare_host_io", "m6a_host_alloc", "m6a_host_free", "m6a_host_is_pinned",
+SYMBOLS = ["m6a_create", "m6a_destroy", "m6a_last_error", "m6a_set_stream", "m6a_set_job_offset", "m6a_set_scan_driver", "m6a_set_table_variant", "m6a_set_encoder_variant", "m6a_last_encoder_variant", "m6a_last_encoder_kernel", "m6a_sync", "m6a_set_host_offsets", "m6a_bag_statistics", "m6a_prepare_host_io", "m6a_host_alloc", "m6a_host_free", "m6a_host_is_pinned",
            "m6a_encode_reads", "m6a_read_representation", "m6a_read_representation_dtype", "m6a_site_pool", "m6a_site_expectation", "m6a_set_site_mode", "m6a_infer", "m6a_job_begin", "m6a_job_feed", "m6a_job_feed_collated", "m6a_job_size", "m6a_job_end", "m6a_job_abort", "m6a_bag_forward", "m6a_validate_pool", "m6a_validate", "m6a_flush_groups",
            "m6a_reference_written_sites",
            "m6a_shard_plan", "m6a_comm_unique_id", "m6a_comm_init", "m6a_gather", "m6a_gather_reads", "m6a_device_count", "m6a_random_stream", "m6a_comm_destroy", "m6a_comm_count", "m6a_comm_info", "m6a_device_link", "m6a_profile_enable", "m6a_profile_read", "m6a_profile_clock", "m6a_last_pool_variant",
@@ -136,6 +137,7 @@
     L.m6a_set_stream.argtypes = [vp, vp]
     L.m6a_sync.argtypes = [vp]
     L.m6a_set_host_offsets.argtypes = [vp, vp]
+    L.m6a_bag_statistics.argtypes = [vp, vp, i64, vp, vp]
     L.m6a_prepare_host_io.argtypes = [vp]
     L.m6a_set_job_offset.argtypes = [vp, i64]
     L.m6a_set_scan_driver.argtypes = [vp, i32]
diff --git a/m6anet_amd/csrc/m6a_api.hip b/m6anet_amd/csrc/m6a_api.hip
--- a/m6anet_amd/csrc/m6a_api.hip
+++ b/m6anet_amd/csrc/m6a_api.hip
@@ -151,6 +151,7 @@
     if (!base_is_group_start(base, bs, spb))
         return fail(c, M6A_EINVAL, "job offset %lld does not start a flush group for batch_size=%lld save_per_batch=%lld",
                     (long long)base, (long long)bs, (long long)spb);
+    c->prep_ops++;
     std::vector<int64_t> g;
     const int64_t G = flush_groups(S, bs, spb, base, g);
     int64_t gmax = 0;
@@ -238,6 +239,7 @@
         return fail(c, M6A_ESTREAM, "a flush group would need %lld MT19937 words (cap 2^31); "
                     "reduce batch_size*save_per_batch or num_iterations", (long long)len);
     len = (len + 1023) / 1024 * 1024;
+    c->prep_ops++;
     c->raw_len = 0;
     c->rt.valid = false;
     HIPCHK(c, c->raw.ensure((size_t)len * 4));
@@ -317,6 +319,7 @@
 int ensure_mean_plan(m6a_ctx *c, hipStream_t st, int T)
 {
     if (c->plan.T == T && c->plan_dev.p) return M6A_OK;
+    c->prep_ops++;
     build_mean_plan(T, c->plan);
     const MeanPlan &p = c->plan;
     if (p.depth > M6A_MEAN_STACK) return fail(c, M6A_EUNSUPPORTED, "n_iters %d: pairwise-sum tree deeper than %d", T, M6A_MEAN_STACK);
@@ -392,6 +395,7 @@
     const size_t slot_bytes = (size_t)c_stride * 2 + (size_t)(n_blk + 1) * 4;
     const bool fresh = !rt.valid || rt.n_blk != n_blk;
     const int want = (fresh ? 1 : rt.used) + (int)todo.size();
+    if (fresh || want > rt.cap || !todo.empty()) c->prep_ops++;
     if (fresh || want > rt.cap) {
         int new_cap = std::max(want, fresh ? 0 : rt.cap * 2);
         new_cap = std::min(std::max(new_cap, std::max(32, c->rt_presize)), M6A_RTAB_MAX_N + 1);
@@ -467,6 +471,7 @@
 {
     auto &k = c->tab_reg_key;
     if (k.valid && k.seed == seed && k.n == n && k.T == T && k.K == K && k.jmax >= jmax) return M6A_OK;
+    c->prep_ops++;
     k.valid = false;
     const size_t per_j = (size_t)(T + 8) * K;
     const size_t bytes = (size_t)jmax * per_j * 2 + 4096;
@@ -491,6 +496,7 @@
     if (rc) return rc;
     auto &k = c->tab_key;
     if (k.valid && k.seed == seed && k.n == n && k.T == T && k.K == K && k.jmax >= jmax) return M6A_OK;
+    c->prep_ops++;
     k.valid = false;
     const MeanPlan &p = c->plan;
     const int rows = (int)p.row_pass.size();
@@ -538,17 +544,18 @@
 void host_bag_range(m6a_ctx *c, const int64_t *off, int64_t S);
 int sync_and_check(m6a_ctx *c);
 
+static unsigned bag_check_blocks(int64_t S) { return (unsigned)std::min<int64_t>((S + 255) / 256, 512); }
+
 int query_bags(m6a_ctx *c, const int64_t *d_off, int64_t S)
 {
     if (c->side_work) { HIPCHK(c, hipStreamSynchronize(c->s_prep)); c->side_work = false; }
-    c->h_minmax[0] = ~0ull; c->h_minmax[1] = 0ull; c->h_minmax[2] = 0ull;
-    HIPCHK(c, hipMemcpyAsync(c->d_minmax, c->h_minmax, 24, hipMemcpyHostToDevice, c->stream));
-    HIPCHK(c, hipMemsetAsync(c->d_hist, 0, M6A_HIST_BINS * 4, c->stream));
-    hipLaunchKernelGGL(bag_minmax_kernel, dim3((unsigned)std::min<int64_t>((S + 255) / 256, 512)), dim3(256), 0,
-                       c->stream, d_off, S, c->d_minmax, c->d_hist);
+    unsigned long long *out_acc = c->d_minmax + 4;
+    uint32_t *out_hist = c->d_hist + M6A_HIST_BINS;
+    hipLaunchKernelGGL(bag_check_kernel, dim3(bag_check_blocks(S)), dim3(256), 0, c->stream, d_off, S, c->d_minmax, c->d_hist,
+                       0ull, 0ull, 0ull, 0ull, c->d_err, out_acc, out_hist);
     HIPCHK(c, hipGetLastError());
-    HIPCHK(c, hipMemcpyAsync(c->h_minmax, c->d_minmax, 24, hipMemcpyDeviceToHost, c->stream));
-    HIPCHK(c, hipMemcpyAsync(c->h_hist, c->d_hist, M6A_HIST_BINS * 4, hipMemcpyDeviceToHost, c->stream));
+    HIPCHK(c, hipMemcpyAsync(c->h_minmax, out_acc, 24, hipMemcpyDeviceToHost, c->stream));
+    HIPCHK(c, hipMemcpyAsync(c->h_hist, out_hist, M6A_HIST_BINS * 4, hipMemcpyDeviceToHost, c->stream));
     HIPCHK(c, hipStreamSynchronize(c->stream));
     c->bag_min = (int64_t)c->h_minmax[0];
     c->bag_max = (int64_t)c->h_minmax[1];
@@ -556,28 +563,31 @@
     return M6A_OK;
 }
 
-int bag_stats(m6a_ctx *c, const int64_t *d_off, int64_t S)
+int bag_stats(m6a_ctx *c, const int64_t *d_off, int64_t S, BagCheck *defer)
 {
     const int64_t *h = c->hint_off;
     c->hint_off = nullptr;
+    if (defer) *defer = BagCheck();
     if (!h) return query_bags(c, d_off, S);
     if (h[0] != 0) return fail(c, M6A_EINVAL, "off[0] must be 0");
     host_bag_range(c, h, S);
     if (c->bag_min < 0) return fail(c, M6A_EINVAL, "off[] must be non-decreasing");
-    unsigned long long hash = 0;
-    for (int i = 0; i < M6A_HIST_BINS; i++) hash += (unsigned long long)c->h_hist[i] * m6a_bin_weight(i);
+    BagCheck k;
+    k.armed = true; k.d_off = d_off; k.S = S;
+    k.mn = (unsigned long long)c->bag_min; k.mx = (unsigned long long)c->bag_max; k.reads = (unsigned long long)c->n_reads;
+    for (int i = 0; i < M6A_HIST_BINS; i++) k.hash += (unsigned long long)c->h_hist[i] * m6a_bin_weight(i);
+    if (defer) { *defer = k; return M6A_OK; }
+    if (c->s_prep) HIPCHK(c, hipEventRecord(c->ev_main, c->stream));
+    return bag_check_submit(c, k);
+}
+
+int bag_check_submit(m6a_ctx *c, const BagCheck &k)
+{
+    if (!k.armed) return M6A_OK;
     hipStream_t st = c->s_prep ? c->s_prep : c->stream;
-    if (st != c->stream) {
-        HIPCHK(c, hipEventRecord(c->ev_main, c->stream));
-        HIPCHK(c, hipStreamWaitEvent(st, c->ev_main, 0));
-    }
-    HIPCHK(c, hipMemsetAsync(c->d_minmax, 0xff, 8, st));
-    HIPCHK(c, hipMemsetAsync(c->d_minmax + 1, 0, 16, st));
-    HIPCHK(c, hipMemsetAsync(c->d_hist, 0, M6A_HIST_BINS * 4, st));
-    hipLaunchKernelGGL(bag_minmax_kernel, dim3((unsigned)std::min<int64_t>((S + 255) / 256, 512)), dim3(256), 0,
-                       st, d_off, S, c->d_minmax, c->d_hist);
-    hipLaunchKernelGGL(bag_verify_kernel, dim3(1), dim3(256), 0, st, c->d_minmax, c->d_hist, (unsigned long long)c->bag_min,
-                       (unsigned long long)c->bag_max, (unsigned long long)c->n_reads, hash, c->d_err);
+    if (st != c->stream) HIPCHK(c, hipStreamWaitEvent(st, c->ev_main, 0));
+    hipLaunchKernelGGL(bag_check_kernel, dim3(bag_check_blocks(k.S)), dim3(256), 0, st, k.d_off, k.S, c->d_minmax, c->d_hist,
+                       k.mn, k.mx, k.reads, k.hash, c->d_err, (unsigned long long *)nullptr, (uint32_t *)nullptr);
     HIPCHK(c, hipGetLastError());
     c->side_work = true;
     return M6A_OK;
@@ -687,6 +697,7 @@
     int rc = ensure_rtab(c, st, seed, T, K, gmax, c->h_hist, &use_rtab);
     if (rc) return rc;
     if (!use_rtab) return M6A_OK;
+    c->prep_ops++;
     a.raw = (const uint32_t *)c->raw.p; a.raw_len = c->raw_len;
     HIPCHK(c, c->rt_rank.ensure((size_t)S * 4));
     HIPCHK(c, c->rt_order.ensure((size_t)S * 4));
@@ -717,12 +728,14 @@
     unsigned blocks = 0, start_blocks = 0;
     size_t lds = 0;
     int64_t n_big = 0, cap_big = 0, cap_small = 0;
+    bool queued = false;
 };
 
 int pool_plan(m6a_ctx *c, hipStream_t st, const int64_t *off, int64_t S, int T, int K, uint32_t seed, int64_t bs, int64_t spb,
               PoolPlan *p)
 {
     *p = PoolPlan();
+    struct Mark { m6a_ctx *c; PoolPlan *p; uint64_t at; ~Mark() { p->queued = c->prep_ops != at; } } mark{c, p, c->prep_ops};
     PoolArgs &a = p->a;
     if (S <= 0) return M6A_OK;
     if (c->site_mode == M6A_SITE_EXPECTED) {
@@ -1072,11 +1085,15 @@
     c->b3 = weights[O_B3];
     CRCHK(hipMalloc((void **)&c->d_err, sizeof(int)));
     CRCHK(hipMemset(c->d_err, 0, sizeof(int)));
-    CRCHK(hipMalloc((void **)&c->d_minmax, 24));
+    CRCHK(hipMalloc((void **)&c->d_minmax, 64));
+    CRCHK(hipMemset(c->d_minmax, 0, 64));
+    CRCHK(hipMemset(c->d_minmax, 0xff, 8));
     CRCHK(hipHostMalloc((void **)&c->h_minmax, 24, hipHostMallocDefault));
     CRCHK(hipHostMalloc((void **)&c->h_err, sizeof(int), hipHostMallocDefault));
     *c->h_err = 0;
-    CRCHK(hipMalloc((void **)&c->d_hist, M6A_HIST_BINS * 4));
+    CRCHK(hipMalloc((void **)&c->d_hist, 2 * M6A_HIST_BINS * 4));
+    CRCHK(hipMemset(c->d_hist, 0, 2 * M6A_HIST_BINS * 4));
+    CRCHK(hipStreamSynchronize(nullptr));
     CRCHK(hipHostMalloc((void **)&c->h_hist, M6A_HIST_BINS * 4, hipHostMallocDefault));
     CRCHK(hipHostMalloc((void **)&c->h_ctl, kCtlWords * 4, hipHostMallocDefault));
     for (int n = 0; n <= M6A_RTAB_MAX_N; n++) c->rt.slot_of_n[n] = -1;
@@ -1157,6 +1174,24 @@
     return M6A_OK;
 }
 
+static_assert(M6A_BAG_HIST_BINS == M6A_HIST_BINS, "include/m6a.h states the histogram's size");
+
+int m6a_bag_statistics(m6a_ctx *c, const int64_t *off_dev, int64_t S, int64_t *stats, uint32_t *hist)
+{
+    settle(c);
+    if (!c) return M6A_EINVAL;
+    if (c->job.open) return job_busy(c);
+    if (S < 1) return fail(c, M6A_EINVAL, "n_sites must be >= 1");
+    if (!off_dev || !stats) return fail(c, M6A_EINVAL, "null pointer argument");
+    HIPCHK(c, hipSetDevice(c->device));
+    if (!is_device_ptr(off_dev)) return fail(c, M6A_EINVAL, "m6a_bag_statistics takes a device pointer");
+    int rc = query_bags(c, off_dev, S);
+    if (rc) return rc;
+    stats[0] = c->bag_min; stats[1] = c->bag_max; stats[2] = c->n_reads;
+    if (hist) std::memcpy(hist, c->h_hist, M6A_HIST_BINS * 4);
+    return M6A_OK;
+}
+
 int m6a_set_job_offset(m6a_ctx *c, int64_t first_site)
 {
     if (!c) return M6A_EINVAL;
@@ -1252,9 +1287,12 @@
         if (rc) return rc;
         return sync_and_check(c);
     }
-    int rc = bag_stats(c, off, S);
-    if (rc) return rc;
-    return launch_encode(c, X, km, off, S, c->n_reads, rp);
+    BagCheck chk;
+    int rc = bag_stats(c, off, S, &chk);
+    if (rc) return rc;
+    if (chk.armed && c->s_prep) HIPCHK(c, hipEventRecord(c->ev_main, c->stream));
+    rc = launch_encode(c, X, km, off, S, c->n_reads, rp);
+    return rc ? rc : bag_check_submit(c, chk);
 }
 
 int m6a_read_representation(m6a_ctx *c, const float *X, const uint8_t *km, const int64_t *off, int64_t S, float *repr, float *rp)
@@ -1280,9 +1318,12 @@
         return fail(c, M6A_EINVAL, "X, site_kmers, off, repr, read_prob must be all host or all device pointers");
     if (dev) {
         if ((uintptr_t)repr & 15) return fail(c, M6A_EINVAL, "repr must be 16-byte aligned in device memory");
-        int rc = bag_stats(c, off, S);
+        BagCheck chk;
+        int rc = bag_stats(c, off, S, &chk);
         if (rc) return rc;
-        return launch_repr(c, X, km, off, S, c->n_reads, repr, dtype, rp);
+        if (chk.armed && c->s_prep) HIPCHK(c, hipEventRecord(c->ev_main, c->stream));
+        rc = launch_repr(c, X, km, off, S, c->n_reads, repr, dtype, rp);
+        return rc ? rc : bag_check_submit(c, chk);
     }
     if (off[0] != 0) return fail(c, M6A_EINVAL, "off[0] must be 0");
     for (int64_t s = 0; s < S; s++) if (off[s + 1] < off[s]) return fail(c, M6A_EINVAL, "off[] must be non-decreasing");
@@ -1432,7 +1473,8 @@
         dev != is_device_ptr(mod) || (rp && dev != is_device_ptr(rp)))
         return fail(c, M6A_EINVAL, "all data pointers must be host pointers or all device pointers");
     if (dev) {
-        rc = bag_stats(c, off, S);
+        BagCheck chk;
+        rc = bag_stats(c, off, S, &chk);
         if (rc) return rc;
         const int64_t R = c->n_reads;
         float *p = rp;
@@ -1440,15 +1482,17 @@
         HIPCHK(c, hipEventRecord(c->ev_main, c->stream));
         rc = launch_encode(c, X, km, off, S, R, p);
         if (rc) return rc;
+        rc = bag_check_submit(c, chk);
+        if (rc) return rc;
         hipStream_t st = c->s_prep ? c->s_prep : c->stream;
-        if (st != c->stream) HIPCHK(c, hipStreamWaitEvent(st, c->ev_main, 0));
+        if (st != c->stream && !chk.armed) HIPCHK(c, hipStreamWaitEvent(st, c->ev_main, 0));
         PoolPlan plan;
         rc = pool_plan(c, st, off, S, T, K, seed, bs, spb, &plan);
-        if (rc) return rc;
-        if (st != c->stream) {
+        if (st != c->stream && plan.queued) {
             HIPCHK(c, hipEventRecord(c->ev_prep, st));
             HIPCHK(c, hipStreamWaitEvent(c->stream, c->ev_prep, 0));
         }
+        if (rc) return rc;
         return pool_run(c, plan, p, thr, site, mod);
     }
     if (off[0] != 0) return fail(c, M6A_EINVAL, "off[0] must be 0");
diff --git a/m6anet_amd/csrc/m6a_ctx.h b/m6anet_amd/csrc/m6a_ctx.h
--- a/m6anet_amd/csrc/m6a_ctx.h
+++ b/m6anet_amd/csrc/m6a_ctx.h
@@ -202,6 +202,7 @@
     uint32_t *h_ctl = nullptr;
     DevBuf ctl_dev, rt_rank, rt_order;
     bool side_work = false;
+    uint64_t prep_ops = 0;
     const int64_t *hint_off = nullptr;
     hipEvent_t ev_ctl = nullptr;
     hipStream_t s_prep = nullptr;
@@ -281,7 +282,13 @@
                       int64_t r0, int64_t nr, void *repr, int dtype);
 int launch_pool(m6a_ctx *c, const float *rp, const int64_t *off, int64_t S, int T, int K, float thr, uint32_t seed, int64_t bs, int64_t spb,
                 float *site, double *mod);
-int bag_stats(m6a_ctx *c, const int64_t *d_off, int64_t S);
+struct BagCheck {
+    bool armed = false;
+    const int64_t *d_off = nullptr; int64_t S = 0;
+    unsigned long long mn = 0, mx = 0, reads = 0, hash = 0;
+};
+int bag_stats(m6a_ctx *c, const int64_t *d_off, int64_t S, BagCheck *defer = nullptr);
+int bag_check_submit(m6a_ctx *c, const BagCheck &k);
 void host_bag_range(m6a_ctx *c, const int64_t *off, int64_t S);
 void prof_begin(m6a_ctx *c, int kind);
 void prof_end(m6a_ctx *c, int kind);
diff --git a/m6anet_amd/csrc/m6a_kernels.h b/m6anet_amd/csrc/m6a_kernels.h
--- a/m6anet_amd/csrc/m6a_kernels.h
+++ b/m6anet_amd/csrc/m6a_kernels.h
@@ -130,9 +130,9 @@
 __global__ void sampled_noisy_or_kernel(const float *read_prob, const int32_t *gidx, int64_t n_bags, int k, float *y);
 __global__ void mean_over_passes_kernel(const float *y, int n_iters, int64_t n_sites, float *avg);
 __global__ void pairwise_mean_kernel(const float *y, int n_iters, float *avg);
-__global__ void bag_minmax_kernel(const int64_t *off, int64_t n_sites, unsigned long long *out, uint32_t *hist);
-__global__ void bag_verify_kernel(const unsigned long long *got, const uint32_t *hist, unsigned long long mn, unsigned long long mx,
-                                  unsigned long long reads, unsigned long long hash, int *err);
+__global__ void bag_check_kernel(const int64_t *off, int64_t n_sites, unsigned long long *acc, uint32_t *hist, unsigned long long mn_want,
+                                 unsigned long long mx_want, unsigned long long reads_want, unsigned long long hash_want, int *err,
+                                 unsigned long long *out_acc, uint32_t *out_hist);
 __global__ void mt19937_kernel(uint32_t seed, int64_t n_words, uint32_t *raw, const uint32_t *hist, int64_t seg_words, uint32_t *xhead, int64_t xhead_n);
 __global__ void mt_jump_kernel(const uint32_t *xhead, const uint64_t *polys, uint32_t *hist);
 __global__ void rtab_count_kernel(RtabBuild a);
diff --git a/m6anet_amd/csrc/m6a_kernels.hip b/m6anet_amd/csrc/m6a_kernels.hip
--- a/m6anet_amd/csrc/m6a_kernels.hip
+++ b/m6anet_amd/csrc/m6a_kernels.hip
@@ -1200,10 +1200,15 @@
     if (i < n_plus_1) off[i] = i * step;
 }
 
-__global__ __launch_bounds__(256) void bag_minmax_kernel(const int64_t *off, int64_t n_sites, unsigned long long *out, uint32_t *hist)
+__global__ __launch_bounds__(256) void bag_check_kernel(const int64_t *off, int64_t n_sites, unsigned long long *acc, uint32_t *hist,
+                                                        unsigned long long mn_want, unsigned long long mx_want,
+                                                        unsigned long long reads_want, unsigned long long hash_want, int *err,
+                                                        unsigned long long *out_acc, uint32_t *out_hist)
 {
     __shared__ int64_t s_mn[4], s_mx[4];
     __shared__ uint32_t s_hist[M6A_HIST_BINS];
+    __shared__ unsigned long long s_part[256];
+    __shared__ unsigned s_ticket;
     for (int i = threadIdx.x; i < M6A_HIST_BINS; i += 256) s_hist[i] = 0;
     __syncthreads();
     int64_t mn = INT64_MAX, mx = 0;
@@ -1226,23 +1231,34 @@
         if (s_hist[i]) atomicAdd(&hist[i], s_hist[i]);
     if (threadIdx.x == 0) {
         for (int w = 1; w < 4; w++) { mn = s_mn[w] < mn ? s_mn[w] : mn; mx = s_mx[w] > mx ? s_mx[w] : mx; }
-        atomicMin(&out[0], (unsigned long long)mn);
-        atomicMax(&out[1], (unsigned long long)mx);
-        if (blockIdx.x == 0) out[2] = (unsigned long long)off[n_sites];
-    }
-}
-
-__global__ __launch_bounds__(256) void bag_verify_kernel(const unsigned long long *got, const uint32_t *hist, unsigned long long mn,
-                                                         unsigned long long mx, unsigned long long reads, unsigned long long hash, int *err)
-{
-    __shared__ unsigned long long s_part[256];
+        atomicMin(&acc[0], (unsigned long long)mn);
+        atomicMax(&acc[1], (unsigned long long)mx);
+        if (blockIdx.x == 0) atomicExch(&acc[2], (unsigned long long)off[n_sites]);
+    }
+    asm volatile("s_waitcnt vmcnt(0)" ::: "memory");
+    __syncthreads();
+    if (threadIdx.x == 0) {
+        __threadfence();
+        asm volatile("s_waitcnt vmcnt(0)" ::: "memory");
+        s_ticket = atomicInc((unsigned *)&acc[3], gridDim.x - 1);
+    }
+    __syncthreads();
+    if (s_ticket != gridDim.x - 1) return;
+    __threadfence();
     unsigned long long h = 0;
-    for (int i = threadIdx.x; i < M6A_HIST_BINS; i += 256) h += (unsigned long long)hist[i] * m6a_bin_weight(i);
+    for (int i = threadIdx.x; i < M6A_HIST_BINS; i += 256) {
+        const uint32_t n = atomicExch(&hist[i], 0u);
+        if (out_hist) out_hist[i] = n;
+        h += (unsigned long long)n * m6a_bin_weight(i);
+    }
     s_part[threadIdx.x] = h;
     __syncthreads();
     if (threadIdx.x == 0) {
         for (int i = 1; i < 256; i++) h += s_part[i];
-        if (got[0] != mn || got[1] != mx || got[2] != reads || h != hash) atomicExch(err, 3);
+        const unsigned long long got_mn = atomicExch(&acc[0], ~0ull), got_mx = atomicExch(&acc[1], 0ull),
+                                 got_reads = atomicExch(&acc[2], 0ull);
+        if (out_acc) { out_acc[0] = got_mn; out_acc[1] = got_mx; out_acc[2] = got_reads; }
+        else if (got_mn != mn_want || got_mx != mx_want || got_reads != reads_want || h != hash_want) atomicExch(err, 3);
     }
 }
 
diff --git a/m6anet_amd/engine.py b/m6anet_amd/engine.py
--- a/m6anet_amd/engine.py
+++ b/m6anet_amd/engine.py
@@ -192,6 +192,15 @@
         a = np.ascontiguousarray(off_host, dtype=np.int64)
         self._host_off_keepalive = a
         self._chk(self._L.m6a_set_host_offsets(self._h, a.ctypes.data))
+
+    def bag_statistics(self, off):
+        aO = _Arg(off, np.int64, "int64")
+        if not aO.is_dev:
+            raise TypeError("off must be a device tensor")
+        stats = np.zeros(3, np.int64)
+        hist = np.zeros(_lib.BAG_HIST_BINS, np.uint32)
+        self._chk(self._L.m6a_bag_statistics(self._h, aO.ptr, aO.size - 1, stats.ctypes.data, hist.ctypes.data))
+        return int(stats[0]), int(stats[1]), int(stats[2]), hist
 
     def comm_init(self, unique_id, rank, world_size):
         buf = (C.c_char * 128).from_buffer_copy(bytes(unique_id))
```
